# qcraftai/pillarnext

Measured on AMD Instinct MI355X. Metric: frames/s PillarNeXt-B nuScenes 300k-pt cloud (inference, end-to-end), higher is better.
Workload: dtype bf16

## Files before the change

include/pnx.h:

```cpp
#ifndef PNX_H
#define PNX_H

#include <stddef.h>
#include <stdint.h>

#ifdef __cplusplus
extern "C" {
#endif

typedef void* pnx_stream_t;

typedef enum pnx_status {
  PNX_OK = 0,
  PNX_ERR_INVALID = -1,
  PNX_ERR_UNSUPPORTED = -2,
  PNX_ERR_WORKSPACE = -3,
  PNX_ERR_HIP = -4
} pnx_status;

typedef enum pnx_dtype { PNX_F32 = 0, PNX_BF16 = 1, PNX_F16 = 2 } pnx_dtype;
typedef enum pnx_layout {
  PNX_NHWC = 0,
  PNX_NCHW = 1
} pnx_layout;
// ... 15 lines not shown
                    const float* w0, const float* gamma0, const float* beta0, const float* mean0, const float* var0,
                    const float* w1, const float* gamma1, const float* beta1, const float* mean1, const float* var1,
                    float eps, float* folded_out, pnx_stream_t stream);

size_t pnx_reader_workspace_bytes(int64_t n_points, int32_t batch, const pnx_geom* geom_host);

int pnx_reader_forward(const float* points, int64_t n_points, int32_t row_stride, int32_t batch, const pnx_geom* geom_host,
                       const float* pfn_folded, void* canvas, int32_t canvas_dtype, int32_t canvas_layout, uint8_t* occupancy,
                       float* feat_max, int32_t* coords, int64_t pillar_capacity, int64_t* unq_inv, int32_t* pillar_of_point,
                       int32_t* counts, void* workspace, size_t workspace_bytes, pnx_stream_t stream);

void pnx_reader_fill_split(int32_t* percent3_host);

int pnx_profile_begin(int32_t max_samples);
int pnx_profile_end(float* reader_us_avg_host, float* canvas_us_avg_host, int32_t* samples_host);
float pnx_profile_last_pfn_us(void);
float pnx_profile_last_voxelize_us(void);

size_t pnx_pfn_train_param_floats(int32_t num_point_features);
size_t pnx_pfn_train_partial_floats(int32_t num_point_features, int32_t which);
int pnx_pfn_forward_train(int32_t pass, const float* points, int64_t n_points, int32_t row_stride, int32_t batch, const pnx_geom* geom_host,
                          const float* params, float* partials, float* feat_max, int64_t pillar_capacity, int32_t* coords,
                          int32_t* pillar_of_point, int32_t* counts, void* workspace, size_t workspace_bytes, pnx_stream_t stream);
int pnx_pfn_backward(int32_t pass, int64_t n_points, int32_t row_stride, int32_t batch, const pnx_geom* geom_host, const float* params,
                     const float* grad_feat_max, const float* feat_max, float* partials, void* workspace, size_t workspace_bytes,
                     pnx_stream_t stream);

int pnx_voxelize(const float* points, int64_t n_points, int32_t row_stride, int32_t batch, const pnx_geom* geom_host,
                 float* features, int32_t* coords, int64_t pillar_capacity, int64_t* unq_inv, int32_t* pillar_of_point,
                 int32_t* counts, void* workspace, size_t workspace_bytes, pnx_stream_t stream);

typedef enum pnx_group_mode { PNX_GROUP_VOXEL = 0, PNX_GROUP_PILLAR_CLAMP = 1, PNX_GROUP_CYLINDER_CLAMP = 2 } pnx_group_mode;
typedef struct pnx_group_geom {
  float min[3], voxel[3];
  int32_t grid[3];
  int32_t mode;
  int32_t prefilter;
  float keep_min[3], keep_max[3];
} pnx_group_geom;
size_t pnx_group_workspace_bytes(int64_t n_points, int32_t row_stride, int32_t batch, const pnx_group_geom* geom_host);
int pnx_group_points(const float* points, int64_t n_points, int32_t row_stride, int32_t batch, const pnx_group_geom* geom_host, float* point_features,
                     int32_t feature_ld, int32_t* coords, int64_t group_capacity, int64_t* unq_inv, float* group_mean, int32_t* counts, void* workspace,
                     size_t workspace_bytes, pnx_stream_t stream);
int pnx_pfn_layer_eval(const float* xa, int32_t lda, int32_t ca, const float* gb, int32_t cb, const int64_t* inv, const float* wt, const float* shift,
                       int32_t cout, int64_t n, int64_t num_groups, float* y, int32_t ldy, float* gmax, pnx_stream_t stream);
int pnx_bilinear_gather(const void* image, int32_t dtype, int32_t batch, int32_t h, int32_t w, int32_t channels, const float* pos, int32_t pos_ld,
                        const float* pos_min2_host, const float* pos_voxel2_host, const int32_t* cell_coords, const int64_t* unq_inv, int32_t ds_rate,
                        int64_t n, float* out, int32_t out_ld, pnx_stream_t stream);
size_t pnx_bilinear_gather_backward_workspace_bytes(int64_t n, int32_t batch, int32_t h, int32_t w);
int pnx_bilinear_gather_backward(const float* grad_out, int32_t grad_ld, int32_t batch, int32_t h, int32_t w, int32_t channels, const float* pos,
                                 int32_t pos_ld, const float* pos_min2_host, const float* pos_voxel2_host, const int32_t* cell_coords,
                                 const int64_t* unq_inv, int32_t ds_rate, int64_t n, float* grad_image, void* workspace, size_t workspace_bytes,
                                 pnx_stream_t stream);

size_t pnx_scatter_max_workspace_bytes(int64_t n, int64_t num_pillars);
int pnx_scatter_max(const float* x, const int64_t* index, int64_t n, int32_t channels, int64_t num_pillars, float* out,
                    int64_t* argmax, void* workspace, size_t workspace_bytes, pnx_stream_t stream);
int pnx_scatter_max_backward(const float* grad_out, const int64_t* argmax, int64_t n, int32_t channels, int64_t num_pillars,
                             float* grad_x, pnx_stream_t stream);

int pnx_scatter_canvas(const float* feat_max, const int32_t* coords, const int32_t* num_pillars_dev, int64_t pillar_capacity,
                       int32_t batch, int32_t gy, int32_t gx, void* canvas, int32_t canvas_dtype, int32_t canvas_layout,
                       pnx_stream_t stream);

size_t pnx_merge_sweeps_desc_bytes(void);
size_t pnx_merge_sweeps_workspace_bytes(int64_t n_raw);
int pnx_merge_sweeps(const float* raw, int64_t n_raw, int32_t raw_stride, int32_t n_copy, const void* seg_descs_dev, int32_t n_segments, float* out,
                     int32_t* n_out_dev, void* workspace, size_t workspace_bytes, pnx_stream_t stream);

int pnx_bias_act_mask(const void* x, const void* residual, const float* bias, const uint8_t* mask, void* out, int64_t sites,
                      int32_t channels, int32_t dtype, int32_t relu, pnx_stream_t stream);
int pnx_sum_bias_act(const void* const* srcs, int32_t n_src, const float* bias, void* out, int64_t sites, int32_t channels, int32_t dtype,
                     int32_t relu, pnx_stream_t stream);
int pnx_deconv2x2_bf16(const void* x, const void* wfrag, const float* bias, void* y, int32_t batch, int32_t h, int32_t w, int32_t cin, int32_t cout,
                       int32_t relu, pnx_stream_t stream);
int pnx_deconv2x2_f16(const void* x, const void* wfrag, const float* bias, void* y, int32_t batch, int32_t h, int32_t w, int32_t cin, int32_t cout,
                       int32_t relu, pnx_stream_t stream);
int pnx_conv3x3_bf16(const void* x, const void* wfrag, const float* bias, const void* residual, const uint8_t* mask, void* y, int32_t batch,
                     int32_t h, int32_t w, int32_t cin, int32_t cout, int32_t stride, int32_t relu, uint8_t* row_dirty, const int32_t* tile_list,
                     const int32_t* tile_count, pnx_stream_t stream);
int pnx_conv3x3_f16(const void* x, const void* wfrag, const float* bias, const void* residual, const uint8_t* mask, void* y, int32_t batch,
                    int32_t h, int32_t w, int32_t cin, int32_t cout, int32_t stride, int32_t relu, uint8_t* row_dirty, const int32_t* tile_list,
                    const int32_t* tile_count, pnx_stream_t stream);
size_t pnx_conv3x3_wgrad_workspace_bytes(int32_t cin, int32_t cout);
int pnx_conv3x3_wgrad_bf16(const void* x, const void* dy, const uint8_t* mask, float* dw, int32_t batch, int32_t h, int32_t w, int32_t cin, int32_t cout,
                           int32_t stride, void* workspace, size_t workspace_bytes, pnx_stream_t stream);
int pnx_conv3x3_wgrad_x3(const void* x_hi, const void* x_lo, const void* dy_hi, const void* dy_lo, const uint8_t* mask, float* dw, int32_t batch, int32_t h,
                         int32_t w, int32_t cin, int32_t cout, int32_t stride, void* workspace, size_t workspace_bytes, pnx_stream_t stream);
int pnx_conv3x3_wgrad_x6(const void* x_hi, const void* x_mid, const void* x_lo, const void* dy_hi, const void* dy_mid, const void* dy_lo, const uint8_t* mask,
                         float* dw, int32_t batch, int32_t h, int32_t w, int32_t cin, int32_t cout, int32_t stride, void* workspace, size_t workspace_bytes,
                         pnx_stream_t stream);
int pnx_conv3x3_pack_weights(const void* w, int32_t dtype, int32_t cout, int32_t cin, int32_t transposed, void* wfrag, pnx_stream_t stream);
int pnx_conv3x3_tile_rows(int32_t cin, int32_t cout, int32_t stride);
int pnx_conv_tile_list(const uint8_t* mask, const uint8_t* const* row_dirty, int32_t n_dirty, int32_t batch, int32_t h, int32_t w, int32_t tile_rows,
                       int32_t* tile_list, int32_t* tile_count, pnx_stream_t stream);
int pnx_sephead_out_bf16(const void* x, const void* wfrag, const float* bias, void* y, int32_t batch, int32_t h, int32_t w, int32_t n_branch,
                         pnx_stream_t stream);
int pnx_sephead_out_f16(const void* x, const void* wfrag, const float* bias, void* y, int32_t batch, int32_t h, int32_t w, int32_t n_branch,
                         pnx_stream_t stream);
typedef struct {
  const void* up;
  const void* wfrag1;
  const float* bias1;
  const float* w2c;
  const float* bias2;
  int32_t h, w;
} PnxLazyTask;
int pnx_sephead_lazy_bf16(const PnxLazyTask* tasks, int32_t n_tasks, const int32_t* class_task, int32_t nc_total, int32_t batch, const int64_t* local,
                          const int32_t* seg_len, int32_t pre_max, float* out, pnx_stream_t stream);
int pnx_sephead_lazy_f16(const PnxLazyTask* tasks, int32_t n_tasks, const int32_t* class_task, int32_t nc_total, int32_t batch, const int64_t* local,
                          const int32_t* seg_len, int32_t pre_max, float* out, pnx_stream_t stream);
int pnx_split_f32(const float* x, void* hi, void* lo, int64_t n, const uint8_t* mask, int32_t channels, pnx_stream_t stream);
int pnx_conv3x3_x3(const void* x_hi, const void* x_lo, const void* wfrag_hi, const void* wfrag_lo, const float* bias, const uint8_t* mask, float* y,
                   int32_t batch, int32_t h, int32_t w, int32_t cin, int32_t cout, int32_t stride, pnx_stream_t stream);
int pnx_split3_f32(const float* x, void* hi, void* mid, void* lo, int64_t n, const uint8_t* mask, int32_t channels, pnx_stream_t stream);
int pnx_conv3x3_x6(const void* x_hi, const void* x_mid, const void* x_lo, const void* wfrag_hi, const void* wfrag_mid, const void* wfrag_lo, const float* bias,
                   const uint8_t* mask, float* y, int32_t batch, int32_t h, int32_t w, int32_t cin, int32_t cout, int32_t stride, pnx_stream_t stream);
int pnx_conv3x3_dgrad_s2_bf16(const void* g, const void* wfrag_t, const uint8_t* mask_in, void* dx, int32_t batch, int32_t h, int32_t w, int32_t cin,
                              int32_t cout, pnx_stream_t stream);
int pnx_conv3x3_dgrad_s2_x3(const void* g_hi, const void* g_lo, const void* wfrag_t_hi, const void* wfrag_t_lo, const uint8_t* mask_in, float* dx, int32_t batch,
                            int32_t h, int32_t w, int32_t cin, int32_t cout, pnx_stream_t stream);
int pnx_conv3x3_dgrad_s2_x6(const void* g_hi, const void* g_mid, const void* g_lo, const void* wfrag_t_hi, const void* wfrag_t_mid, const void* wfrag_t_lo,
                            const uint8_t* mask_in, float* dx, int32_t batch, int32_t h, int32_t w, int32_t cin, int32_t cout, pnx_stream_t stream);
int pnx_conv3x3_smallk(const void* x, const float* weight, const float* bias, void* y, int32_t batch, int32_t h, int32_t w, int32_t cin, int32_t k,
                       int32_t dtype, pnx_stream_t stream);
size_t pnx_conv3x3_smallk_wgrad_workspace_bytes(int32_t k);
int pnx_conv3x3_smallk_wgrad(const void* x, const void* dy, float* dw, float* dbias, int32_t batch, int32_t h, int32_t w, int32_t cin, int32_t k,
                             int32_t dtype, void* workspace, size_t workspace_bytes, pnx_stream_t stream);
int pnx_mask_pool3(const uint8_t* mask_in, int32_t batch, int32_t h, int32_t w, int32_t stride, uint8_t* mask_out, pnx_stream_t stream);

int pnx_boxes_overlap_bev(const float* boxes_a, int64_t n, const float* boxes_b, int64_t m, float* out, pnx_stream_t stream);
int pnx_boxes_iou_bev(const float* boxes_a, int64_t n, const float* boxes_b, int64_t m, float* out, pnx_stream_t stream);
int pnx_boxes_aligned_overlap_bev(const float* boxes_a, const float* boxes_b, int64_t n, float* out, pnx_stream_t stream);
int pnx_boxes_aligned_iou3d(const float* boxes_a, const float* boxes_b, int64_t n, float* out, pnx_stream_t stream);

int pnx_boxes_iou_bev_cpu(const float* boxes_a_host, int64_t n, const float* boxes_b_host, int64_t m, float* out_host);
int pnx_boxes_aligned_iou_bev_cpu(const float* boxes_a_host, const float* boxes_b_host, int64_t n, float* out_host);
size_t pnx_nms_workspace_bytes(int64_t total_boxes, int32_t num_segments, int32_t max_seg_len);
int32_t pnx_debug_nms_pair_cap(int32_t cap);
int pnx_nms_rotated_batched(const float* boxes, const int32_t* seg_offsets, const int32_t* seg_len, int32_t num_segments, int32_t max_seg_len,
                            const float* thresh, int32_t post_max, int32_t* keep, int32_t* keep_count, void* workspace,
                            size_t workspace_bytes, pnx_stream_t stream);
int pnx_nms_normal_batched(const float* boxes, const int32_t* seg_offsets, const int32_t* seg_len, int32_t num_segments, int32_t max_seg_len,
                           const float* thresh, int32_t post_max, int32_t* keep, int32_t* keep_count, void* workspace,
                           size_t workspace_bytes, pnx_stream_t stream);

size_t pnx_decode_task_desc_bytes(void);
size_t pnx_decode_topk_workspace_bytes(int64_t n_keys, int32_t num_segments);
int pnx_decode_topk(const uint64_t* keys, int64_t n_keys, int32_t num_segments, int32_t pre_max, uint64_t* sorted_keys, int64_t* order,
                    int64_t* seg_start, int32_t* seg_len, int32_t* seg_total, void* workspace, size_t workspace_bytes, pnx_stream_t stream);
int pnx_decode_keys(const void* packed, int32_t dtype, int32_t batch, int32_t n_classes_total, const void* task_desc_host, uint64_t* keys,
                    pnx_stream_t stream);
size_t pnx_sort_keys_workspace_bytes(int64_t n_keys);
int pnx_sort_keys(const uint64_t* keys, int64_t n_keys, int32_t num_segments, uint64_t* sorted_keys, int64_t* order, void* workspace,
                  size_t workspace_bytes, pnx_stream_t stream);
int pnx_decode_boxes(const void* const* task_ptrs_dev, const void* task_descs_dev, const int64_t* task_key_off_dev, int32_t n_tasks,
                     int32_t dtype, int32_t batch, const uint64_t* sorted_keys, const int64_t* order, const int64_t* seg_start,
                     const int32_t* seg_len, int32_t num_segments, int32_t pre_max, float* boxes9, float* boxes7, float* scores,
                     pnx_stream_t stream);
int pnx_decode_boxes_lazy(const void* task_descs_dev, const int64_t* task_key_off_dev, int32_t n_tasks, int32_t n_classes_total,
                          const uint64_t* sorted_keys, const int64_t* order, const int64_t* seg_start, int32_t* seg_len, const int32_t* seg_total,
                          int32_t num_segments, int32_t pre_max, const float* cand, float* boxes9, float* boxes7, float* scores, int32_t* flag_dev,
                          pnx_stream_t stream);
int pnx_gather_kept(const float* boxes9, const float* scores, const int32_t* keep, const int32_t* keep_count, int32_t num_segments,
                    int32_t pre_max, int32_t post_max, float* out, pnx_stream_t stream);

// ... 136 lines not shown
```

pillarnext_amd/_lib.py:

```python
import ctypes
import os

_HERE = os.path.dirname(os.path.abspath(__file__))
LIB_PATH = os.environ.get("PNX_LIB") or os.path.join(_HERE, "libpnx_hip.so")

PNX_F32, PNX_BF16, PNX_F16 = 0, 1, 2
PNX_NHWC, PNX_NCHW = 0, 1


class PnxError(RuntimeError):
    pass


class PnxGeom(ctypes.Structure):
    _fields_ = [("pc_min", ctypes.c_float * 3), ("voxel", ctypes.c_float * 3), ("gx", ctypes.c_int32), ("gy", ctypes.c_int32)]


PNX_GROUP_VOXEL, PNX_GROUP_PILLAR_CLAMP, PNX_GROUP_CYLINDER_CLAMP = 0, 1, 2


class PnxGroupGeom(ctypes.Structure):
    _fields_ = [("min", ctypes.c_float * 3), ("voxel", ctypes.c_float * 3), ("grid", ctypes.c_int32 * 3), ("mode", ctypes.c_int32),
                ("prefilter", ctypes.c_int32), ("keep_min", ctypes.c_float * 3), ("keep_max", ctypes.c_float * 3)]


PNX_ASSIGN_MAX_TASKS, PNX_ASSIGN_MAX_CLASSES = 8, 32
PNX_PASTE_MAX_BOXES, PNX_PASTE_MAX_BATCH = 512, 64
PNX_AUG_ROTATE, PNX_AUG_SCALE, PNX_AUG_TRANSLATE, PNX_AUG_FLIP_X, PNX_AUG_FLIP_Y = 1, 2, 4, 8, 16


class PnxAssignDesc(ctypes.Structure):
    _fields_ = [("lo", ctypes.c_double * 2), ("voxel", ctypes.c_double * 2), ("overlap", ctypes.c_double), ("min_radius", ctypes.c_int32),
                ("max_objs", ctypes.c_int32), ("n_tasks", ctypes.c_int32), ("n_classes", ctypes.c_int32)] + \
               [(k, ctypes.c_int32 * PNX_ASSIGN_MAX_TASKS) for k in ("osf", "h", "w", "ncls")] + \
               [(k, ctypes.c_int32 * PNX_ASSIGN_MAX_CLASSES) for k in ("class_task", "class_cls")]


_vp = ctypes.c_void_p
_i64 = ctypes.c_int64
_i32 = ctypes.c_int32
_f32 = ctypes.c_float
_sz = ctypes.c_size_t
_i3p = ctypes.POINTER(ctypes.c_int32)

PROTOTYPES = {
    "pnx_last_error": (ctypes.c_char_p, []),
    "pnx_version": (ctypes.c_char_p, []),
    "pnx_geom_init": (ctypes.c_int, [ctypes.POINTER(ctypes.c_double), ctypes.POINTER(ctypes.c_double), ctypes.POINTER(PnxGeom)]),
    "pnx_pfn_fold_bn": (ctypes.c_int, [_i32] + [_vp] * 10 + [_f32, _vp, _vp]),
    "pnx_reader_workspace_bytes": (_sz, [_i64, _i32, ctypes.POINTER(PnxGeom)]),
    "pnx_reader_forward": (ctypes.c_int, [_vp, _i64, _i32, _i32, ctypes.POINTER(PnxGeom), _vp, _vp, _i32, _i32, _vp, _vp, _vp, _i64, _vp, _vp,
                                          _vp, _vp, _sz, _vp]),
    "pnx_reader_fill_split": (None, [ctypes.POINTER(ctypes.c_int32)]),
    "pnx_profile_begin": (ctypes.c_int, [_i32]),
    "pnx_profile_end": (ctypes.c_int, [ctypes.POINTER(ctypes.c_float), ctypes.POINTER(ctypes.c_float), ctypes.POINTER(ctypes.c_int32)]),
    "pnx_profile_last_pfn_us": (ctypes.c_float, []),
    "pnx_profile_last_voxelize_us": (ctypes.c_float, []),
    "pnx_pfn_train_param_floats": (_sz, [_i32]),
    "pnx_pfn_train_partial_floats": (_sz, [_i32, _i32]),
    "pnx_pfn_forward_train": (ctypes.c_int, [_i32, _vp, _i64, _i32, _i32, ctypes.POINTER(PnxGeom), _vp, _vp, _vp, _i64, _vp, _vp, _vp, _vp, _sz, _vp]),
    "pnx_pfn_backward": (ctypes.c_int, [_i32, _i64, _i32, _i32, ctypes.POINTER(PnxGeom), _vp, _vp, _vp, _vp, _vp, _sz, _vp]),
    "pnx_voxelize": (ctypes.c_int, [_vp, _i64, _i32, _i32, ctypes.POINTER(PnxGeom), _vp, _vp, _i64, _vp, _vp, _vp, _vp, _sz, _vp]),
    "pnx_group_workspace_bytes": (_sz, [_i64, _i32, _i32, ctypes.POINTER(PnxGroupGeom)]),
    "pnx_group_points": (ctypes.c_int, [_vp, _i64, _i32, _i32, ctypes.POINTER(PnxGroupGeom), _vp, _i32, _vp, _i64, _vp, _vp, _vp, _vp, _sz, _vp]),
    "pnx_pfn_layer_eval": (ctypes.c_int, [_vp, _i32, _i32, _vp, _i32, _vp, _vp, _vp, _i32, _i64, _i64, _vp, _i32, _vp, _vp]),
    "pnx_bilinear_gather": (ctypes.c_int, [_vp, _i32, _i32, _i32, _i32, _i32, _vp, _i32, ctypes.POINTER(ctypes.c_float), ctypes.POINTER(ctypes.c_float), _vp,
                                           _vp, _i32, _i64, _vp, _i32, _vp]),
    "pnx_bilinear_gather_backward_workspace_bytes": (_sz, [_i64, _i32, _i32, _i32]),
    "pnx_bilinear_gather_backward": (ctypes.c_int, [_vp, _i32, _i32, _i32, _i32, _i32, _vp, _i32, ctypes.POINTER(ctypes.c_float),
                                                    ctypes.POINTER(ctypes.c_float), _vp, _vp, _i32, _i64, _vp, _vp, _sz, _vp]),
    "pnx_scatter_max_workspace_bytes": (_sz, [_i64, _i64]),
    "pnx_scatter_max": (ctypes.c_int, [_vp, _vp, _i64, _i32, _i64, _vp, _vp, _vp, _sz, _vp]),
    "pnx_scatter_max_backward": (ctypes.c_int, [_vp, _vp, _i64, _i32, _i64, _vp, _vp]),
    "pnx_scatter_canvas": (ctypes.c_int, [_vp, _vp, _vp, _i64, _i32, _i32, _i32, _vp, _i32, _i32, _vp]),
    "pnx_merge_sweeps_desc_bytes": (_sz, []),
    "pnx_merge_sweeps_workspace_bytes": (_sz, [_i64]),
    "pnx_merge_sweeps": (ctypes.c_int, [_vp, _i64, _i32, _i32, _vp, _i32, _vp, _vp, _vp, _sz, _vp]),
    "pnx_bias_act_mask": (ctypes.c_int, [_vp, _vp, _vp, _vp, _vp, _i64, _i32, _i32, _i32, _vp]),
    "pnx_sum_bias_act": (ctypes.c_int, [_vp, _i32, _vp, _vp, _i64, _i32, _i32, _i32, _vp]),
    "pnx_deconv2x2_bf16": (ctypes.c_int, [_vp, _vp, _vp, _vp, _i32, _i32, _i32, _i32, _i32, _i32, _vp]),
    "pnx_deconv2x2_f16": (ctypes.c_int, [_vp, _vp, _vp, _vp, _i32, _i32, _i32, _i32, _i32, _i32, _vp]),
    "pnx_sephead_out_bf16": (ctypes.c_int, [_vp, _vp, _vp, _vp, _i32, _i32, _i32, _i32, _vp]),
    "pnx_sephead_out_f16": (ctypes.c_int, [_vp, _vp, _vp, _vp, _i32, _i32, _i32, _i32, _vp]),
    "pnx_masked_bn_blocks": (_i32, []),
    "pnx_masked_bn_reduce": (ctypes.c_int, [_vp, _i32, _i32, _vp, _vp]),
    "pnx_masked_bn_finalize": (ctypes.c_int, [_vp, _i32, _vp, _vp, _vp, ctypes.c_double, ctypes.c_double, _vp, _vp, _vp, _vp, _vp, _vp, _vp, _vp, _vp]),
    "pnx_masked_bn_bwd_finalize": (ctypes.c_int, [_vp, _vp, _i32, _vp, _vp, _vp, _vp, _vp, _vp]),
    "pnx_masked_bn_stats": (ctypes.c_int, [_vp, _i32, _vp, _i64, _i32, _vp, _vp, _vp]),
    "pnx_masked_bn_apply": (ctypes.c_int, [_vp, _vp, _i32, _vp, _i64, _i32, _vp, _vp, _i32, _vp, _vp]),
    "pnx_masked_bn_bwd_stats": (ctypes.c_int, [_vp, _vp, _vp, _i32, _vp, _i64, _i32, _vp, _vp, _vp, _vp, _i32, _vp, _vp]),
    "pnx_masked_bn_bwd_apply": (ctypes.c_int, [_vp, _vp, _vp, _i32, _vp, _i64, _i32, _vp, _vp, _vp, _vp, _i32, _vp, _vp, _vp, _vp, _vp]),
    "pnx_sephead_lazy_bf16": (ctypes.c_int, [_vp, _i32, _vp, _i32, _i32, _vp, _vp, _i32, _vp, _vp]),
    "pnx_sephead_lazy_f16": (ctypes.c_int, [_vp, _i32, _vp, _i32, _i32, _vp, _vp, _i32, _vp, _vp]),
    "pnx_conv3x3_bf16": (ctypes.c_int, [_vp, _vp, _vp, _vp, _vp, _vp, _i32, _i32, _i32, _i32, _i32, _i32, _i32, _vp, _vp, _vp, _vp]),
    "pnx_conv3x3_f16": (ctypes.c_int, [_vp, _vp, _vp, _vp, _vp, _vp, _i32, _i32, _i32, _i32, _i32, _i32, _i32, _vp, _vp, _vp, _vp]),
    "pnx_conv3x3_tile_rows": (ctypes.c_int, [_i32, _i32, _i32]),
    "pnx_conv3x3_pack_weights": (ctypes.c_int, [_vp, _i32, _i32, _i32, _i32, _vp, _vp]),
    "pnx_conv3x3_wgrad_workspace_bytes": (_sz, [_i32, _i32]),
    "pnx_conv3x3_wgrad_bf16": (ctypes.c_int, [_vp, _vp, _vp, _vp, _i32, _i32, _i32, _i32, _i32, _i32, _vp, _sz, _vp]),
    "pnx_conv3x3_wgrad_x3": (ctypes.c_int, [_vp, _vp, _vp, _vp, _vp, _vp, _i32, _i32, _i32, _i32, _i32, _i32, _vp, _sz, _vp]),
    "pnx_conv3x3_wgrad_x6": (ctypes.c_int, [_vp, _vp, _vp, _vp, _vp, _vp, _vp, _vp, _i32, _i32, _i32, _i32, _i32, _i32, _vp, _sz, _vp]),
    "pnx_conv3x3_dgrad_s2_bf16": (ctypes.c_int, [_vp, _vp, _vp, _vp, _i32, _i32, _i32, _i32, _i32, _vp]),
    "pnx_conv3x3_dgrad_s2_x3": (ctypes.c_int, [_vp, _vp, _vp, _vp, _vp, _vp, _i32, _i32, _i32, _i32, _i32, _vp]),
    "pnx_conv3x3_dgrad_s2_x6": (ctypes.c_int, [_vp, _vp, _vp, _vp, _vp, _vp, _vp, _vp, _i32, _i32, _i32, _i32, _i32, _vp]),
    "pnx_conv3x3_smallk": (ctypes.c_int, [_vp, _vp, _vp, _vp, _i32, _i32, _i32, _i32, _i32, _i32, _vp]),
    "pnx_conv3x3_smallk_wgrad_workspace_bytes": (_sz, [_i32]),
    "pnx_conv3x3_smallk_wgrad": (ctypes.c_int, [_vp, _vp, _vp, _vp, _i32, _i32, _i32, _i32, _i32, _i32, _vp, _sz, _vp]),
    "pnx_conv_tile_list": (ctypes.c_int, [_vp, _vp, _i32, _i32, _i32, _i32, _i32, _vp, _vp, _vp]),
    "pnx_mask_pool3": (ctypes.c_int, [_vp, _i32, _i32, _i32, _i32, _vp, _vp]),
    "pnx_split_f32": (ctypes.c_int, [_vp, _vp, _vp, _i64, _vp, _i32, _vp]),
    "pnx_conv3x3_x3": (ctypes.c_int, [_vp, _vp, _vp, _vp, _vp, _vp, _vp, _i32, _i32, _i32, _i32, _i32, _i32, _vp]),
    "pnx_split3_f32": (ctypes.c_int, [_vp, _vp, _vp, _vp, _i64, _vp, _i32, _vp]),
    "pnx_conv3x3_x6": (ctypes.c_int, [_vp, _vp, _vp, _vp, _vp, _vp, _vp, _vp, _vp, _i32, _i32, _i32, _i32, _i32, _i32, _vp]),
    "pnx_decode_task_desc_bytes": (_sz, []),
    "pnx_decode_topk_workspace_bytes": (_sz, [_i64, _i32]),
    "pnx_decode_topk": (ctypes.c_int, [_vp, _i64, _i32, _i32, _vp, _vp, _vp, _vp, _vp, _vp, _sz, _vp]),
    "pnx_decode_keys": (ctypes.c_int, [_vp, _i32, _i32, _i32, _vp, _vp, _vp]),
    "pnx_sort_keys_workspace_bytes": (ctypes.c_size_t, [_i64]),
    "pnx_sort_keys": (ctypes.c_int, [_vp, _i64, _i32, _vp, _vp, _vp, ctypes.c_size_t, _vp]),
    "pnx_decode_boxes": (ctypes.c_int, [_vp, _vp, _vp, _i32, _i32, _i32, _vp, _vp, _vp, _vp, _i32, _i32, _vp, _vp, _vp, _vp]),
    "pnx_decode_boxes_lazy": (ctypes.c_int, [_vp, _vp, _i32, _i32, _vp, _vp, _vp, _vp, _vp, _i32, _i32, _vp, _vp, _vp, _vp, _vp, _vp]),
    "pnx_gather_kept": (ctypes.c_int, [_vp, _vp, _vp, _vp, _i32, _i32, _i32, _vp, _vp]),
    "pnx_enqueue": (ctypes.c_int, [_vp, _i32, _vp]),
    "pnx_decode_lazy_enqueue": (ctypes.c_int, [_vp, _vp]),
    "pnx_op_bytes": (_sz, []),
    "pnx_lazy_decode_bytes": (_sz, []),
    "pnx_center_loss_workspace_bytes": (_sz, [_i32, _i32]),
    "pnx_center_loss_forward": (ctypes.c_int, [_vp, _vp, _vp, _vp, _vp, _vp, _vp, _i32, _i32, _i32, _i32, _i32, _vp, _i32, _vp, _vp, _sz, _vp]),
    "pnx_center_loss_backward": (ctypes.c_int, [_vp, _vp, _vp, _vp, _vp, _vp, _vp, _vp, _i32, _i32, _i32, _i32, _i32, _vp, _i32, _vp, _vp, _vp, _vp, _sz, _vp]),
    "pnx_assign_workspace_bytes": (_sz, [_i32, _i32, _i32]),
    "pnx_assign_labels": (ctypes.c_int, [_vp, _vp, _vp, _i32, _i32, ctypes.POINTER(PnxAssignDesc), _vp, _vp, _vp, _vp, _vp, _vp, _vp, _vp, _sz, _vp]),
    "pnx_paste_chunk_rows": (_i32, []),
    "pnx_paste_select": (ctypes.c_int, [_vp, _vp, _vp, _i32, _i32, _i32, _vp, _vp, _vp, _vp, _i32, _i32, _vp, _i32, _vp, _vp, _vp, _vp, _vp, _vp, _vp]),
    "pnx_paste_augment_workspace_bytes": (_sz, [_i64, _i32]),
    "pnx_paste_augment_points": (ctypes.c_int, [_vp, _i64, _i32, _i32, _vp, _vp, _vp, _vp, _i32, _i32, _vp, _vp, _i32, _i64, _vp, _vp, _i64, _vp, _vp, _vp,
                                                _sz, _vp]),
    "pnx_augment_boxes": (ctypes.c_int, [_vp, _vp, _i32, _i32, _i32, _vp, _vp]),
    "pnx_boxes_overlap_bev": (ctypes.c_int, [_vp, _i64, _vp, _i64, _vp, _vp]),
    "pnx_boxes_iou_bev": (ctypes.c_int, [_vp, _i64, _vp, _i64, _vp, _vp]),
    "pnx_boxes_aligned_overlap_bev": (ctypes.c_int, [_vp, _vp, _i64, _vp, _vp]),
    "pnx_boxes_aligned_iou3d": (ctypes.c_int, [_vp, _vp, _i64, _vp, _vp]),
    "pnx_boxes_iou_bev_cpu": (ctypes.c_int, [_vp, _i64, _vp, _i64, _vp]),
    "pnx_boxes_aligned_iou_bev_cpu": (ctypes.c_int, [_vp, _vp, _i64, _vp]),
    "pnx_nms_workspace_bytes": (_sz, [_i64, _i32, _i32]),
    "pnx_debug_nms_pair_cap": (_i32, [_i32]),
    "pnx_nms_rotated_batched": (ctypes.c_int, [_vp, _vp, _vp, _i32, _i32, _vp, _i32, _vp, _vp, _vp, _sz, _vp]),
    "pnx_nms_normal_batched": (ctypes.c_int, [_vp, _vp, _vp, _i32, _i32, _vp, _i32, _vp, _vp, _vp, _sz, _vp]),
    "pnx_sp3_index_bytes": (_sz, [_i32, _i3p]),
    "pnx_sp3_index_build": (ctypes.c_int, [_vp, _i64, _i32, _i3p, _vp, _sz, _vp, _vp, _vp]),
    "pnx_sp3_out_grid": (ctypes.c_int, [_i32, _i3p, _i3p, _i3p, _i3p, _i3p]),
    "pnx_sp3_out_index": (ctypes.c_int, [_vp, _i64, _i32, _i3p, _i3p, _i3p, _i3p, _vp, _sz, _vp, _vp]),
    "pnx_sp3_index_coords": (ctypes.c_int, [_vp, _sz, _i32, _i3p, _vp, _i64, _vp]),
    "pnx_sp3_neighbor_map": (ctypes.c_int, [_vp, _i64, _vp, _sz, _i32, _i3p, _vp, _i3p, _i3p, _i3p, _vp, _vp]),
    "pnx_sp3_packed_weight_floats": (_sz, [_i32, _i32, _i32]),
    "pnx_sp3_conv": (ctypes.c_int, [_vp, _i64, _i32, _vp, _i64, _i32, _vp, _vp, _vp, _i32, _vp, _i32, _vp]),
    "pnx_sp3_conv_train": (ctypes.c_int, [_vp, _i64, _i32, _vp, _i64, _i32, _vp, _vp, _vp, _i32, _vp, _i32, _vp]),
    "pnx_sp3_dense": (ctypes.c_int, [_vp, _vp, _i64, _i32, _i32, _i3p, _vp, _vp]),
    "pnx_sp3_packed_weight_halfs": (_sz, [_i32, _i32, _i32]),
    "pnx_sp3_conv_h": (ctypes.c_int, [_vp, _i64, _i32, _i32, _vp, _i64, _i32, _vp, _vp, _vp, _i32, _vp, _i32, _i32, _i32, _vp]),
    "pnx_sp3_dense_h": (ctypes.c_int, [_vp, _i32, _vp, _i64, _i32, _i32, _i32, _i3p, _vp, _vp]),
    "pnx_sp3_transpose_map": (ctypes.c_int, [_vp, _i64, _i32, _i64, _vp, _vp]),
    "pnx_sp3_wgrad_workspace_bytes": (_sz, [_i64, _i32, _i32, _i32]),
    "pnx_sp3_wgrad": (ctypes.c_int, [_vp, _i64, _i32, _vp, _i32, _vp, _i64, _i32, _vp, _vp, _sz, _vp]),
    "pnx_sp3_dense_backward": (ctypes.c_int, [_vp, _vp, _i64, _i32, _i32, _i3p, _vp, _vp]),
}

_LIB = None


def lib():
    global _LIB
    if _LIB is None:
        if not os.path.exists(LIB_PATH):
            raise PnxError(f"{LIB_PATH} is missing: run `python -m pillarnext_amd.build` (hipcc, gfx950). "
                           "There is no CPU fallback for the product path.")
        L = ctypes.CDLL(LIB_PATH)
        for name, (res, args) in PROTOTYPES.items():
            fn = getattr(L, name)
# ... 29 lines not shown
```

pillarnext_amd/csrc/conv3x3.hip:

```cpp
#include "pnx_common.h"

namespace {

#include "conv_tile.h"

template <int CIN, int COUT, int STRIDE, bool W_LDS>
__global__ __launch_bounds__(256, 2) void k_conv3x3(const uint16_t* __restrict__ x, const uint4* __restrict__ wfrag,
                                                 const float* __restrict__ bias, const uint16_t* __restrict__ res,
                                                 const uint8_t* __restrict__ mask, uint16_t* __restrict__ y, int B, int H, int W, int Ho,
                                                 int Wo, int relu, uint8_t* __restrict__ row_dirty) {
  constexpr int CB = CIN / 16, MT = COUT / 32, KSTEPS = 9 * CB;
  constexpr int NT = (MT <= 2) ? 4 : 2;
  extern __shared__ uint4 s_w[];
  const int lane = threadIdx.x & 63, wv = threadIdx.x >> 6;
  const int px = lane & 31, kb = lane >> 5;
  if (W_LDS) {
    for (int i = threadIdx.x; i < KSTEPS * MT * 64; i += 256) s_w[i] = wfrag[i];
    __syncthreads();
  }
  const int tiles_x = (Wo + 31) >> 5, tiles_y = (Ho + NT - 1) / NT;
  const int64_t n_tiles = (int64_t)B * tiles_y * tiles_x;
  for (int64_t tile = (int64_t)blockIdx.x * 4 + wv; tile < n_tiles; tile += (int64_t)gridDim.x * 4) {
    const int tx = (int)(tile % tiles_x);
    const int ty = (int)((tile / tiles_x) % tiles_y);
// ... 199 lines not shown
  return PNX_OK;
}

}

extern "C" {

#if defined(PNX_CONV_TIMERS) && !defined(PNX_CONV_F16)
int pnx_debug_conv_timers(unsigned long long* out) {
  unsigned long long z[8] = {0, 0, 0, 0, 0, 0, 0, 0};
  PNX_CHECK_HIP(hipDeviceSynchronize());
  PNX_CHECK_HIP(hipMemcpyFromSymbol(out, HIP_SYMBOL(g_conv_T), sizeof(z)));
  PNX_CHECK_HIP(hipMemcpyToSymbol(HIP_SYMBOL(g_conv_T), z, sizeof(z)));
  return PNX_OK;
}
#endif

int PNX_CONV_FN(pnx_sephead_out)(const void* x, const void* wfrag, const float* bias, void* y, int32_t batch, int32_t h, int32_t w, int32_t n_branch,
                         pnx_stream_t stream) {
  PNX_REQUIRE(x && wfrag && bias && y && batch > 0 && h > 0 && w > 0, PNX_ERR_INVALID, "bad arguments");
  PNX_REQUIRE((((uintptr_t)x | (uintptr_t)y | (uintptr_t)wfrag | (uintptr_t)bias) & 15) == 0, PNX_ERR_INVALID, "16-byte alignment required");
  hipStream_t st = (hipStream_t)stream;
  switch (n_branch) {
    case 1: return launch_sephead<1>(x, wfrag, bias, y, batch, h, w, st);
    case 2: return launch_sephead<2>(x, wfrag, bias, y, batch, h, w, st);
    case 5: return launch_sephead<5>(x, wfrag, bias, y, batch, h, w, st);
    case 6: return launch_sephead<6>(x, wfrag, bias, y, batch, h, w, st);
    case 7: return launch_sephead<7>(x, wfrag, bias, y, batch, h, w, st);
    default: break;
  }
  pnx_set_error("pnx_sephead_out: no kernel for %d branches", n_branch);
  return PNX_ERR_UNSUPPORTED;
}

int PNX_CONV_FN(pnx_deconv2x2)(const void* x, const void* wfrag, const float* bias, void* y, int32_t batch, int32_t h, int32_t w, int32_t cin, int32_t cout,
                       int32_t relu, pnx_stream_t stream) {
  PNX_REQUIRE(x && wfrag && bias && y && batch > 0 && h > 0 && w > 0, PNX_ERR_INVALID, "bad arguments");
  PNX_REQUIRE((((uintptr_t)x | (uintptr_t)y | (uintptr_t)wfrag | (uintptr_t)bias) & 15) == 0, PNX_ERR_INVALID, "16-byte alignment required");
  if (cin != 64 || cout != 64) {
    pnx_set_error("pnx_deconv2x2: no kernel for %d -> %d channels", cin, cout);
    return PNX_ERR_UNSUPPORTED;
  }
  const int64_t n_seg = (int64_t)batch * h * ((w + 31) / 32);
  int64_t nb = (n_seg + 3) / 4;
  if (nb > 512) nb = 512;
  k_deconv2x2_64<<<(unsigned)nb, 256, 0, (hipStream_t)stream>>>((const uint16_t*)x, (const uint4*)wfrag, bias, (uint16_t*)y, batch, h, w, relu);
  PNX_LAUNCH_CHECK();
  return PNX_OK;
}

#ifndef PNX_CONV_F16
int pnx_conv3x3_tile_rows(int32_t cin, int32_t cout, int32_t stride) {
  if (stride != 1) return 0;
  if (cin == 64 && (cout == 64 || cout == 320 || cout == 384 || cout == 448)) return LDS_TH;
  if ((cin == 128 && cout == 128) || (cin == 256 && (cout == 256 || cout == 64))) return L128_TH;
  return 0;
}

static int conv_tile_list_impl(const uint8_t* mask, const uint8_t* const* row_dirty, int32_t n_dirty, int32_t batch, int32_t h, int32_t w, int32_t tile_rows,
                               int32_t* tile_list, int32_t* tile_count, pnx_stream_t stream, bool zero_count) {
  PNX_REQUIRE(mask && tile_list && tile_count && batch > 0 && h > 0 && w > 0 && tile_rows > 0, PNX_ERR_INVALID, "bad arguments");
  PNX_REQUIRE(n_dirty >= 0 && n_dirty <= 4 && (n_dirty == 0 || row_dirty != nullptr), PNX_ERR_INVALID, "0..4 row_dirty arrays");
  DirtySet ds;
  for (int k = 0; k < 4; k++) ds.p[k] = k < n_dirty ? row_dirty[k] : nullptr;
  hipStream_t st = (hipStream_t)stream;
  if (zero_count) PNX_CHECK_HIP(hipMemsetAsync(tile_count, 0, sizeof(int32_t), st));
  const int64_t n_tiles = (int64_t)batch * ((h + tile_rows - 1) / tile_rows) * ((w + 31) / 32);
  PNX_REQUIRE(tile_rows <= 16, PNX_ERR_UNSUPPORTED, "tile_rows %d (at most 16: one lane per row)", tile_rows);
  k_tile_list<<<(unsigned)((n_tiles + 15) / 16), 256, 0, st>>>(mask, ds, batch, h, w, tile_rows, tile_list, tile_count);
  PNX_LAUNCH_CHECK();
  return PNX_OK;
}
int pnx_conv_tile_list(const uint8_t* mask, const uint8_t* const* row_dirty, int32_t n_dirty, int32_t batch, int32_t h, int32_t w, int32_t tile_rows,
                       int32_t* tile_list, int32_t* tile_count, pnx_stream_t stream) {
  return conv_tile_list_impl(mask, row_dirty, n_dirty, batch, h, w, tile_rows, tile_list, tile_count, stream, true);
}
int pnx_conv_tile_list_prezeroed(const uint8_t* mask, const uint8_t* const* row_dirty, int32_t n_dirty, int32_t batch, int32_t h, int32_t w, int32_t tile_rows,
                                 int32_t* tile_list, int32_t* tile_count, pnx_stream_t stream) {
  return conv_tile_list_impl(mask, row_dirty, n_dirty, batch, h, w, tile_rows, tile_list, tile_count, stream, false);
}

#endif

int PNX_CONV_FN(pnx_conv3x3)(const void* x, const void* wfrag, const float* bias, const void* residual, const uint8_t* mask, void* y, int32_t batch,
                     int32_t h, int32_t w, int32_t cin, int32_t cout, int32_t stride, int32_t relu, uint8_t* row_dirty, const int32_t* tile_list,
                     const int32_t* tile_count, pnx_stream_t stream) {
  PNX_REQUIRE((tile_list == nullptr) == (tile_count == nullptr), PNX_ERR_INVALID, "tile_list and tile_count come together");
  PNX_REQUIRE(tile_list == nullptr || (mask != nullptr && pnx_conv3x3_tile_rows(cin, cout, stride) > 0), PNX_ERR_INVALID,
              "a tile list needs a mask and a kernel that takes one (pnx_conv3x3_tile_rows)");
  PNX_REQUIRE(x && wfrag && bias && y && batch > 0 && h > 0 && w > 0, PNX_ERR_INVALID, "bad arguments");
  PNX_REQUIRE(stride == 1 || stride == 2, PNX_ERR_UNSUPPORTED, "stride %d", stride);
  PNX_REQUIRE(row_dirty == nullptr || mask != nullptr, PNX_ERR_INVALID, "row_dirty needs an active-site mask");
  PNX_REQUIRE((((uintptr_t)x | (uintptr_t)y | (uintptr_t)wfrag | (uintptr_t)bias | (uintptr_t)residual) & 15) == 0, PNX_ERR_INVALID,
              "16-byte alignment required");
  const int ho = (h + 2 - 3) / stride + 1, wo = (w + 2 - 3) / stride + 1;
  hipStream_t st = (hipStream_t)stream;
  const ConvArgs a = {(const uint16_t*)x, (const uint4*)wfrag, bias, (const uint16_t*)residual, mask, (uint16_t*)y, batch, h, w, relu, row_dirty, tile_list,
                      tile_count, st};
  if (stride == 1 && getenv("PNX_CONV_DIRECT") == nullptr) {
    static const int pc_mode = getenv("PNX_CONV_PC") != nullptr ? atoi(getenv("PNX_CONV_PC")) : 1;
    static const int pack_mode = getenv("PNX_CONV_PACK") != nullptr ? atoi(getenv("PNX_CONV_PACK")) : 3;
    if (pc_mode != 0) {
      if (cin == 64 && cout == 64) return launch_pc<64, 64>(a, (pack_mode & 2) != 0);
      if (residual == nullptr && (pc_mode & 4)) {
        if (cin == 64 && cout == 320) return launch_pc<64, 320>(a);
        if (cin == 64 && cout == 384) return launch_pc<64, 384>(a);
        if (cin == 64 && cout == 448) return launch_pc<64, 448>(a);
      }
      if (pc_mode & 2) {
        if (cin == 128 && cout == 128) return launch_pc<128, 128>(a);
        if (cin == 256 && cout == 256) return launch_pc<256, 256>(a);
      }
    }
    if (cin == 64 && cout == 64) return launch_lds<64>(a);
    const bool pack = (pack_mode & 1) != 0;
    if (cin == 128 && cout == 128) return launch_ldsx<128, 128>(a, pack);
    if (cin == 256 && cout == 64) return launch_ldsx<256, 64>(a);
    if (cin == 256 && cout == 256) return launch_ldsx<256, 256>(a, pack);
    if (cin == 64 && cout == 384) return launch_lds<384>(a);
    if (cin == 64 && cout == 320) return launch_lds<320>(a);
    if (cin == 64 && cout == 448) return launch_lds<448>(a);
  }
  if (stride == 2 && residual == nullptr && getenv("PNX_CONV_DIRECT") == nullptr) {
    if (cin == 64 && cout == 128) return launch_s2<64, 128, 1>(x, wfrag, bias, mask, y, batch, h, w, ho, wo, relu, row_dirty, st);
    if (cin == 128 && cout == 256) return launch_s2<128, 256, 1>(x, wfrag, bias, mask, y, batch, h, w, ho, wo, relu, row_dirty, st);
    if (cin == 256 && cout == 256) return launch_s2<256, 256, 1>(x, wfrag, bias, mask, y, batch, h, w, ho, wo, relu, row_dirty, st);
  }
#define PNX_CONV_CASE(CI, CO)                             \
  if (cin == CI && cout == CO) {                          \
    if (stride == 1) return launch<CI, CO, 1>(a, ho, wo); \
    return launch<CI, CO, 2>(a, ho, wo);                  \
  }
  PNX_CONV_CASE(64, 64)
  PNX_CONV_CASE(64, 128)
  PNX_CONV_CASE(128, 128)
#undef PNX_CONV_CASE
  pnx_set_error("pnx_conv3x3: no kernel for %d -> %d channels", cin, cout);
  return PNX_ERR_UNSUPPORTED;
}

#ifndef PNX_CONV_F16
}
namespace {
#include "conv_dgrad_s2.h"

template <int NP>
int dgrad_s2_impl(const char* name, PnxPieces<NP> g, PnxPieces<NP> wfrag_t, const uint8_t* mask_in, void* dx, int32_t batch, int32_t h, int32_t w, int32_t cin,
                  int32_t cout, pnx_stream_t stream) {
  PNX_REQUIRE(g.complete() && wfrag_t.complete() && mask_in && dx && batch > 0 && h > 0 && w > 0, PNX_ERR_INVALID, "%s: bad arguments", name);
  PNX_REQUIRE(((g.bits() | wfrag_t.bits() | (uintptr_t)dx) & 15) == 0, PNX_ERR_INVALID, "16-byte alignment required");
  hipStream_t st = (hipStream_t)stream;
  if (cin == 64 && cout == 128) return launch_dgrad_s2<128, 64, NP>(g, wfrag_t, mask_in, dx, batch, h, w, st);
  if (cin == 128 && cout == 256) return launch_dgrad_s2<256, 128, NP>(g, wfrag_t, mask_in, dx, batch, h, w, st);
  if (cin == 256 && cout == 256) return launch_dgrad_s2<256, 256, NP>(g, wfrag_t, mask_in, dx, batch, h, w, st);
  pnx_set_error("%s: no kernel for %d -> %d channels", name, cin, cout);
  return PNX_ERR_UNSUPPORTED;
}

template <int NP>
int conv3x3_f32_impl(const char* name, PnxPieces<NP> x, PnxPieces<NP> wfrag, const float* bias, const uint8_t* mask, float* y, int32_t batch, int32_t h, int32_t w,
                     int32_t cin, int32_t cout, int32_t stride, pnx_stream_t stream) {
  PNX_REQUIRE(x.complete() && wfrag.complete() && y, PNX_ERR_INVALID, "null pointer");
  PNX_REQUIRE(batch > 0 && h > 0 && w > 0, PNX_ERR_INVALID, "bad shape");
  PNX_REQUIRE(stride == 1 || stride == 2, PNX_ERR_UNSUPPORTED, "stride %d", stride);
  PNX_REQUIRE(((x.bits() | wfrag.bits() | (uintptr_t)y | (uintptr_t)bias) & 15) == 0, PNX_ERR_INVALID, "16-byte alignment required");
  hipStream_t st = (hipStream_t)stream;
  if (stride == 1) {
    if (cin == 64 && cout == 64) return launch_pc_f32<64, 64, NP>(x, wfrag, bias, mask, y, batch, h, w, st);
    if (cin == 128 && cout == 128) return launch_pc_f32<128, 128, NP>(x, wfrag, bias, mask, y, batch, h, w, st);
    if (cin == 256 && cout == 256) return launch_pc_f32<256, 256, NP>(x, wfrag, bias, mask, y, batch, h, w, st);
  } else {
    const int ho = (h - 1) / 2 + 1, wo = (w - 1) / 2 + 1;
    if (cin == 64 && cout == 128) return launch_s2<64, 128, NP>(x, wfrag, bias, mask, y, batch, h, w, ho, wo, 0, nullptr, st);
    if (cin == 128 && cout == 256) return launch_s2<128, 256, NP>(x, wfrag, bias, mask, y, batch, h, w, ho, wo, 0, nullptr, st);
    if (cin == 256 && cout == 256) return launch_s2<256, 256, NP>(x, wfrag, bias, mask, y, batch, h, w, ho, wo, 0, nullptr, st);
  }
  pnx_set_error("%s: no kernel for %d -> %d channels, stride %d", name, cin, cout, stride);
  return PNX_ERR_UNSUPPORTED;
}

}
extern "C" {

int pnx_conv3x3_dgrad_s2_bf16(const void* g, const void* wfrag_t, const uint8_t* mask_in, void* dx, int32_t batch, int32_t h, int32_t w, int32_t cin, int32_t cout,
                              pnx_stream_t stream) {
  return dgrad_s2_impl<1>("pnx_conv3x3_dgrad_s2_bf16", {g}, {wfrag_t}, mask_in, dx, batch, h, w, cin, cout, stream);
}

int pnx_conv3x3_dgrad_s2_x3(const void* g_hi, const void* g_lo, const void* wfrag_t_hi, const void* wfrag_t_lo, const uint8_t* mask_in, float* dx, int32_t batch,
                            int32_t h, int32_t w, int32_t cin, int32_t cout, pnx_stream_t stream) {
  return dgrad_s2_impl<2>("pnx_conv3x3_dgrad_s2_x3", {g_hi, g_lo}, {wfrag_t_hi, wfrag_t_lo}, mask_in, dx, batch, h, w, cin, cout, stream);
}

int pnx_conv3x3_dgrad_s2_x6(const void* g_hi, const void* g_mid, const void* g_lo, const void* wfrag_t_hi, const void* wfrag_t_mid, const void* wfrag_t_lo,
                            const uint8_t* mask_in, float* dx, int32_t batch, int32_t h, int32_t w, int32_t cin, int32_t cout, pnx_stream_t stream) {
  return dgrad_s2_impl<3>("pnx_conv3x3_dgrad_s2_x6", {g_hi, g_mid, g_lo}, {wfrag_t_hi, wfrag_t_mid, wfrag_t_lo}, mask_in, dx, batch, h, w, cin, cout, stream);
}

int pnx_conv3x3_x3(const void* x_hi, const void* x_lo, const void* wfrag_hi, const void* wfrag_lo, const float* bias, const uint8_t* mask, float* y,
                   int32_t batch, int32_t h, int32_t w, int32_t cin, int32_t cout, int32_t stride, pnx_stream_t stream) {
  return conv3x3_f32_impl<2>("pnx_conv3x3_x3", {x_hi, x_lo}, {wfrag_hi, wfrag_lo}, bias, mask, y, batch, h, w, cin, cout, stride, stream);
}

int pnx_conv3x3_x6(const void* x_hi, const void* x_mid, const void* x_lo, const void* wfrag_hi, const void* wfrag_mid, const void* wfrag_lo, const float* bias,
                   const uint8_t* mask, float* y, int32_t batch, int32_t h, int32_t w, int32_t cin, int32_t cout, int32_t stride, pnx_stream_t stream) {
  return conv3x3_f32_impl<3>("pnx_conv3x3_x6", {x_hi, x_mid, x_lo}, {wfrag_hi, wfrag_mid, wfrag_lo}, bias, mask, y, batch, h, w, cin, cout, stride, stream);
}
#endif

}

namespace {

constexpr int kLzG = 32, kLzN = kLzG * 9, kLzNT = kLzN / 32;
constexpr int kLzPatch = kLzG * 25 * 8;
constexpr int kLzW2 = 10 * 9 * 32 * 3;
constexpr int kLzMaxTasks = 8, kLzMaxClasses = 32;
constexpr int kLzAhead = 2;

#include "sephead_lazy.h"

// ... 26 lines not shown
```

pillarnext_amd/csrc/conv_rows.h:

```cpp
#pragma once


template <int NR, int COUT, bool HAS_RES>
__device__ __forceinline__ void conv_rows(const uint4* __restrict__ s_in, const uint4* __restrict__ wfrag, const float* __restrict__ bias,
                                          const uint16_t* const (&rrow_res)[4], uint32_t res_off, const int (&rbase)[4], const uint32_t (&rmask)[4],
                                          uint16_t* const (&yrow)[4], int n_valid, int relu, int px, int kb, int lane) {
  constexpr int MTALL = COUT / 32;
#pragma unroll 1
  for (int mg = 0; mg < MTALL; mg += 2) {
    v16f acc[NR][2];
#pragma unroll
    for (int m = 0; m < 2; m++) {
      const v16f bq = bias_tile(bias, (mg + m) * 32, kb);
#pragma unroll
      for (int j = 0; j < NR; j++) acc[j][m] = bq;
    }
    uint4 rq[2][2];
    if (HAS_RES) load_residual_u(rq, rrow_res[0], res_off, rmask[0] >> px & 1u);
    conv_taps<NR, MTALL, 4, 1, 2, COUT == 64 ? 2 : TAPS_WD>(acc, s_in, wfrag, rbase, mg, px, kb, lane);
#pragma unroll
    for (int j = 0; j < NR; j++) {
      const bool act = (rmask[j] >> px) & 1u;
      uint4 rc[2][2];
      if (HAS_RES) {
// ... 70 lines not shown
#pragma unroll
    for (int j = 0; j < 4; j++) {
      was[j] = __builtin_amdgcn_readfirstlane(wasP[j]) != 0;
      const uint32_t bal = (uint32_t)__ballot(aP[j]);
      if (lane == 0) s_rowmask[wv * 4 + j] = bal;
    }
    __syncthreads();
    idxC = sched_next2(s_next, it, slot, idxB);
    tileC = tile_at(tlist, idxC, n_tiles);
    load_mask(tileB, aN, wasN);
#pragma unroll
    for (int j = 0; j < 4; j++) aP[j] = aN[j], wasP[j] = wasN[j];
    CT_TOCK(0)
    const uint32_t my_rm = s_rowmask[lane & 15];
    const uint32_t am = (uint32_t)__ballot(my_rm != 0) & 0xffffu;
#pragma unroll
    for (int j = 0; j < 4; j++) {
      const int rr = wv * 4 + j, oy = y0 + rr;
      const bool active = (am >> rr) & 1u;
      if (!active && was[j] && oy < H && ox < W) {
        uint4* dst = reinterpret_cast<uint4*>(y + (((int64_t)b * H + oy) * W + ox) * COUT);
#pragma unroll 1
        for (int ch = kb; ch < COUT / 8; ch += 2) dst[ch] = make_uint4(0, 0, 0, 0);
      }
      if (row_dirty != nullptr && oy < H && lane == 0 && was[j] != active) row_dirty[((int64_t)b * H + oy) * tiles_x + tx] = active ? 1 : 0;
    }
    if (am == 0) continue;
    int nr = 0;
    int rbase[4], rrow[4];
    {
      uint32_t rest = am;
      for (int k = 0; k < wv && rest; k++) rest &= rest - 1;
#pragma unroll
      for (int j = 0; j < 4; j++) {
        const bool has = rest != 0;
        rrow[j] = has ? __builtin_ctz(rest) : 0;
        nr += has ? 1 : 0;
        for (int k = 0; k < 4 && rest; k++) rest &= rest - 1;
      }
    }
    nr = __builtin_amdgcn_readfirstlane(nr);
    uint32_t rmask[4];
    uint16_t* yrow[4];
#pragma unroll
    for (int j = 0; j < 4; j++) {
      rrow[j] = __builtin_amdgcn_readfirstlane(rrow[j]);
      rbase[j] = rrow[j] * HW_ * 8;
      rmask[j] = j < nr ? __builtin_amdgcn_readfirstlane(s_rowmask[rrow[j]]) : 0u;
      yrow[j] = y + (((int64_t)b * H + (y0 + rrow[j])) * W + x0) * COUT;
    }
    const uint32_t need = am | (am << 1) | (am << 2);
    CT_TOCK(1)
    const uint16_t* rres[4];
#pragma unroll
    for (int j = 0; j < 4; j++) rres[j] = HAS_RES ? res + (((int64_t)b * H + (y0 + rrow[j])) * W + x0) * COUT : nullptr;
    const uint32_t res_off = (uint32_t)(px * COUT + 8 * kb) * 2u;
    stage_tile64<CIN>(s_in, x, b, H, W, 0, y0, x0, need);
    CT_TOCK(2)
    __syncthreads();
    CT_TOCK(3)
    const int n_valid = W - x0;
    switch (nr) {
      case 1: conv_rows<1, COUT, HAS_RES>(s_in, wfrag, bias, rres, res_off, rbase, rmask, yrow, n_valid, relu, px, kb, lane); break;
      case 2: conv_rows<2, COUT, HAS_RES>(s_in, wfrag, bias, rres, res_off, rbase, rmask, yrow, n_valid, relu, px, kb, lane); break;
      case 3: conv_rows<3, COUT, HAS_RES>(s_in, wfrag, bias, rres, res_off, rbase, rmask, yrow, n_valid, relu, px, kb, lane); break;
      case 4: conv_rows<4, COUT, HAS_RES>(s_in, wfrag, bias, rres, res_off, rbase, rmask, yrow, n_valid, relu, px, kb, lane); break;
      default: break;
    }
    CT_TOCK(4)
  }
  sched_done(slot);
  CT_FLUSH
}

constexpr int L128_TH = 8;
constexpr int L128_NSTAGE = (L128_TH + 2) * LDS_HW * 8;

int next_sched_slot() {
  static unsigned int n = 0;
  return (int)(n++ & 63u);
}

constexpr int LDSX_RES_WD = 2;
template <int NR, int CIN, int COUT, bool HAS_RES>
__device__ __forceinline__ void conv_rows_x(uint4* __restrict__ s_in, const uint16_t* __restrict__ x, const uint4* __restrict__ wfrag,
                                            const float* __restrict__ bias, const uint16_t* __restrict__ res, const int (&rrow)[4],
                                            const int (&rbase)[4], const uint32_t (&rmask)[4], uint16_t* const (&yrow)[4], int b, int H, int W,
                                            int y0, int x0, uint32_t need, int mg0, int relu, int px, int kb, int lane, int hsel) {
  constexpr int NS = CIN / 64, NRA = NR > 0 ? NR : 1;
  const int ox = x0 + px;
  {
    const int h = hsel;
    const int mg = mg0 + 4 * h;
    v16f acc[NRA][2];
    if (NR > 0) {
#pragma unroll
      for (int m = 0; m < 2; m++) {
        const v16f bq = bias_tile(bias, (mg + m) * 32, kb);
#pragma unroll
        for (int j = 0; j < NR; j++) acc[j][m] = bq;
      }
    }
    const uint16_t* rres[NRA];
    const uint32_t res_off = (uint32_t)(px * COUT + 8 * kb) * 2u;
    uint4 rq[2][2];
    if (NR > 0 && HAS_RES) {
#pragma unroll
      for (int j = 0; j < NR; j++) rres[j] = res + (((int64_t)b * H + (y0 + rrow[j])) * W + x0) * COUT + mg * 32;
    }
#pragma unroll 1
    for (int sl = 0; sl < NS; sl++) {
      if (sl) {
        __syncthreads();
        stage_tile64<CIN, L128_TH>(s_in, x, b, H, W, 64 * sl, y0, x0, need);
        __syncthreads();
      }
      if (NR > 0 && HAS_RES && sl == NS - 1) load_residual_u(rq, rres[0], res_off, rmask[0] >> px & 1u);
      if (NR > 0) conv_taps<NRA, COUT / 32, CIN / 16, 1, 2, HAS_RES ? LDSX_RES_WD : TAPS_WD>(acc, s_in, wfrag, rbase, mg, px, kb, lane, 4 * sl);
    }
    if (NR > 0) {
      const int n_valid = W - x0;
#pragma unroll
      for (int j = 0; j < NR; j++) {
        const bool act = (rmask[j] >> px) & 1u;
        uint4 rc[2][2];
        if (HAS_RES) {
#pragma unroll
          for (int m = 0; m < 2; m++)
#pragma unroll
            for (int t = 0; t < 2; t++) rc[m][t] = rq[m][t];
          if (j + 1 < NR) load_residual_u(rq, rres[j + 1], res_off, rmask[j + 1] >> px & 1u);
        }
        uint4 D[4];
#pragma unroll
        for (int m = 0; m < 2; m++) {
          uint4 pk[2];
          pack_tile(acc[j][m], act, relu, pk, HAS_RES ? rc[m] : nullptr);
          D[2 * m] = pk[0], D[2 * m + 1] = pk[1];
        }
        transpose_row64(D, lane);
        store_row64<COUT>(D, yrow[j] + mg * 32, n_valid, lane);
      }
    }
  }
}

__device__ __forceinline__ int pix_code(int row, int col) { return (row << 5) | col; }
template <int CSTRIDE>
__device__ __forceinline__ uint32_t pix_off(int code, int W) { return (uint32_t)(((code >> 5) * W + (code & 31)) * CSTRIDE) * 2u; }

template <int CSTRIDE>
__device__ __forceinline__ void store_pix64(const uint4 (&D)[4], uint16_t* __restrict__ tile, int code, int n_valid, int W, int lane) {
  int l = lane;
  asm volatile("" : "+v"(l));
#pragma unroll
  for (int d = 0; d < 4; d++) {
    const int P = 8 * d + (l >> 3);
    const int pc = __builtin_amdgcn_ds_bpermute(P << 2, code);
    if (P < n_valid) *reinterpret_cast<uint4*>(reinterpret_cast<char*>(tile) + pix_off<CSTRIDE>(pc, W) + (uint32_t)((l & 7) * 16)) = D[d];
  }
}

template <int NR, int CIN, int COUT, bool HAS_RES>
__device__ __forceinline__ void conv_pix_x(uint4* __restrict__ s_in, const uint16_t* __restrict__ x, const uint4* __restrict__ wfrag,
                                           const float* __restrict__ bias, const uint16_t* __restrict__ rtile, int codes, const int (&n_g)[4],
                                           uint16_t* __restrict__ ytile, int b, int H, int W, int y0, int x0, uint32_t need, int mg0, int relu, int px,
                                           int kb, int lane, int hsel) {
  constexpr int NS = CIN / 64, NRA = NR > 0 ? NR : 1;
  const int mg = mg0 + 4 * hsel;
  v16f acc[NRA][2];
  if (NR > 0) {
#pragma unroll
    for (int m = 0; m < 2; m++) {
      const v16f bq = bias_tile(bias, (mg + m) * 32, kb);
#pragma unroll
      for (int j = 0; j < NR; j++) acc[j][m] = bq;
    }
  }
  const uint16_t* const rres = HAS_RES ? rtile + mg * 32 : nullptr;
  auto code = [&](int j) { return (codes >> (8 * j)) & 255; };
  auto res_off = [&](int j) { return pix_off<COUT>(code(j), W) + (uint32_t)(16 * kb); };
  const int cw[4] = {codes, 0, 0, 0};
  uint4 rq[2][2];
#pragma unroll 1
  for (int sl = 0; sl < NS; sl++) {
    if (sl) {
      __syncthreads();
      stage_tile64<CIN, L128_TH>(s_in, x, b, H, W, 64 * sl, y0, x0, need);
      __syncthreads();
    }
    if (NR > 0 && HAS_RES && sl == NS - 1) load_residual_u(rq, rres, res_off(0), px < n_g[0]);
    if (NR > 0) conv_taps<NRA, COUT / 32, CIN / 16, 1, 2, HAS_RES ? LDSX_RES_WD : TAPS_WD, true>(acc, s_in, wfrag, cw, mg, px, kb, lane, 4 * sl);
  }
  if (NR > 0) {
#pragma unroll
    for (int j = 0; j < NR; j++) {
      const bool act = px < n_g[j];
      uint4 rc[2][2];
      if (HAS_RES) {
#pragma unroll
        for (int m = 0; m < 2; m++)
#pragma unroll
          for (int t = 0; t < 2; t++) rc[m][t] = rq[m][t];
        if (j + 1 < NR) load_residual_u(rq, rres, res_off(j + 1), px < n_g[j + 1]);
      }
      uint4 D[4];
#pragma unroll
      for (int m = 0; m < 2; m++) {
        uint4 pk[2];
        pack_tile(acc[j][m], act, relu, pk, HAS_RES ? rc[m] : nullptr);
        D[2 * m] = pk[0], D[2 * m + 1] = pk[1];
      }
      transpose_row64(D, lane);
      store_pix64<COUT>(D, ytile + mg * 32, code(j), n_g[j], W, lane);
    }
  }
}

template <int CIN, int COUT, bool HAS_RES, bool PACK = false>
__global__ __launch_bounds__(256, 2) void k_conv3x3_ldsx(const uint16_t* __restrict__ x, const uint4* __restrict__ wfrag,
                                                      const float* __restrict__ bias, const uint16_t* __restrict__ res,
                                                      const uint8_t* __restrict__ mask, uint16_t* __restrict__ y, int B, int H, int W,
                                                      int relu, uint8_t* __restrict__ row_dirty, int slot, const int32_t* __restrict__ tlist,
                                                      const int32_t* __restrict__ tcount) {
  static_assert(CIN % 64 == 0 && (COUT % 128 == 0 || COUT == 64), "64-channel input slabs, 128-channel output passes (or one of 64)");
  constexpr int TH = L128_TH, HW_ = LDS_HW;
  constexpr int NRG = COUT == 64 ? 4 : 2, NRMAX = TH / NRG;
  static_assert(!PACK || (CIN == COUT && NRG == 2), "the packed-pixel form serves 128 -> 128 and 256 -> 256");
  __shared__ uint4 s_in[L128_NSTAGE];
  __shared__ uint16_t s_list[PACK ? TH * 32 : 1];
  __shared__ uint32_t s_rowmask2[2 * TH];
  __shared__ unsigned int s_next[2];
  const int lane = threadIdx.x & 63, wv = threadIdx.x >> 6;
  const int px = lane & 31, kb = lane >> 5;
  const int rg = wv % NRG, mg0 = 2 * (wv / NRG);
  const int tiles_x = (W + 31) >> 5, tiles_y = (H + TH - 1) / TH;
  const int n_tiles = tlist != nullptr ? __builtin_amdgcn_readfirstlane(*tcount) : B * tiles_y * tiles_x;
  constexpr int NH = (COUT + 127) / 128;
  const int n_units = n_tiles * NH;
  auto unit_at = [&](int64_t idx) -> int {
    if (idx >= n_units) return -1;
    const int i = (int)idx;
    const int t = tlist != nullptr ? tlist[i / NH] : i / NH;
    return t * NH + i % NH;
  };
  auto load_mask = [&](int t, bool (&a)[2], int (&wz)[2]) {
#pragma unroll
    for (int j = 0; j < 2; j++) a[j] = false, wz[j] = 1;
    if (t < 0) return;
    const int tx = (int)(t % tiles_x);
    const int ty = (int)((t / tiles_x) % tiles_y);
    const int b = (int)(t / ((int64_t)tiles_x * tiles_y));
    const int ox = tx * 32 + px;
#pragma unroll
    for (int j = 0; j < 2; j++) {
      const int oy = ty * TH + wv * 2 + j;
      a[j] = ox < W && oy < H && (mask == nullptr || mask[((int64_t)b * H + oy) * W + ox] != 0);
      if (row_dirty != nullptr && oy < H) wz[j] = (int)row_dirty[((int64_t)b * H + oy) * tiles_x + tx];
    }
  };
  int64_t idxB = (int64_t)blockIdx.x + gridDim.x, idxC = 0;
  int tileA = unit_at(blockIdx.x), tileB = unit_at(idxB), tileC = -1;
  bool aP[2], aN[2];
  int wasP[2], wasN[2];
  load_mask(tileA >= 0 ? tileA / NH : -1, aP, wasP);
#pragma unroll
  for (int j = 0; j < 2; j++) aN[j] = false, wasN[j] = 1;
  int it = 0;
  for (; tileA >= 0; tileA = tileB, tileB = tileC, idxB = idxC, it++) {
    const int unit = __builtin_amdgcn_readfirstlane(tileA);
    const int tile = unit / NH;
    const int hsel = unit - tile * NH;
    sched_draw(s_next, it, slot);
    uint32_t* const s_rowmask = s_rowmask2 + (it & 1) * TH;
    const int tx = (int)(tile % tiles_x);
    const int ty = (int)((tile / tiles_x) % tiles_y);
    const int b = (int)(tile / ((int64_t)tiles_x * tiles_y));
    const int x0 = tx * 32, y0 = ty * TH;
    const int ox = x0 + px;
    bool was[2];
    uint32_t bal[2];
#pragma unroll
    for (int j = 0; j < 2; j++) {
      was[j] = __builtin_amdgcn_readfirstlane(wasP[j]) != 0;
      bal[j] = (uint32_t)__ballot(aP[j]);
      if (lane == 0) s_rowmask[wv * 2 + j] = bal[j];
    }
    __syncthreads();
    idxC = sched_next2(s_next, it, slot, idxB);
    tileC = unit_at(idxC);
    load_mask(tileB >= 0 ? tileB / NH : -1, aN, wasN);
#pragma unroll
    for (int j = 0; j < 2; j++) aP[j] = aN[j], wasP[j] = wasN[j];
    const uint32_t my_rm = s_rowmask[lane & 7];
    const uint32_t am = (uint32_t)__ballot(my_rm != 0) & 0xffu;
#pragma unroll
    for (int j = 0; j < 2; j++) {
      const int rr = wv * 2 + j, oy = y0 + rr;
      const bool active = (am >> rr) & 1u;
      if (hsel != 0) continue;
      if (!active && was[j] && oy < H && ox < W) {
        uint4* dst = reinterpret_cast<uint4*>(y + (((int64_t)b * H + oy) * W + ox) * COUT);
#pragma unroll 1
        for (int ch = kb; ch < COUT / 8; ch += 2) dst[ch] = make_uint4(0, 0, 0, 0);
      }
      if (row_dirty != nullptr && oy < H && lane == 0 && was[j] != active) row_dirty[((int64_t)b * H + oy) * tiles_x + tx] = active ? 1 : 0;
    }
    if (am == 0) continue;
    if constexpr (PACK) {
      const int wvu = __builtin_amdgcn_readfirstlane(wv);
      int n_px = 0, pos = 0;
#pragma unroll
      for (int k = 0; k < TH; k++) {
        const int n = __builtin_popcount(__builtin_amdgcn_readlane(my_rm, k));
        n_px += n;
        pos += k < 2 * wvu ? n : 0;
      }
#pragma unroll
      for (int j = 0; j < 2; j++) {
        if (kb == 0 && ((bal[j] >> px) & 1u)) s_list[pos + __builtin_popcount(bal[j] & ((1u << px) - 1u))] = (uint16_t)pix_code(wvu * 2 + j, px);
        pos += __builtin_popcount(bal[j]);
      }
      const int n_grp = (n_px + 31) >> 5, rgu = __builtin_amdgcn_readfirstlane(rg);
      const int nr = n_grp > rgu ? (n_grp - rgu + 1) >> 1 : 0;
      const uint32_t need = am | (am << 1) | (am << 2);
      stage_tile64<CIN, TH>(s_in, x, b, H, W, 0, y0, x0, need);
      __syncthreads();
      int codes = 0, n_g[4];
#pragma unroll
      for (int j = 0; j < 4; j++) {
        const int g = rgu + 2 * j;
        n_g[j] = min(max(n_px - 32 * g, 0), 32);
        if (j < nr && px < n_g[j]) codes |= (int)s_list[32 * g + px] << (8 * j);
      }
      const int64_t t0 = (((int64_t)b * H + y0) * W + x0) * COUT;
#define PNX_PIX_X(N_) conv_pix_x<N_, CIN, COUT, HAS_RES>(s_in, x, wfrag, bias, HAS_RES ? res + t0 : nullptr, codes, n_g, y + t0, b, H, W, y0, x0, need, mg0, relu, px, kb, lane, hsel)
      switch (nr) {
        case 0: PNX_PIX_X(0); break;
        case 1: PNX_PIX_X(1); break;
        case 2: PNX_PIX_X(2); break;
        case 3: PNX_PIX_X(3); break;
        default: PNX_PIX_X(4); break;
      }
#undef PNX_PIX_X
      int l = lane;
      asm volatile("" : "+v"(l));
      const uint32_t cols = W - x0 >= 32 ? 0xffffffffu : (1u << (W - x0)) - 1u;
#pragma unroll
      for (int j = 0; j < 2; j++) {
        const int rr = wvu * 2 + j;
        const uint32_t idle = ~bal[j] & cols;
        if (!((am >> rr) & 1u) || !was[j] || y0 + rr >= H || idle == 0) continue;
        char* const row = reinterpret_cast<char*>(y + t0) + (uint32_t)(rr * W * COUT * 2 + hsel * 256);
#pragma unroll 1
        for (int c0 = 0; c0 < 32; c0 += 4) {
          if (((idle >> c0) & 15u) == 0) continue;
          const int p = c0 + (l >> 4);
          if ((idle >> p) & 1u) *reinterpret_cast<uint4*>(row + (uint32_t)(p * COUT * 2 + (l & 15) * 16)) = make_uint4(0, 0, 0, 0);
        }
      }
      continue;
    }
    int nr = 0;
    int rbase[4], rrow[4];
    {
      uint32_t rest = am;
      for (int k = 0; k < rg && rest; k++) rest &= rest - 1;
#pragma unroll
      for (int j = 0; j < 4; j++) {
        const bool has = j < NRMAX && rest != 0;
        rrow[j] = has ? __builtin_ctz(rest) : 0;
        nr += has ? 1 : 0;
        for (int k = 0; k < NRG && rest; k++) rest &= rest - 1;
      }
    }
    nr = __builtin_amdgcn_readfirstlane(nr);
    uint32_t rmask[4];
    uint16_t* yrow[4];
#pragma unroll
    for (int j = 0; j < 4; j++) {
      rrow[j] = __builtin_amdgcn_readfirstlane(rrow[j]);
      rbase[j] = rrow[j] * HW_ * 8;
      rmask[j] = j < nr ? __builtin_amdgcn_readfirstlane(s_rowmask[rrow[j]]) : 0u;
      yrow[j] = y + (((int64_t)b * H + (y0 + rrow[j])) * W + x0) * COUT;
    }
    const uint32_t need = am | (am << 1) | (am << 2);
    stage_tile64<CIN, TH>(s_in, x, b, H, W, 0, y0, x0, need);
    __syncthreads();
#define PNX_ROWS_X(N_) conv_rows_x<(N_ <= NRMAX ? N_ : NRMAX), CIN, COUT, HAS_RES>(s_in, x, wfrag, bias, res, rrow, rbase, rmask, yrow, b, H, W, y0, x0, need, mg0, relu, px, kb, lane, hsel)
    switch (nr) {
      case 0: PNX_ROWS_X(0); break;
      case 1: PNX_ROWS_X(1); break;
      case 2: PNX_ROWS_X(2); break;
      case 3: PNX_ROWS_X(3); break;
      default: PNX_ROWS_X(4); break;
    }
#undef PNX_ROWS_X
  }
  sched_done(slot);
}

template <int CIN, int COUT>
int launch_ldsx(const ConvArgs& a, bool pack = false) {
  const int slot = a.mask != nullptr ? next_sched_slot() : -1;
  int64_t nb = (int64_t)a.B * ((a.H + L128_TH - 1) / L128_TH) * ((a.W + 31) / 32) * ((COUT + 127) / 128);
  if (nb > 512) nb = 512;
  if constexpr (CIN == COUT) {
    if (pack && a.mask != nullptr) {
      if (a.res != nullptr)
        k_conv3x3_ldsx<CIN, COUT, true, true><<<(unsigned)nb, 256, 0, a.st>>>(a.x, a.wfrag, a.bias, a.res, a.mask, a.y, a.B, a.H, a.W, a.relu, a.row_dirty, slot,
                                                                            a.tlist, a.tcount);
      else
        k_conv3x3_ldsx<CIN, COUT, false, true><<<(unsigned)nb, 256, 0, a.st>>>(a.x, a.wfrag, a.bias, nullptr, a.mask, a.y, a.B, a.H, a.W, a.relu, a.row_dirty, slot,
                                                                             a.tlist, a.tcount);
      PNX_LAUNCH_CHECK();
      return PNX_OK;
    }
  }
  if (a.res != nullptr)
    k_conv3x3_ldsx<CIN, COUT, true><<<(unsigned)nb, 256, 0, a.st>>>(a.x, a.wfrag, a.bias, a.res, a.mask, a.y, a.B, a.H, a.W, a.relu, a.row_dirty, slot, a.tlist,
                                                                   a.tcount);
  else
    k_conv3x3_ldsx<CIN, COUT, false><<<(unsigned)nb, 256, 0, a.st>>>(a.x, a.wfrag, a.bias, nullptr, a.mask, a.y, a.B, a.H, a.W, a.relu, a.row_dirty, slot, a.tlist,
                                                                    a.tcount);
  PNX_LAUNCH_CHECK();
  return PNX_OK;
}
```

pillarnext_amd/csrc/conv_s2.h:

```cpp
#pragma once

constexpr int S2_TH = 4;
constexpr int S2_ROWS = 2 * S2_TH + 1;
constexpr int S2_NSTAGE = S2_ROWS * S2_RS * 8;

template <int CSTRIDE>
__device__ __forceinline__ void stage_tile64_s2(uint4* __restrict__ s_in, const uint16_t* __restrict__ x, int b, int H, int W, int ch0, int iy0,
                                                int ix0, uint32_t need) {
  typedef __attribute__((address_space(1))) const void* gptr_t;
  typedef __attribute__((address_space(3))) void* lptr_t;
  int tid = threadIdx.x;
  asm volatile("" : "+v"(tid));
  const int slot = tid & 7, col = tid >> 3, wbase = (tid >> 6) * 8;
  const uint16_t* xb = x + (int64_t)b * H * W * CSTRIDE + ch0;
#pragma unroll
  for (int pl = 0; pl < 2; pl++) {
    const int ls = pl * 32 + col;
    const int ix = ix0 + 2 * col + (1 - pl);
    const bool col_ok = (unsigned)ix < (unsigned)W;
    const int chunk = slot ^ lds_swz(ls);
#pragma unroll
    for (int r = 0; r < S2_ROWS; r++) {
      if (!((need >> r) & 1u)) continue;
      const int iy = iy0 + r;
      if ((unsigned)iy < (unsigned)H && col_ok) {
        __builtin_amdgcn_global_load_lds((gptr_t)(xb + ((int64_t)iy * W + ix) * CSTRIDE + chunk * 8),
                                         (lptr_t)(s_in + (r * S2_RS + pl * 32 + wbase) * 8), 16, 0, 0);
      } else {
        s_in[(r * S2_RS + ls) * 8 + slot] = make_uint4(0, 0, 0, 0);
      }
    }
  }
  if (tid < S2_ROWS * 8) {
    const int re = tid >> 3, ce = tid & 7;
    if ((need >> re) & 1u) {
      const int iy = iy0 + re, ix = ix0 + 64;
      uint4 qe = make_uint4(0, 0, 0, 0);
      if ((unsigned)iy < (unsigned)H && (unsigned)ix < (unsigned)W) qe = *reinterpret_cast<const uint4*>(xb + ((int64_t)iy * W + ix) * CSTRIDE + ce * 8);
      s_in[(re * S2_RS + 64) * 8 + (ce ^ lds_swz(64))] = qe;
    }
  }
}

template <int NR, int CIN, int COUT, int MB, int NP = 1>
__device__ __forceinline__ void conv_rows_s2(uint4* __restrict__ s_in, const uint16_t* __restrict__ x, const uint16_t* __restrict__ x2,
                                             const uint16_t* __restrict__ x3, const uint4* __restrict__ wfrag, const uint4* __restrict__ wfrag2,
                                             const uint4* __restrict__ wfrag3, const float* __restrict__ bias, const int (&rbase)[4], const uint32_t (&rmask)[4],
                                             uint16_t* const (&yrow)[4], int b, int H, int W, int iy0, int ix0, int n_valid, uint32_t need, int mg,
                                             int relu, int px, int kb, int lane) {
  constexpr int NS = CIN / 64, NRA = NR > 0 ? NR : 1;
  constexpr bool X3 = NP == 2, F32 = NP > 1;
  v16f acc[NRA][MB];
  if (NR > 0) {
#pragma unroll
    for (int m = 0; m < MB; m++) {
      v16f bq;
      if (F32 && bias == nullptr) {
#pragma unroll
        for (int i = 0; i < 16; i++) bq[i] = 0.f;
      } else {
        bq = bias_tile(bias, (mg + m) * 32, kb);
      }
#pragma unroll
      for (int j = 0; j < NR; j++) acc[j][m] = bq;
    }
  }
#pragma unroll 1
  for (int sq = 0; sq < NS * NP; sq++) {
    const int sl = F32 ? sq % NS : sq;
    if (sq) {
      __syncthreads();
      const uint16_t* xs = X3 && sq >= NS ? x2 : x;
      if constexpr (NP == 3) xs = sq < NS ? x3 : sq < 2 * NS ? x2 : x;
      stage_tile64_s2<CIN>(s_in, xs, b, H, W, 64 * sl, iy0, ix0, need);
      __syncthreads();
    }
    if (NR > 0) {
      if constexpr (NP == 3) {
        const int q = sq / NS;
#pragma unroll 1
        for (int k = q; k >= 0; k--)
          conv_taps<NRA, COUT / 32, CIN / 16, 2, MB>(acc, s_in, k == 0 ? wfrag : k == 1 ? wfrag2 : wfrag3, rbase, mg, px, kb, lane, 4 * sl);
      } else {
        conv_taps<NRA, COUT / 32, CIN / 16, 2, MB>(acc, s_in, wfrag, rbase, mg, px, kb, lane, 4 * sl);
        if constexpr (X3) {
          if (sq < NS) conv_taps<NRA, COUT / 32, CIN / 16, 2, MB>(acc, s_in, wfrag2, rbase, mg, px, kb, lane, 4 * sl);
        }
      }
    }
  }
  if (NR > 0) {
#pragma unroll
    for (int j = 0; j < NR; j++) {
      const bool act = (rmask[j] >> px) & 1u;
      if constexpr (F32) {
#pragma unroll
        for (int m = 0; m < MB; m++) store_tile_f32<COUT>(acc[j][m], act, reinterpret_cast<float*>(yrow[j]) + (mg + m) * 32, n_valid, px, kb);
      } else if constexpr (MB == 2) {
        uint4 D[4];
#pragma unroll
        for (int m = 0; m < 2; m++) {
          uint4 pk[2];
          pack_tile(acc[j][m], act, relu, pk);
          D[2 * m] = pk[0], D[2 * m + 1] = pk[1];
        }
        transpose_row64(D, lane);
        store_row64<COUT>(D, yrow[j] + mg * 32, n_valid, lane);
      } else {
        uint4 pk[2];
        pack_tile(acc[j][0], act, relu, pk);
        transpose_row32(pk, lane);
        store_row32<COUT>(pk, yrow[j] + mg * 32, n_valid, lane);
      }
    }
  }
}

template <int CIN, int COUT, int NP = 1>
__global__ __launch_bounds__(256, 2) void k_conv3x3_s2(const uint16_t* __restrict__ x, const uint16_t* __restrict__ x2, const uint4* __restrict__ wfrag,
                                                    const uint4* __restrict__ wfrag2, const float* __restrict__ bias,
                                                    const uint8_t* __restrict__ mask, uint16_t* __restrict__ y, int B, int H, int W, int Ho, int Wo,
                                                    int relu, uint8_t* __restrict__ row_dirty, int slot, const uint16_t* __restrict__ x3 = nullptr,
                                                    const uint4* __restrict__ wfrag3 = nullptr) {
  static_assert(CIN % 64 == 0 && (COUT == 128 || COUT == 256), "64-channel input slabs; 4 groups of 32 or of 64 output channels");
  constexpr int TH = S2_TH, MB = COUT / 128, NCG = 4, NRG = 1, NRMAX = TH / NRG;
  constexpr int YS = NP > 1 ? 2 : 1;
  extern __shared__ uint4 s_in[];
  __shared__ uint32_t s_rowmask2[2 * TH];
  __shared__ unsigned int s_next[2];
  const int lane = threadIdx.x & 63, wv = threadIdx.x >> 6;
  const int px = lane & 31, kb = lane >> 5;
  const int rg = wv % NRG, mg = MB * (wv / NRG);
  static_assert(NCG * NRG == 4, "four waves");
  const int tiles_x = (Wo + 31) >> 5, tiles_y = (Ho + TH - 1) / TH;
  const int64_t n_tiles = (int64_t)B * tiles_y * tiles_x;
  int64_t next = 0;
  int it = 0;
  for (int64_t tile = blockIdx.x; tile < n_tiles; tile = next, it++) {
    sched_draw(s_next, it, slot);
    uint32_t* const s_rowmask = s_rowmask2 + (it & 1) * TH;
    const int tx = (int)(tile % tiles_x);
    const int ty = (int)((tile / tiles_x) % tiles_y);
    const int b = (int)(tile / ((int64_t)tiles_x * tiles_y));
    const int x0 = tx * 32, y0 = ty * TH;
    const int ox = x0 + px;
    bool was = true;
    {
      const int oy = y0 + wv;
      const bool a = ox < Wo && oy < Ho && (mask == nullptr || mask[((int64_t)b * Ho + oy) * Wo + ox] != 0);
      if (row_dirty != nullptr && oy < Ho) was = __builtin_amdgcn_readfirstlane((int)row_dirty[((int64_t)b * Ho + oy) * tiles_x + tx]) != 0;
      const uint32_t bal = (uint32_t)__ballot(a);
      if (lane == 0) s_rowmask[wv] = bal;
    }
    __syncthreads();
    next = sched_next(s_next, it, slot, tile);
    const uint32_t my_rm = s_rowmask[lane & 3];
    const uint32_t am = (uint32_t)__ballot(my_rm != 0) & 0xfu;
    {
      const int oy = y0 + wv;
      const bool active = (am >> wv) & 1u;
      if (!active && was && oy < Ho && ox < Wo) {
        uint4* dst = reinterpret_cast<uint4*>(y + (((int64_t)b * Ho + oy) * Wo + ox) * COUT * YS);
#pragma unroll 1
        for (int ch = kb; ch < COUT * YS / 8; ch += 2) dst[ch] = make_uint4(0, 0, 0, 0);
      }
      if (row_dirty != nullptr && oy < Ho && lane == 0 && was != active) row_dirty[((int64_t)b * Ho + oy) * tiles_x + tx] = active ? 1 : 0;
    }
    if (am == 0) continue;
    int nr = 0;
    int rbase[4], rrow[4];
    {
      uint32_t rest = am;
      for (int k = 0; k < rg && rest; k++) rest &= rest - 1;
#pragma unroll
      for (int j = 0; j < 4; j++) {
        const bool has = j < NRMAX && rest != 0;
        rrow[j] = has ? __builtin_ctz(rest) : 0;
        nr += has ? 1 : 0;
        for (int k = 0; k < NRG && rest; k++) rest &= rest - 1;
      }
    }
    nr = __builtin_amdgcn_readfirstlane(nr);
    uint32_t rmask[4];
    uint16_t* yrow[4];
#pragma unroll
    for (int j = 0; j < 4; j++) {
      rrow[j] = __builtin_amdgcn_readfirstlane(rrow[j]);
      rbase[j] = 2 * rrow[j] * S2_RS * 8;
      rmask[j] = j < nr ? __builtin_amdgcn_readfirstlane(s_rowmask[rrow[j]]) : 0u;
      yrow[j] = y + (((int64_t)b * Ho + (y0 + rrow[j])) * Wo + x0) * COUT * YS;
    }
    uint32_t need = 0;
#pragma unroll
    for (int r = 0; r < TH; r++)
      if ((am >> r) & 1u) need |= 7u << (2 * r);
    const int iy0 = 2 * y0 - 1, ix0 = 2 * x0 - 1;
    stage_tile64_s2<CIN>(s_in, NP == 3 ? x3 : x, b, H, W, 0, iy0, ix0, need);
    __syncthreads();
#define PNX_ROWS_S2(N_) conv_rows_s2<(N_ <= NRMAX ? N_ : NRMAX), CIN, COUT, MB, NP>(s_in, x, x2, x3, wfrag, wfrag2, wfrag3, bias, rbase, rmask, yrow, b, H, W, iy0, ix0, Wo - x0, need, mg, relu, px, kb, lane)
    switch (nr) {
      case 0: PNX_ROWS_S2(0); break;
      case 1: PNX_ROWS_S2(1); break;
      case 2: PNX_ROWS_S2(2); break;
      case 3: PNX_ROWS_S2(3); break;
      default: PNX_ROWS_S2(4); break;
    }
#undef PNX_ROWS_S2
  }
  sched_done(slot);
}

template <int CIN, int COUT, int NP>
int launch_s2(PnxPieces<NP> x, PnxPieces<NP> wfrag, const float* bias, const uint8_t* mask, void* y, int B, int H, int W, int Ho, int Wo, int relu,
              uint8_t* row_dirty, hipStream_t st) {
  const int slot = mask != nullptr ? next_sched_slot() : -1;
  int64_t nb = (int64_t)B * ((Ho + S2_TH - 1) / S2_TH) * ((Wo + 31) / 32);
  if (nb > 512) nb = 512;
  constexpr auto kern = k_conv3x3_s2<CIN, COUT, NP>;
  constexpr int lds = S2_NSTAGE * 16;
  if (const int rc = pnx_lds_optin<kern>(lds); rc != PNX_OK) return rc;
  kern<<<(unsigned)nb, 256, lds, st>>>((const uint16_t*)x.hi, (const uint16_t*)x.slot2(), (const uint4*)wfrag.hi, (const uint4*)wfrag.slot2(), bias, mask,
                                       (uint16_t*)y, B, H, W, Ho, Wo, relu, row_dirty, slot, (const uint16_t*)x.slot3(), (const uint4*)wfrag.slot3());
  PNX_LAUNCH_CHECK();
  return PNX_OK;
}
```

pillarnext_amd/csrc/conv_taps.h:

```cpp
#pragma once

#ifdef PNX_CONV_TIMERS
__device__ unsigned long long g_conv_T[8];
#define CT_DECL unsigned long long ct_T[8] = {0, 0, 0, 0, 0, 0, 0, 0}; unsigned long long tk = __builtin_amdgcn_s_memtime();
#define CT_TOCK(k)                                              \
  {                                                             \
    const unsigned long long _n = __builtin_amdgcn_s_memtime(); \
    ct_T[k] += _n - tk;                                         \
    tk = _n;                                                    \
  }
#define CT_FLUSH                                                                     \
  if ((threadIdx.x & 63) == 0) {                                                     \
    for (int k = 0; k < 8; k++) atomicAdd(&g_conv_T[k], ct_T[k]);                     \
  }
#else
#define CT_DECL
#define CT_TOCK(k)
#define CT_FLUSH
#endif

constexpr int LDS_TH = 16;
constexpr int LDS_HW = 34;
constexpr int LDS_NSTAGE = (LDS_TH + 2) * LDS_HW * 8;

__device__ __forceinline__ int lds_swz(int c) { return (c & 7) ^ ((c >> 3) & 1); }

__device__ unsigned int g_tile_ctr[64][2];
__device__ __forceinline__ void sched_draw(unsigned int* s_next, int it, int slot) {
  if (slot >= 0 && threadIdx.x == 0) s_next[it & 1] = atomicAdd(&g_tile_ctr[slot][0], 1u);
}
__device__ __forceinline__ int64_t sched_next(const unsigned int* s_next, int it, int slot, int64_t tile) {
  return slot >= 0 ? (int64_t)s_next[it & 1] + gridDim.x : tile + gridDim.x;
}
__device__ __forceinline__ int64_t sched_next2(const unsigned int* s_next, int it, int slot, int64_t idx_b) {
  return slot >= 0 ? (int64_t)s_next[it & 1] + 2 * (int64_t)gridDim.x : idx_b + gridDim.x;
}
__device__ __forceinline__ int64_t tile_at(const int32_t* __restrict__ tlist, int64_t idx, int64_t n) {
  if (idx >= n) return -1;
  return tlist != nullptr ? (int64_t)tlist[idx] : idx;
}
__device__ __forceinline__ void sched_done(int slot) {
  if (slot >= 0 && threadIdx.x == 0) {
    __threadfence();
    if (atomicAdd(&g_tile_ctr[slot][1], 1u) == gridDim.x - 1) {
      g_tile_ctr[slot][0] = 0;
      g_tile_ctr[slot][1] = 0;
      __threadfence();
    }
  }
}

template <int CSTRIDE, int TH = LDS_TH>
__device__ __forceinline__ void stage_tile64(uint4* __restrict__ s_in, const uint16_t* __restrict__ x, int b, int H, int W, int ch0, int y0, int x0,
                                             uint32_t need) {
  constexpr int NROW = TH + 2, NEXTRA = NROW * 16;
  static_assert(NEXTRA <= 512, "two slots of the extra columns per thread");
  typedef __attribute__((address_space(1))) const void* gptr_t;
  typedef __attribute__((address_space(3))) void* lptr_t;
  const uint16_t* xt = x + (((int64_t)b * H + (y0 - 1)) * W + (x0 - 1)) * CSTRIDE + ch0;
  int tid = threadIdx.x;
  asm volatile("" : "+v"(tid));
  const int slot = tid & 7, col = tid >> 3, wbase = (tid >> 6) * 8;
  uint32_t rows_in = (1u << NROW) - 1u;
  if (y0 == 0) rows_in &= ~1u;
  if (y0 - 1 + NROW > H) rows_in &= (1u << (H - (y0 - 1))) - 1u;
  const bool col_ok = (unsigned)(x0 - 1 + col) < (unsigned)W;
  const uint32_t voff = (uint32_t)(col * CSTRIDE + (slot ^ lds_swz(col)) * 8) * 2u;
#pragma unroll
  for (int r = 0; r < NROW; r++) {
    if (!((need >> r) & 1u)) continue;
    if (((rows_in >> r) & 1u) && col_ok) {
      __builtin_amdgcn_global_load_lds((gptr_t)(reinterpret_cast<const char*>(xt + (int64_t)r * W * CSTRIDE) + voff),
                                       (lptr_t)(s_in + (r * LDS_HW + wbase) * 8), 16, 0, 0);
    } else {
      s_in[(r * LDS_HW + col) * 8 + slot] = make_uint4(0, 0, 0, 0);
    }
  }
#pragma unroll
  for (int part = 0; part < (NEXTRA + 255) / 256; part++) {
    const int e = part * 256 + tid;
    const int re = e >> 4, ce = 32 + ((e >> 3) & 1);
    if (e < NEXTRA && ((need >> re) & 1u)) {
      uint4 qe = make_uint4(0, 0, 0, 0);
      if (((rows_in >> re) & 1u) && (unsigned)(x0 - 1 + ce) < (unsigned)W)
        qe = *reinterpret_cast<const uint4*>(xt + ((int64_t)re * W + ce) * CSTRIDE + (e & 7) * 8);
      s_in[(re * LDS_HW + ce) * 8 + ((e & 7) ^ lds_swz(ce))] = qe;
    }
  }
}

constexpr int S2_RS = 65;
template <int STRIDE>
__device__ __forceinline__ int tap_slot(int px, int dx) {
  return STRIDE == 1 ? px + dx : (dx == 1 ? px : 32 + px + (dx >> 1));
}

constexpr int TAPS_PD = 1;
constexpr int TAPS_WD = 4;
template <int NR, int MTALL, int CB = 4, int STRIDE = 1, int MB = 2, int WD = TAPS_WD, bool PIX = false, int PIXB = 8>
__device__ __forceinline__ void conv_taps(v16f (&acc)[NR][MB], const uint4* __restrict__ s_in, const uint4* __restrict__ wfrag, const int (&rbase)[4],
                                          int mg, int px, int kb, int lane, int kstep0 = 0) {
  constexpr int RS = STRIDE == 1 ? LDS_HW : S2_RS;
  constexpr int KS = 36, PD = TAPS_PD;
  const uint4* wu = wfrag + (int64_t)__builtin_amdgcn_readfirstlane(kstep0 * MTALL + mg) * 64;
  const __amdgpu_buffer_rsrc_t wrs = __builtin_amdgcn_make_buffer_rsrc(const_cast<uint4*>(wu), 0, 0x7fffffff, 0x00020000);
  const int wlo = lane * 16;
  auto wload = [&](int ks, uint4 (&dst)[MB]) {
    const int grp = ks / 3, cbl = grp & 3;
    const int tap = (ks % 3) * 3 + (grp >> 2);
#pragma unroll
    for (int m = 0; m < MB; m++) {
      typedef unsigned int u32x4 __attribute__((ext_vector_type(4)));
      const u32x4 r = __builtin_amdgcn_raw_buffer_load_b128(wrs, wlo, (((tap * CB + cbl) * MTALL + m) * 64) * 16, 0);
      dst[m] = make_uint4(r.x, r.y, r.z, r.w);
    }
  };
  int addr[NR];
  auto group_addr = [&](int grp) {
    const int dx = grp >> 2, cbl = grp & 3;
    if constexpr (PIX && PIXB == 16) {
      int p[2] = {rbase[0], rbase[1]};
      asm volatile("" : "+v"(p[0]));
      if (NR > 2) asm volatile("" : "+v"(p[1]));
#pragma unroll
      for (int j = 0; j < NR; j++) {
        const int q = (p[j >> 1] >> (16 * (j & 1))) & 0xffff;
        const int c = tap_slot<STRIDE>(q & 31, dx);
        addr[j] = (q >> 5) * (RS * 8) + c * 8 + ((2 * cbl + kb) ^ lds_swz(c));
        asm volatile("" : "+v"(addr[j]));
      }
      return;
    } else if constexpr (PIX) {
      int p = rbase[0];
      asm volatile("" : "+v"(p));
#pragma unroll
      for (int j = 0; j < NR; j++) {
        const int q = (p >> (8 * j)) & 255;
        const int c = tap_slot<STRIDE>(q & 31, dx);
        addr[j] = (q >> 5) * (RS * 8) + c * 8 + ((2 * cbl + kb) ^ lds_swz(c));
        asm volatile("" : "+v"(addr[j]));
      }
      return;
    }
    int p = px;
    asm volatile("" : "+v"(p));
    const int c = tap_slot<STRIDE>(p, dx);
    const int a = c * 8 + ((2 * cbl + kb) ^ lds_swz(c));
#pragma unroll
    for (int j = 0; j < NR; j++) addr[j] = a + rbase[j];
  };
  auto bload = [&](int ks, uint4 (&dst)[NR]) {
    const int dy = ks % 3;
    if (dy == 0) group_addr(ks / 3);
#pragma unroll
    for (int j = 0; j < NR; j++) dst[j] = s_in[addr[j] + dy * (RS * 8)];
  };
  uint4 w[WD][MB];
  uint4 q[PD + 1][NR];
#pragma unroll
  for (int k = 0; k < WD; k++) wload(k, w[k]);
#pragma unroll
  for (int k = 0; k < PD; k++) bload(k, q[k]);
#pragma unroll
  for (int ks = 0; ks < KS; ks++) {
    if (ks + PD < KS) bload(ks + PD, q[(ks + PD) % (PD + 1)]);
#pragma unroll
    for (int j = 0; j < NR; j++) {
      const el8 bfr = __builtin_bit_cast(el8, q[ks % (PD + 1)][j]);
// ... 8 lines not shown
```

pillarnext_amd/csrc/conv_tile.h:

```cpp
#pragma once

typedef float v16f __attribute__((ext_vector_type(16)));
typedef float f32x2 __attribute__((ext_vector_type(2)));

#ifdef PNX_CONV_F16
typedef _Float16 el8 __attribute__((ext_vector_type(8)));
typedef _Float16 el2 __attribute__((ext_vector_type(2)));
#define PNX_MFMA32(a, b, c) __builtin_amdgcn_mfma_f32_32x32x16_f16(a, b, c, 0, 0, 0)
#define PNX_MFMA16(a, b, c) __builtin_amdgcn_mfma_f32_16x16x32_f16(a, b, c, 0, 0, 0)
#define PNX_CONV_FN(name) name##_f16
__device__ __forceinline__ uint32_t el_lo_bits(uint32_t w) { return __float_as_uint((float)__builtin_bit_cast(el2, w)[0]); }
__device__ __forceinline__ uint32_t el_hi_bits(uint32_t w) { return __float_as_uint((float)__builtin_bit_cast(el2, w)[1]); }
#else
typedef __bf16 el8 __attribute__((ext_vector_type(8)));
typedef __bf16 el2 __attribute__((ext_vector_type(2)));
#define PNX_MFMA32(a, b, c) __builtin_amdgcn_mfma_f32_32x32x16_bf16(a, b, c, 0, 0, 0)
#define PNX_MFMA16(a, b, c) __builtin_amdgcn_mfma_f32_16x16x32_bf16(a, b, c, 0, 0, 0)
#define PNX_CONV_FN(name) name##_bf16
__device__ __forceinline__ uint32_t el_lo_bits(uint32_t w) { return w << 16; }
__device__ __forceinline__ uint32_t el_hi_bits(uint32_t w) { return w & 0xffff0000u; }
#endif
__device__ __forceinline__ uint32_t pack_el(float lo, float hi) {
  const f32x2 v = {lo, hi};
  return __builtin_bit_cast(uint32_t, __builtin_convertvector(v, el2));
// ... 79 lines not shown
    R[k].w = (uint32_t)__builtin_amdgcn_ds_bpermute(src << 2, (int)R[k].w);
  }
  cswap(T != 0, R[0], R[1]);
}

template <int CSTRIDE>
__device__ __forceinline__ void store_row32(const uint4 (&D)[2], uint16_t* __restrict__ row, int n_valid, int lane) {
  const uint32_t voff = (uint32_t)((lane >> 2) * CSTRIDE + (lane & 3) * 8) * 2u;
#pragma unroll
  for (int d = 0; d < 2; d++) {
    const int P = 16 * d + (lane >> 2);
    if (P < n_valid) *reinterpret_cast<uint4*>(reinterpret_cast<char*>(row) + voff + (uint32_t)(d * 16 * CSTRIDE * 2)) = D[d];
  }
}

template <int COUT>
__device__ __forceinline__ void store_tile_f32(const v16f& a, bool act, float* __restrict__ row, int n_valid, int px, int kb) {
  if (px >= n_valid) return;
  float* p = row + (int64_t)px * COUT + 4 * kb;
#pragma unroll
  for (int g = 0; g < 4; g++) {
    float4 v = make_float4(a[4 * g], a[4 * g + 1], a[4 * g + 2], a[4 * g + 3]);
    if (!act) v = make_float4(0.f, 0.f, 0.f, 0.f);
    *reinterpret_cast<float4*>(p + 8 * g) = v;
  }
}

__device__ __forceinline__ v16f bias_tile(const float* __restrict__ bias, int cbase, int kb) {
  v16f r;
#pragma unroll
  for (int g = 0; g < 4; g++) {
    const float4 q = *reinterpret_cast<const float4*>(bias + cbase + 8 * g + 4 * kb);
    r[4 * g + 0] = q.x, r[4 * g + 1] = q.y, r[4 * g + 2] = q.z, r[4 * g + 3] = q.w;
  }
  return r;
}

__device__ __forceinline__ void load_residual(uint4 (&rq)[2][2], const uint16_t* __restrict__ res_px, bool act, int kb) {
#pragma unroll
  for (int m = 0; m < 2; m++)
#pragma unroll
    for (int t = 0; t < 2; t++) {
      rq[m][t] = make_uint4(0, 0, 0, 0);
      if (act) rq[m][t] = *reinterpret_cast<const uint4*>(res_px + m * 32 + 16 * t + 8 * kb);
    }
}
__device__ __forceinline__ void load_residual_u(uint4 (&rq)[2][2], const uint16_t* __restrict__ row, uint32_t lane_off, bool act) {
#pragma unroll
  for (int m = 0; m < 2; m++)
#pragma unroll
    for (int t = 0; t < 2; t++) {
      rq[m][t] = make_uint4(0, 0, 0, 0);
      if (act) rq[m][t] = *reinterpret_cast<const uint4*>(reinterpret_cast<const char*>(row) + lane_off + (uint32_t)((m * 32 + 16 * t) * 2));
    }
}
__device__ __forceinline__ void add_residual(v16f (&acc2)[2], const uint4 (&rq)[2][2]) {
#pragma unroll
  for (int m = 0; m < 2; m++)
#pragma unroll
    for (int t = 0; t < 2; t++) {
      const uint4 r = rq[m][t];
      const uint32_t lo[4] = {el_lo_bits(r.x), el_hi_bits(r.x), el_lo_bits(r.y), el_hi_bits(r.y)};
      const uint32_t hi[4] = {el_lo_bits(r.z), el_hi_bits(r.z), el_lo_bits(r.w), el_hi_bits(r.w)};
#pragma unroll
      for (int i = 0; i < 4; i++) {
        const u32x2 q = __builtin_amdgcn_permlane32_swap(lo[i], hi[i], false, false);
        acc2[m][8 * t + i] += __uint_as_float(q.x);
        acc2[m][8 * t + 4 + i] += __uint_as_float(q.y);
      }
    }
}

struct ConvArgs {
  const uint16_t* x;
  const uint4* wfrag;
  const float* bias;
  const uint16_t* res;
  const uint8_t* mask;
  uint16_t* y;
  int B, H, W, relu;
  uint8_t* row_dirty;
  const int32_t *tlist, *tcount;
  hipStream_t st;
};
```

pillarnext_amd/csrc/enqueue.hip:

```cpp
#include "pnx_common.h"

extern "C" int pnx_conv_tile_list_prezeroed(const uint8_t* mask, const uint8_t* const* row_dirty, int32_t n_dirty, int32_t batch, int32_t h, int32_t w,
                                            int32_t tile_rows, int32_t* tile_list, int32_t* tile_count, pnx_stream_t stream);

namespace {

__global__ __launch_bounds__(256) void k_lazy_cells(const int64_t* __restrict__ order, const int32_t* __restrict__ seg_len, const int64_t* __restrict__ list_key_off,
                                                    int32_t pre_max, int64_t n, int64_t* __restrict__ local) {
  const int64_t i = (int64_t)blockIdx.x * blockDim.x + threadIdx.x;
  if (i >= n) return;
  const int64_t s = i / pre_max;
  const int32_t j = (int32_t)(i - s * pre_max);
  local[i] = j < seg_len[s] ? order[i] - list_key_off[s] : 0;
}

struct ZeroRanges {
  uint32_t* p[8];
  int64_t end[8];
  int n;
};
__global__ __launch_bounds__(256) void k_zero_ranges(ZeroRanges z) {
  const int64_t total = z.end[z.n - 1];
  for (int64_t i = (int64_t)blockIdx.x * 256 + threadIdx.x; i < total; i += (int64_t)gridDim.x * 256) {
    int r = 0;
    while (i >= z.end[r]) r++;
    z.p[r][i - (r ? z.end[r - 1] : 0)] = 0u;
  }
}
int launch_zero_ranges(ZeroRanges& z, hipStream_t st) {
  if (z.n == 0) return PNX_OK;
  const int64_t total = z.end[z.n - 1];
  int nb = (int)((total + 256 * 8 - 1) / (256 * 8));
  nb = nb < 1 ? 1 : (nb > 2048 ? 2048 : nb);
  k_zero_ranges<<<nb, 256, 0, st>>>(z);
  PNX_LAUNCH_CHECK();
  return PNX_OK;
}
void add_range(ZeroRanges& z, void* p, int64_t words) {
  z.p[z.n] = (uint32_t*)p;
  z.end[z.n] = (z.n ? z.end[z.n - 1] : 0) + words;
  z.n++;
}

int run_op(const pnx_op& o, hipStream_t st) {
  const int32_t* i = o.i;
  const void* const* p = o.p;
  switch (o.kind) {
    case PNX_OP_MASK_POOL3:
      return pnx_mask_pool3((const uint8_t*)p[0], i[0], i[1], i[2], i[3], (uint8_t*)p[1], st);
    case PNX_OP_TILE_LIST:
      PNX_REQUIRE(i[0] >= 0 && i[0] <= 8, PNX_ERR_INVALID, "tile list over %d row_dirty arrays (at most 8)", i[0]);
      return pnx_conv_tile_list_prezeroed((const uint8_t*)p[0], (const uint8_t* const*)&p[3], i[0], i[1], i[2], i[3], i[4], (int32_t*)p[1], (int32_t*)p[2], st);
    case PNX_OP_CONV3X3:
      return (i[7] == PNX_F16 ? pnx_conv3x3_f16 : pnx_conv3x3_bf16)(p[0], p[1], (const float*)p[2], p[3], (const uint8_t*)p[4], (void*)p[5], i[0], i[1], i[2],
                                                                    i[3], i[4], i[5], i[6], (uint8_t*)p[6], (const int32_t*)p[7], (const int32_t*)p[8], st);
    case PNX_OP_DECONV2X2:
      return (i[6] == PNX_F16 ? pnx_deconv2x2_f16 : pnx_deconv2x2_bf16)(p[0], p[1], (const float*)p[2], (void*)p[3], i[0], i[1], i[2], i[3], i[4], i[5], st);
    case PNX_OP_SEPHEAD_OUT:
      return (i[4] == PNX_F16 ? pnx_sephead_out_f16 : pnx_sephead_out_bf16)(p[0], p[1], (const float*)p[2], (void*)p[3], i[0], i[1], i[2], i[3], st);
    default:
      pnx_set_error("unknown op kind %d", o.kind);
      return PNX_ERR_INVALID;
  }
}

}

extern "C" int pnx_enqueue(const pnx_op* ops, int32_t n_ops, pnx_stream_t stream) {
  PNX_REQUIRE(ops != nullptr && n_ops >= 0, PNX_ERR_INVALID, "pnx_enqueue: bad arguments");
  hipStream_t st = (hipStream_t)stream;
  {
    ZeroRanges z;
    z.n = 0;
    for (int32_t k = 0; k < n_ops; k++) {
      if (ops[k].kind != PNX_OP_TILE_LIST) continue;
      if (z.n == 8) {
        const int rc = launch_zero_ranges(z, st);
        if (rc != PNX_OK) return rc;
        z.n = 0;
      }
      add_range(z, const_cast<void*>(ops[k].p[2]), 1);
    }
    const int rc = launch_zero_ranges(z, st);
    if (rc != PNX_OK) return rc;
  }
  for (int32_t k = 0; k < n_ops; k++) {
    const int rc = run_op(ops[k], st);
    if (rc != PNX_OK) {
      char msg[400];
      snprintf(msg, sizeof msg, "%s", pnx_last_error());
      pnx_set_error("pnx_enqueue: entry %d (kind %d): %s", k, ops[k].kind, msg);
      return rc;
    }
  }
  return PNX_OK;
}

extern "C" int pnx_decode_lazy_enqueue(const pnx_lazy_decode* d, pnx_stream_t stream) {
  PNX_REQUIRE(d != nullptr, PNX_ERR_INVALID, "pnx_decode_lazy_enqueue: null descriptor");
  PNX_REQUIRE(d->n_tasks > 0 && d->n_tasks <= 8 && d->n_classes_total > 0 && d->batch > 0 && d->pre_max > 0 && d->post_max > 0, PNX_ERR_INVALID,
              "pnx_decode_lazy_enqueue: bad sizes");
  PNX_REQUIRE(d->dense_host && d->task_descs_host && d->task_descs_dev && d->task_key_off_host && d->task_key_off_dev && d->list_key_off_dev &&
                  d->lazy_tasks_host && d->class_task_host && d->seg_off_dev && d->nms_thresh_dev,
              PNX_ERR_INVALID, "pnx_decode_lazy_enqueue: null table");
  PNX_REQUIRE(d->keys && d->sorted_keys && d->order && d->seg_start && d->seg_len && d->seg_total && d->local && d->cand && d->boxes9 && d->boxes7 &&
                  d->scores && d->flag && d->keep && d->keep_count && d->topk_ws && d->nms_ws && d->out,
              PNX_ERR_INVALID, "pnx_decode_lazy_enqueue: null buffer");
  hipStream_t st = (hipStream_t)stream;
  const int32_t S = d->batch * d->n_classes_total;
  const int64_t n_rows = (int64_t)S * d->pre_max;
  const int64_t n_keys = d->task_key_off_host[d->n_tasks];
  const size_t desc_bytes = pnx_decode_task_desc_bytes();
  int rc;
  for (int32_t t = 0; t < d->n_tasks; t++) {
    rc = pnx_decode_keys(d->dense_host[t], d->dtype, d->batch, d->n_classes_total, (const char*)d->task_descs_host + (size_t)t * desc_bytes,
                         d->keys + d->task_key_off_host[t], st);
    if (rc != PNX_OK) return rc;
  }
  {
    ZeroRanges z;
    z.n = 0;
    add_range(z, d->order, n_rows * 2);
    add_range(z, d->boxes7, n_rows * 7);
    add_range(z, d->flag, 1);
    add_range(z, d->keep_count, S);
    rc = launch_zero_ranges(z, st);
    if (rc != PNX_OK) return rc;
  }
  rc = pnx_decode_topk(d->keys, n_keys, S, d->pre_max, d->sorted_keys, d->order, d->seg_start, d->seg_len, d->seg_total, d->topk_ws, d->topk_ws_bytes, st);
  if (rc != PNX_OK) return rc;
  k_lazy_cells<<<(unsigned)((n_rows + 255) / 256), 256, 0, st>>>(d->order, d->seg_len, d->list_key_off_dev, d->pre_max, n_rows, d->local);
  PNX_LAUNCH_CHECK();
  rc = (d->dtype == PNX_F16 ? pnx_sephead_lazy_f16 : pnx_sephead_lazy_bf16)(d->lazy_tasks_host, d->n_tasks, d->class_task_host, d->n_classes_total, d->batch, d->local, d->seg_len, d->pre_max, d->cand, st);
  if (rc != PNX_OK) return rc;
  rc = pnx_decode_boxes_lazy(d->task_descs_dev, d->task_key_off_dev, d->n_tasks, d->n_classes_total, d->sorted_keys, d->order, d->seg_start, d->seg_len,
                             d->seg_total, S, d->pre_max, d->cand, d->boxes9, d->boxes7, d->scores, d->flag, st);
  if (rc != PNX_OK) return rc;
  rc = pnx_nms_rotated_batched(d->boxes7, d->seg_off_dev, d->seg_len, S, d->pre_max, d->nms_thresh_dev, d->post_max, d->keep, d->keep_count, d->nms_ws,
// ... 13 lines not shown
```

pillarnext_amd/models.py:

```python
import copy
import inspect
import os
import weakref

import numpy as np

import torch
import torch.nn.functional as F
from torch import nn

from . import ops
from .plan import Dyn, LaunchPlan


def _spconv_weight_to_conv2d(w, conv):
    want = tuple(conv.weight.shape)
    co, ci, kh, kw = want
    layout = getattr(conv, "assume_layout", None)
    if layout == "dense":
        if tuple(w.shape) != want:
            raise RuntimeError(f"dense-layout checkpoint holds {tuple(w.shape)} for Conv2d {want}")
        return w
    if layout == "spconv":
        if tuple(w.shape) != (co, kh, kw, ci):
# ... 883 lines not shown
    def validation_step(self, example):
        preds = self._forward(example)
        outputs = self.head.predict(example, preds, self.post_processing)
        detections = {}
        for output in outputs:
            token = output["token"]
            for k, v in output.items():
                if k != "token":
                    output[k] = v.to(torch.device("cpu"))
            detections[token] = output
        return detections


NUSC_TASKS = [["car"], ["truck", "construction_vehicle"], ["bus", "trailer"], ["barrier"], ["motorcycle", "bicycle"], ["pedestrian", "traffic_cone"]]


def build_pillarnext_b(pc_range, voxel_size, tasks=None, num_point_features=5, ds_layer_strides=(1, 2, 2, 2), with_iou_head=False,
                       rectifier=None, post_processing=None):
    from .reader import PillarFeatureNet

    tasks = tasks or NUSC_TASKS
    common = {"reg": (2, 2), "height": (1, 2), "dim": (3, 2), "rot": (2, 2), "vel": (2, 2)}
    if with_iou_head:
        common["iou"] = (1, 2)
    reader = PillarFeatureNet(num_point_features, [64, 64], list(voxel_size), list(pc_range))
    backbone = SparseResNet([2, 2, 2, 2], list(ds_layer_strides), [64, 128, 256, 256], 64)
    neck = ASPPNeck(256)
    rect = rectifier or [[0.5] * len(t) for t in tasks]
    head = CenterHead(256, tasks, 0.25, [1.0] * 6 + [0.2, 0.2, 1.0, 1.0], common, [2] * len(tasks), with_reg_iou=True,
                      voxel_size=list(voxel_size), pc_range=list(pc_range), out_size_factor=[4] * len(tasks), rectifier=rect)
    if post_processing is None:
        post_processing = dict(post_center_limit_range=[-61.2, -61.2, -10.0, 61.2, 61.2, 10.0], score_threshold=0.1,
                               nms=dict(nms_pre_max_size=1000, nms_post_max_size=83, nms_iou_threshold=[[0.2] * len(t) for t in tasks]),
                               out_size_factor=[4] * len(tasks), voxel_size=list(voxel_size), pc_range=list(pc_range))
    return SingleStageDetector(reader, backbone, neck, head, post_processing)


def _fold_bn(weight, bn, conv_bias=None, transposed=False):
    w = weight.detach().float()
    a = bn.weight.detach().float() * torch.rsqrt(bn.running_var.detach().float() + bn.eps)
    shape = (1, -1, 1, 1) if transposed else (-1, 1, 1, 1)
    b0 = conv_bias.detach().float() if conv_bias is not None else torch.zeros_like(a)
    return w * a.view(shape), (b0 - bn.running_mean.detach().float()) * a + bn.bias.detach().float()


def fold_aspp(nk):
    wp, bp = _fold_bn(nk.post_conv.conv.conv.weight, nk.post_conv.norm)
    C = nk.weight.shape[0]
    P = wp.detach().float().reshape(wp.shape[0], 6, C)
    w1 = nk.conv1x1.weight.detach().float().reshape(C, C)
    ws = nk.weight.detach().float()
    wds = [torch.einsum("om,mikl->oikl", P[:, 2 + k], ws) for k in range(4)]
    wds[0][:, :, 1, 1] += P[:, 0] + P[:, 1] @ w1
    return wds, bp.float()


class _FusedConv(nn.Module):

    def __init__(self, weight, bias, stride=1, padding=0, dilation=1, relu=True, transposed=False, dtype=torch.bfloat16):
        super().__init__()
        self.register_buffer("weight", weight.to(dtype).contiguous(memory_format=torch.channels_last) if weight.dim() == 4 else weight.to(dtype))
        self.register_buffer("bias", bias.float().contiguous())
        self.stride, self.padding, self.dilation, self.relu, self.transposed = stride, padding, dilation, relu, transposed

    def forward(self, x, mask=None, residual=None, post_residual=None):
        if self.transposed:
            y = F.conv_transpose2d(x, self.weight, None, self.stride, self.padding)
        else:
            y = F.conv2d(x, self.weight, None, self.stride, self.padding, self.dilation)
        if not y.is_contiguous(memory_format=torch.channels_last):
            y = y.contiguous(memory_format=torch.channels_last)
        if post_residual is not None:
            return ops.bias_act_mask_(y, self.bias, mask, post_residual, 2 if self.relu else 0)
        return ops.bias_act_mask_(y, self.bias, mask, residual, self.relu)


class _HipConv3x3(nn.Module):

    def __init__(self, weight, bias, stride=1, dtype=torch.bfloat16):
        super().__init__()
        self.cout, self.cin, self.stride = weight.shape[0], weight.shape[1], int(stride)
        self.register_buffer("wfrag", ops.conv3x3_pack_weights(weight, dtype=dtype))
        self.register_buffer("bias", bias.float().contiguous())
    def forward(self, x, mask=None, residual=None, out=None, tiles=None, plan=None):
        call = ops.conv3x3_masked if plan is None else plan.conv3x3
        return call(x, self.wfrag, self.bias, self.cout, self.stride, mask, residual, True, out=out, tiles=tiles if self.stride == 1 else None)


class _HipDeconv2x2(nn.Module):

    def __init__(self, weight, bias, relu=True, dtype=torch.bfloat16):
        super().__init__()
        self.cout, self.relu = weight.shape[1], relu
        self.register_buffer("wfrag", ops.deconv2x2_pack_weights(weight, dtype=dtype))
        self.register_buffer("bias", bias.float().contiguous())

    def forward(self, x, mask=None, residual=None, out=None, plan=None):
        if plan is None:
            return ops.deconv2x2(x, self.wfrag, self.bias, self.cout, self.relu)
        return plan.deconv2x2(x, self.wfrag, self.bias, self.cout, out, self.relu)


class _HipSepHeadOut(nn.Module):

    def __init__(self, weight, bias, dtype=torch.bfloat16):
        super().__init__()
        self.cout = weight.shape[0]
        self.register_buffer("wfrag", ops.sephead_pack_weights(weight, dtype=dtype))
        self.register_buffer("bias", bias.float().contiguous())

    def forward(self, x, mask=None, residual=None, out=None, plan=None):
        if plan is None:
            return ops.sephead_out(x, self.wfrag, self.bias)
        return plan.sephead_out(x, self.wfrag, self.bias, out)


def _backbone_conv(weight, bias, stride, padding, dtype, hip_conv):
    co, ci, kh, kw = weight.shape
    shapes = ops.CONV3X3_SHAPES_S1 if stride == 1 else ops.CONV3X3_SHAPES_S2
    if hip_conv and dtype in ops._HALF and (kh, kw) == (3, 3) and padding == 1 and (ci, co) in shapes and stride in (1, 2):
        return _HipConv3x3(weight, bias, stride, dtype=dtype)
    return _FusedConv(weight, bias, stride, padding, dtype=dtype)


class LazyTask:

    def __init__(self, dense, up):
        self.dense, self.up = dense, up


class _DeferredDecode:

    def __init__(self, model, packed, tokens):
        self.model, self.packed, self.tokens = model, packed, tokens
        self.head_done = torch.cuda.Event()
        self.head_done.record()
        self.launched, self.pend = False, None

    def launch(self, behind_reader=False):
        if self.launched:
            return
        self.launched = True
        m = self.model
        main = torch.cuda.current_stream()
        side = m.__dict__.get("_decode_stream")
        if side is None or side.device != main.device:
            side = m.__dict__["_decode_stream"] = torch.cuda.Stream(device=main.device)
        side.wait_event(self.head_done)
        if behind_reader:
            ev = torch.cuda.Event()
            ev.record(main)
            side.wait_event(ev)
        with torch.cuda.stream(side):
            self.pend = m.launch_decode(self.packed, self.tokens)
        for p in self.packed:
            p.dense.record_stream(side), p.up.record_stream(side)
        self.packed = None
        ref = m.__dict__.get("_deferred")
        if ref is not None and ref() is self:
            m.__dict__["_deferred"] = None

    def result(self):
        self.launch()
        return self.pend.result()

    def __getattr__(self, name):
        if name in ("pend", "launched", "packed", "model", "tokens", "head_done"):
            raise AttributeError(name)
        self.launch()
# ... 116 lines not shown
                o = 0
                for j in range(5):
                    w2 = w2s[j]
                    for pos in range(9):
                        w2m[pos * 5 * hc + j * hc: pos * 5 * hc + (j + 1) * hc, o:o + outs[j]] = w2[:, :, pos // 3, pos % 3].t()
                    b2z[o:o + outs[j]] = b2s[j]
                    o += outs[j]
                self.register_buffer(f"lazy_w1_{ti}", w1m.to(dtype).contiguous())
                self.register_buffer(f"lazy_b1_{ti}", torch.cat(b1s[:5]).float().contiguous())
                self.register_buffer(f"lazy_w2_{ti}", w2m.to(dtype).float().contiguous())
                self.register_buffer(f"lazy_b2_{ti}", b2z)
                self.register_buffer(f"lazy_wf1_{ti}", ops.conv3x3_pack_weights(W1z, dtype=dtype))
                self.register_buffer(f"lazy_w2c_{ti}", ops.sephead_lazy_pack_w2(getattr(self, f"lazy_w2_{ti}")))
            else:
                self.lazy_conv1.append(nn.Identity())
                self.lazy_conv2.append(nn.Identity())
        self.lazy_head = self.lazy_head and all(self._lazy_ok)

    @torch.no_grad()
    def forward_preds(self, points, batch_size, marks=None, packed_out=None, taps=None, lazy=None, after_reader=None):
        def mark(name):
            if marks is not None:
                e = torch.cuda.Event(enable_timing=True)
                e.record()
                marks.append((name, e))

        mark("start")
        planned = marks is None and taps is None and self._plan_ok()
        if planned:
            bb = self._backbone_plan(batch_size, points.device)
            canvas, occ = bb["canvas"], bb["occ"]
        else:
            ny, nx = (int(v) for v in self.reader.grid_size)
            canvas, occ = None, torch.empty((batch_size, ny, nx), dtype=torch.uint8, device=points.device)
        x = self.reader.forward_dense(points, batch_size, dtype=self.dtype, out=canvas, occupancy=occ)
        if after_reader is not None:
            after_reader()
        mark("reader")
        if planned:
            bb["plan"].run()
            x, mask = bb["out"], bb["mask"]
        else:
            x, mask = self._backbone(x, occ, mark=mark, taps=taps)
        x = self.mapping(x, mask)
        x = self.pre2(self.pre1(x), post_residual=x)
        parts = [F.conv2d(x, getattr(self, f"aspp_w{k}"), None, 1, d, d) for k, d in enumerate((1, 6, 12, 18))]
        parts = [p if p.is_contiguous(memory_format=torch.channels_last) else p.contiguous(memory_format=torch.channels_last) for p in parts]
        x = ops.sum_bias_act(parts, self.aspp_bias, relu=True)
        mark("mapping+neck")
        if taps is not None:
            taps["neck"] = x
        lazy = packed_out is not None and self.lazy_head and (lazy is None or lazy)
        if planned and lazy and self._head_plan_ok():
            packed_out.extend(self._run_head_plan(x))
            return []
        preds = []
        for (t, up), (names, outs_n) in zip(self._head(x, lazy), self.task_split):
            if lazy:
                packed_out.append(LazyTask(t, up))
            elif packed_out is not None:
                packed_out.append(t)
            else:
                d, o = {}, 0
                for nme, k in zip(names, outs_n):
                    d[nme] = t[:, o:o + k]
                    o += k
                preds.append(d)
        mark("head")
        return preds

    def _backbone(self, x, mask, plan=None, mark=lambda name: None, taps=None):
        for si, (mods, (stride, subm)) in enumerate(zip(self.stages, self.stage_meta)):
            if not subm:
                mask = ops.mask_pool3(mask, stride) if plan is None else plan.mask_pool3(mask, ops.mask_pool3_out(mask, stride), stride)
            ws, k = self._stage_workspace(si, mods, mask), 0
            tiles = self._stage_tiles(si, mods, mask, ws, plan)

            def run(m, inp, res=None):
                nonlocal k
                if ws is None or not isinstance(m, _HipConv3x3):
                    assert plan is None
                    return m(inp, mask, residual=res)
                k += 1
                return m(inp, mask, residual=res, out=ws[(k - 1) % 3], tiles=tiles, plan=plan)

            x = run(mods[0], x)
            for j in range(1, len(mods), 2):
                y = run(mods[j], x)
                x = run(mods[j + 1], y, x)
            mark(f"backbone.stage{si}")
            if taps is not None:
                taps[f"stage{si}"] = x
        return x, mask

    def _head(self, x, lazy, plan=None):
        c1s, c2s = (self.lazy_conv1, self.lazy_conv2) if lazy else (self.task_conv1, self.task_conv2)

        def run(m, inp, out):
            return m(inp) if plan is None else m(inp, out=out, plan=plan)

        o_sh, outs = None, [(None, None, None)] * len(c1s)
        if plan is not None:
            def new(c, s):
                return torch.empty((x.shape[0], c, s * x.shape[2], s * x.shape[3]), dtype=self.dtype, device=x.device, memory_format=torch.channels_last)

            o_sh, mids = (new(self.shared.cout, 1), None), {c1.cout: new(c1.cout, 2) for c1 in c1s}
            outs = [(Dyn(f"up{ti}", new(64, 2)), (mids[c1.cout], None), Dyn(f"dense{ti}", new(16, 2))) for ti, c1 in enumerate(c1s)]
            x = Dyn("x", x)
        sh = run(self.shared, x, o_sh)
        for db, c1, c2, (o_up, o_mid, o_map) in zip(self.task_deblock, c1s, c2s, outs):
            up = run(db, sh, o_up)
            yield run(c2, run(c1, up, o_mid), o_map), up

    def _plan_ok(self):
        return (self.use_plan and self.sparse_ws and self.tile_lists and self.dtype in ops._HALF and not self.reader.training
                and self.reader._fused_supported() and all(isinstance(m, _HipConv3x3) for mods in self.stages for m in mods))

    def _head_plan_ok(self):
        return isinstance(self.shared, _HipConv3x3) and all(isinstance(d, _HipDeconv2x2) for d in self.task_deblock)

    def _backbone_plan(self, B, dev):
        key = ("plan_bb", B, dev)
        st = self._ws.get(key)
        wkey = tuple(t.data_ptr() for mods in self.stages for m in mods for t in (m.wfrag, m.bias))
        if st is not None and st["weights_at"] == wkey:
            return st
        ny, nx = (int(v) for v in self.reader.grid_size)
        canvas = torch.empty((B, 64, ny, nx), dtype=self.dtype, device=dev, memory_format=torch.channels_last)
        occ = torch.empty((B, ny, nx), dtype=torch.uint8, device=dev)
        plan = LaunchPlan()
        x, mask = self._backbone(canvas, occ, plan)
        st = self._ws[key] = {"canvas": canvas, "occ": occ, "plan": plan.freeze(), "out": x, "mask": mask, "weights_at": wkey}
        return st

    def _head_plan(self, x):
        key = ("plan_head", *x.shape[:1], *x.shape[2:], x.device, self.shared.wfrag.data_ptr())
        if key not in self._ws:
            plan = LaunchPlan()
            list(self._head(x, True, plan))
            self._ws[key] = plan.freeze()
        return self._ws[key]

    def _run_head_plan(self, x):
        st = self._head_plan(x)
        B, _, H, W = x.shape
        st.bind("x", x)
        tasks = []
        for ti in range(len(self.task_deblock)):
            up, dense = (torch.empty((B, c, 2 * H, 2 * W), dtype=self.dtype, device=x.device, memory_format=torch.channels_last) for c in (64, 16))
            st.bind(f"up{ti}", up)
            st.bind(f"dense{ti}", dense)
            tasks.append(LazyTask(dense, up))
        st.run()
        return tasks

    def _stage_workspace(self, si, mods, mask):
        if not self.sparse_ws or not any(isinstance(m, _HipConv3x3) for m in mods):
            return None
        B, H, W = mask.shape
        key = (si, B, H, W, mask.device)
        if key not in self._ws:
            cout = next(m.cout for m in mods if isinstance(m, _HipConv3x3))
            self._ws[key] = [ops.conv3x3_workspace(B, cout, H, W, mask.device, self.dtype) for _ in range(3)]
        return self._ws[key]

    def _stage_tiles(self, si, mods, mask, ws, plan=None):
        if ws is None or not self.tile_lists:
# ... 110 lines not shown
```

pillarnext_amd/ops.py:

```python
import ctypes

import torch

from . import _lib
from ._lib import PNX_BF16, PNX_F16, PNX_F32, PNX_NCHW, PNX_NHWC, PnxError, check, lib, ptr, stream_ptr

_DT = {torch.float32: PNX_F32, torch.bfloat16: PNX_BF16, torch.float16: PNX_F16}


def _need_cuda(t, name):
    if not t.is_cuda:
        raise PnxError(f"{name} must be a CUDA (ROCm) tensor; the PillarNeXt hot path has no CPU implementation")
    if not t.is_contiguous():
        raise PnxError(f"{name} must be contiguous")


class Workspace:

    def __init__(self):
        self.buf = None

    def get(self, nbytes, device):
        if self.buf is None or self.buf.numel() < nbytes or self.buf.device != device:
            self.buf = torch.empty(int(nbytes * 1.25) + 256, dtype=torch.uint8, device=device)
# ... 532 lines not shown
    name = "pnx_conv3x3_wgrad_" + _PIECES_TAG[len(xs)]
    check(getattr(lib(), name)(*map(ptr, xs), *map(ptr, gs), ptr(mask), ptr(dw), B, H, W, ci, co, stride, ptr(ws), ws.numel(), stream_ptr()), name)
    return dw


def conv3x3_dgrad_s2(g, wfrag_t, cin, in_hw, mask_in):
    gs, ws = _pieces(g), _pieces(wfrag_t)
    if len(gs) not in _PIECES_TAG:
        raise PnxError("conv3x3_dgrad_s2: g must be one bf16 tensor or a tuple of 2 or 3 pieces")
    _bf16_maps(gs, "conv3x3_dgrad_s2")
    _bf16_packs(ws, len(gs), "conv3x3_dgrad_s2")
    H, W = in_hw
    B, co, Ho, Wo = gs[0].shape
    if (Ho, Wo) != ((H - 1) // 2 + 1, (W - 1) // 2 + 1) or tuple(mask_in.shape) != (B, H, W) or mask_in.dtype != torch.uint8 or not mask_in.is_contiguous():
        raise PnxError("conv3x3_dgrad_s2: g (B,cout,Ho,Wo) with Ho = (H - 1) // 2 + 1 and a contiguous uint8 (B,H,W) mask of the input sites")
    dx = torch.empty((B, cin, H, W), dtype=torch.bfloat16 if len(gs) == 1 else torch.float32, device=gs[0].device, memory_format=torch.channels_last)
    name = "pnx_conv3x3_dgrad_s2_" + _PIECES_TAG[len(gs)]
    check(getattr(lib(), name)(*map(ptr, gs), *map(ptr, ws), ptr(mask_in), ptr(dx), B, H, W, cin, co, stream_ptr()), name)
    return dx


def _smallk_check(x, what):
    if not (x.is_cuda and x.dim() == 4 and x.dtype in (torch.float32, torch.bfloat16) and x.is_contiguous(memory_format=torch.channels_last)):
        raise PnxError(f"{what} must be a channels_last fp32 / bf16 CUDA tensor")


def conv3x3_smallk(x, weight, bias=None):
    _smallk_check(x, "conv3x3_smallk: x")
    k = weight.shape[0]
    if not (weight.is_cuda and weight.dtype == torch.float32 and tuple(weight.shape[1:]) == (64, 3, 3) and weight.is_contiguous() and 1 <= k <= 4
            and x.shape[1] == 64 and (bias is None or (bias.is_cuda and bias.dtype == torch.float32 and bias.numel() == k and bias.is_contiguous()))):
        raise PnxError("conv3x3_smallk: weight must be a contiguous fp32 (k,64,3,3) with k <= 4, bias fp32 (k)")
    B, _, H, W = x.shape
    y = torch.empty((B, k, H, W), dtype=x.dtype, device=x.device, memory_format=torch.channels_last)
    if k == 1:
        y = torch.empty((B, H, W, 1), dtype=x.dtype, device=x.device).permute(0, 3, 1, 2)
    check(lib().pnx_conv3x3_smallk(ptr(x), ptr(weight), ptr(bias), ptr(y), B, H, W, 64, k, 0 if x.dtype == torch.float32 else 1, stream_ptr()), "pnx_conv3x3_smallk")
    return y


def conv3x3_smallk_wgrad(x, dy, want_bias=True):
    _smallk_check(x, "conv3x3_smallk_wgrad: x")
    B, c, H, W = x.shape
    k = dy.shape[1]
    if not (c == 64 and 1 <= k <= 4 and dy.is_cuda and dy.dtype == x.dtype and tuple(dy.shape) == (B, k, H, W)):
        raise PnxError("conv3x3_smallk_wgrad: x (B,64,H,W), dy (B,k,H,W) of the same dtype, k <= 4")
    dyc = dy.permute(0, 2, 3, 1).contiguous()
    nbytes = int(lib().pnx_conv3x3_smallk_wgrad_workspace_bytes(k))
    ws = _wgrad_workspace(nbytes, x.device)
    dw = torch.empty((k, 64, 3, 3), dtype=torch.float32, device=x.device)
    db = torch.empty((k,), dtype=torch.float32, device=x.device) if want_bias else None
    check(lib().pnx_conv3x3_smallk_wgrad(ptr(x), ptr(dyc), ptr(dw), ptr(db), B, H, W, 64, k, 0 if x.dtype == torch.float32 else 1, ptr(ws), ws.numel(), stream_ptr()),
          "pnx_conv3x3_smallk_wgrad")
    return dw, db


def conv3x3_workspace(batch, cout, ho, wo, device, dtype=torch.bfloat16):
    y = torch.zeros((batch, cout, ho, wo), dtype=dtype, device=device).contiguous(memory_format=torch.channels_last)
    return y, torch.zeros((batch, ho, (wo + 31) // 32), dtype=torch.uint8, device=device)


def conv_tile_rows(cin, cout, stride=1):
    return int(lib().pnx_conv3x3_tile_rows(cin, cout, stride))


def conv_tile_buffers(mask, tile_rows, out=None):
    B, H, W = _like(mask).shape
    n_tiles = B * ((H + tile_rows - 1) // tile_rows) * ((W + 31) // 32)
    if out is None:
        return torch.empty((n_tiles,), dtype=torch.int32, device=mask.device), torch.zeros((1,), dtype=torch.int32, device=mask.device)
    if out[0].numel() < n_tiles or out[0].dtype != torch.int32 or out[1].dtype != torch.int32:
        raise PnxError("conv_tile_list: needs an int32 list of >= n_tiles entries + an int32 count")
    return out


def conv_tile_list(mask, dirties, tile_rows, out=None):
    B, H, W = mask.shape
    out = conv_tile_buffers(mask, tile_rows, out)
    arr = (ctypes.c_void_p * max(len(dirties), 1))(*[d.data_ptr() for d in dirties])
    check(lib().pnx_conv_tile_list(ptr(mask), arr, len(dirties), B, H, W, tile_rows, ptr(out[0]), ptr(out[1]), stream_ptr()), "pnx_conv_tile_list")
    return out


def _conv3x3_dims(x, wfrag, cout, stride, mask, residual, out, cuda=False):
    xs = _half_nhwc(x, "conv3x3", cuda=cuda)
    if wfrag.dtype != xs.dtype or (residual is not None and _like(residual).dtype != xs.dtype):
        raise PnxError("conv3x3: weights / residual of another dtype than the input")
    B, ci, H, W = xs.shape
    Ho, Wo = _out_hw(H, W, stride)
    if out is not None:
        y, dirty = out
        if (tuple(_half_nhwc(y, "conv3x3 output", xs.dtype).shape) != (B, cout, Ho, Wo)
                or (dirty is not None and (mask is None or tuple(dirty.shape) != (B, Ho, (Wo + 31) // 32)))):
            raise PnxError("conv3x3: output / workspace of the wrong shape (a workspace needs a mask)")
    return B, H, W, ci, _DT[xs.dtype], Ho, Wo


def conv3x3_masked(x, wfrag, bias, cout, stride=1, mask=None, residual=None, relu=True, out=None, tiles=None):
    B, H, W, ci, _, Ho, Wo = _conv3x3_dims(x, wfrag, cout, stride, mask, residual, out, cuda=True)
    y, dirty = out if out is not None else (torch.empty((B, cout, Ho, Wo), dtype=x.dtype, device=x.device, memory_format=torch.channels_last), None)
    tl, tc = tiles if tiles is not None else (None, None)
    check(_conv_fn("conv3x3", x.dtype)(ptr(x), ptr(wfrag), ptr(bias), ptr(residual), ptr(mask), ptr(y), B, H, W, ci, cout, stride, 1 if relu else 0,
                                       ptr(dirty), ptr(tl), ptr(tc), stream_ptr()), "pnx_conv3x3")
    return y


def _i3(v):
    return (ctypes.c_int32 * 3)(*[int(a) for a in v])


class Sp3Index:

    def __init__(self, batch, grid, device):
        self.batch, self.grid = int(batch), tuple(int(g) for g in grid)
        self.nbytes = lib().pnx_sp3_index_bytes(self.batch, _i3(self.grid))
        if self.nbytes == 0:
            raise PnxError(f"sparse3d: bad grid {self.batch} x {self.grid}")
        self.buf = torch.empty((self.nbytes,), dtype=torch.uint8, device=device)


def _need_coords(coords):
    _need_cuda(coords, "coords")
    if coords.dtype != torch.int32 or coords.dim() != 2 or coords.shape[1] != 4:
        raise PnxError("coords must be (N, 4) int32 [b, z, y, x]")


def sp3_out_grid(batch, grid, kernel, stride, pad):
    out = _i3((0, 0, 0))
    check(lib().pnx_sp3_out_grid(int(batch), _i3(grid), _i3(kernel), _i3(stride), _i3(pad), out), "pnx_sp3_out_grid")
    return tuple(out)


def sp3_index_build(coords, batch, grid, want_rows=False):
    _need_coords(coords)
    ix = Sp3Index(batch, grid, coords.device)
    n = coords.shape[0]
    rows = torch.full((max(n, 1),), -1, dtype=torch.int32, device=coords.device) if want_rows else None
    count = torch.zeros((1,), dtype=torch.int32, device=coords.device)
    check(lib().pnx_sp3_index_build(ptr(coords), n, ix.batch, _i3(ix.grid), ptr(ix.buf), ix.nbytes, ptr(rows), ptr(count), stream_ptr()),
          "pnx_sp3_index_build")
    return ix, (rows[:n] if want_rows else None), count


def sp3_out_index(coords_in, batch, grid_in, kernel, stride, pad):
    _need_coords(coords_in)
    ix = Sp3Index(batch, sp3_out_grid(batch, grid_in, kernel, stride, pad), coords_in.device)
    count = torch.zeros((1,), dtype=torch.int32, device=coords_in.device)
    check(lib().pnx_sp3_out_index(ptr(coords_in), coords_in.shape[0], ix.batch, _i3(grid_in), _i3(kernel), _i3(stride), _i3(pad), ptr(ix.buf), ix.nbytes,
                                  ptr(count), stream_ptr()), "pnx_sp3_out_index")
    return ix, count


def sp3_index_coords(ix, n):
    coords = torch.empty((max(int(n), 1), 4), dtype=torch.int32, device=ix.buf.device)
    check(lib().pnx_sp3_index_coords(ptr(ix.buf), ix.nbytes, ix.batch, _i3(ix.grid), ptr(coords), int(n), stream_ptr()), "pnx_sp3_index_coords")
    return coords[: int(n)]


def sp3_neighbor_map(coords_out, ix_in, row_of_rank, kernel, stride, pad):
    _need_coords(coords_out)
    T = int(kernel[0]) * int(kernel[1]) * int(kernel[2])
    m = torch.empty((coords_out.shape[0], T), dtype=torch.int32, device=coords_out.device)
    check(lib().pnx_sp3_neighbor_map(ptr(coords_out), coords_out.shape[0], ptr(ix_in.buf), ix_in.nbytes, ix_in.batch, _i3(ix_in.grid), ptr(row_of_rank),
                                     _i3(kernel), _i3(stride), _i3(pad), ptr(m), stream_ptr()), "pnx_sp3_neighbor_map")
    return m


def sp3_pack_weight(w):
    co, ci = w.shape[0], w.shape[-1]
    T = w.shape[1] * w.shape[2] * w.shape[3]
    n = lib().pnx_sp3_packed_weight_floats(T, ci, co)
    ci4, co16 = (ci + 3) // 4 * 4, (co + 15) // 16 * 16
    if n != T * ci4 * co16:
        raise PnxError(f"sp3_pack_weight: no packing for {tuple(w.shape)}")
    wp = torch.zeros((T, ci4, co16), dtype=torch.float32, device=w.device)
    wp[:, :ci, :co] = w.float().reshape(co, T, ci).permute(1, 2, 0)
    return wp


def sp3_conv(x, nbmap, w_packed, shift, cout, residual=None, relu=True, per_tap=False):
    for t, name in ((x, "x"), (nbmap, "nbmap"), (w_packed, "w_packed"), (shift, "shift")):
        _need_cuda(t, name)
    if x.dtype != torch.float32 or w_packed.dtype != torch.float32 or shift.dtype != torch.float32 or nbmap.dtype != torch.int32:
        raise PnxError("sp3_conv: fp32 features, weights and shift, int32 map")
    n_out, T = nbmap.shape
    ci = x.shape[1]
# ... 286 lines not shown
```

pillarnext_amd/plan.py:

```python
import ctypes

from . import ops
from ._lib import PnxError, check, lib, stream_ptr

OP_MASK_POOL3, OP_TILE_LIST, OP_CONV3X3, OP_DECONV2X2, OP_SEPHEAD_OUT = 1, 2, 3, 4, 5


class PnxOp(ctypes.Structure):
    _fields_ = [("kind", ctypes.c_int32), ("i", ctypes.c_int32 * 9), ("p", ctypes.c_void_p * 11)]


assert ctypes.sizeof(PnxOp) == 128, "pnx_op layout drifted (include/pnx.h)"


class Dyn:

    def __init__(self, name, like):
        self.name, self.like = name, like


class LaunchPlan:
    def __init__(self):
        self._ops, self._keep, self._dyn, self._arr = [], [], {}, None

    def __len__(self):
        return len(self._ops)

    def _add(self, kind, ints, ptrs):
        if self._arr is not None:
            raise PnxError("the plan is frozen")
        op = PnxOp()
        op.kind = kind
        for k, v in enumerate(ints):
            op.i[k] = int(v)
        for k, a in enumerate(ptrs):
            if isinstance(a, Dyn):
                meta = (a.like.shape, a.like.dtype, a.like.stride(), a.like.device)
                self._dyn.setdefault(a.name, (meta, []))[1].append((len(self._ops), k))
                op.p[k] = a.like.data_ptr()
            elif a is not None:
                op.p[k] = a.data_ptr()
                self._keep.append(a)
        self._ops.append(op)

    def mask_pool3(self, mask_in, mask_out, stride):
        self._add(OP_MASK_POOL3, [*ops._like(mask_in).shape, stride], [mask_in, ops.mask_pool3_out(mask_in, stride, mask_out)])
        return mask_out

    def tile_list(self, mask, dirties, tile_rows, out):
        if len(dirties) > 8:
            raise PnxError("tile_list: an entry has room for 8 row_dirty arrays")
        tl, tc = ops.conv_tile_buffers(mask, tile_rows, out)
        self._add(OP_TILE_LIST, [len(dirties), *ops._like(mask).shape, tile_rows], [mask, tl, tc] + list(dirties))
        return out

    def conv3x3(self, x, wfrag, bias, cout, stride=1, mask=None, residual=None, relu=True, out=None, tiles=None):
        B, H, W, ci, dt, _, _ = ops._conv3x3_dims(x, wfrag, cout, stride, mask, residual, out)
        tl, tc = tiles if tiles is not None else (None, None)
        self._add(OP_CONV3X3, [B, H, W, ci, cout, stride, 1 if relu else 0, dt], [x, wfrag, bias, residual, mask, *out, tl, tc])
        return out[0]

    def deconv2x2(self, x, wfrag, bias, cout, y, relu=True):
        B, H, W, ci, dt = ops._conv_dims("deconv2x2", x, wfrag, y, cout, 2)
        self._add(OP_DECONV2X2, [B, H, W, ci, cout, 1 if relu else 0, dt], [x, wfrag, bias, y])
        return y

    def sephead_out(self, x, wfrag, bias, y):
        B, H, W, ci, dt = ops._conv_dims("sephead_out", x, wfrag, y, 16, 1)
        self._add(OP_SEPHEAD_OUT, [B, H, W, ci // 64, dt], [x, wfrag, bias, y])
        return y

    def freeze(self):
        self._arr = (PnxOp * max(len(self._ops), 1))(*self._ops)
        self._bound = {}
        return self

    def bind(self, name, t):
        if self._arr is None:
            self.freeze()
        meta, where = self._dyn[name]
        if (t.shape, t.dtype, t.stride(), t.device) != meta:
            raise PnxError(f"plan: tensor bound to '{name}' differs from the one the plan was built for")
        a = t.data_ptr()
        for k, j in where:
            self._arr[k].p[j] = a
        self._bound[name] = t

    def run(self):
        if self._arr is None:
            self.freeze()
        missing = set(self._dyn) - set(self._bound)
        if missing:
            raise PnxError(f"plan: dynamic tensors never bound: {sorted(missing)}")
        if not all(a.is_cuda for a in self._keep) or not all(t.is_cuda for t in self._bound.values()):
            raise PnxError("plan: every tensor of a launch table must live on the GPU")
        check(lib().pnx_enqueue(self._arr, len(self._ops), stream_ptr()), "pnx_enqueue")
```

Baseline: 761.6.

## Skip global loads of inactive input sites in sparse 3x3 conv via input mask

Adds an input-site mask (x_mask) path to the LDS-staged 3x3 conv kernels. Each tile's mask window is prefetched into LDS, and the tile is staged from global memory only at active input sites; inactive ones read from a zero line. This targets memory bandwidth wasted loading empty pillars. The cost is extra mask fetch, LDS use and sync per tile. The path is enabled by default for stride-1 stages after the first when a plan is used.

```diff
diff --git a/include/pnx.h b/include/pnx.h
--- a/include/pnx.h
+++ b/include/pnx.h
@@ -121,6 +121,12 @@
 int pnx_conv3x3_f16(const void* x, const void* wfrag, const float* bias, const void* residual, const uint8_t* mask, void* y, int32_t batch,
                     int32_t h, int32_t w, int32_t cin, int32_t cout, int32_t stride, int32_t relu, uint8_t* row_dirty, const int32_t* tile_list,
                     const int32_t* tile_count, pnx_stream_t stream);
+int pnx_conv3x3_xm_bf16(const void* x, const void* wfrag, const float* bias, const void* residual, const uint8_t* mask, const uint8_t* x_mask, void* y,
+                        int32_t batch, int32_t h, int32_t w, int32_t cin, int32_t cout, int32_t stride, int32_t relu, uint8_t* row_dirty,
+                        const int32_t* tile_list, const int32_t* tile_count, pnx_stream_t stream);
+int pnx_conv3x3_xm_f16(const void* x, const void* wfrag, const float* bias, const void* residual, const uint8_t* mask, const uint8_t* x_mask, void* y,
+                       int32_t batch, int32_t h, int32_t w, int32_t cin, int32_t cout, int32_t stride, int32_t relu, uint8_t* row_dirty,
+                       const int32_t* tile_list, const int32_t* tile_count, pnx_stream_t stream);
 size_t pnx_conv3x3_wgrad_workspace_bytes(int32_t cin, int32_t cout);
 int pnx_conv3x3_wgrad_bf16(const void* x, const void* dy, const uint8_t* mask, float* dw, int32_t batch, int32_t h, int32_t w, int32_t cin, int32_t cout,
                            int32_t stride, void* workspace, size_t workspace_bytes, pnx_stream_t stream);
diff --git a/pillarnext_amd/_lib.py b/pillarnext_amd/_lib.py
--- a/pillarnext_amd/_lib.py
+++ b/pillarnext_amd/_lib.py
@@ -94,6 +94,8 @@
     "pnx_sephead_lazy_f16": (ctypes.c_int, [_vp, _i32, _vp, _i32, _i32, _vp, _vp, _i32, _vp, _vp]),
     "pnx_conv3x3_bf16": (ctypes.c_int, [_vp, _vp, _vp, _vp, _vp, _vp, _i32, _i32, _i32, _i32, _i32, _i32, _i32, _vp, _vp, _vp, _vp]),
     "pnx_conv3x3_f16": (ctypes.c_int, [_vp, _vp, _vp, _vp, _vp, _vp, _i32, _i32, _i32, _i32, _i32, _i32, _i32, _vp, _vp, _vp, _vp]),
+    "pnx_conv3x3_xm_bf16": (ctypes.c_int, [_vp, _vp, _vp, _vp, _vp, _vp, _vp, _i32, _i32, _i32, _i32, _i32, _i32, _i32, _vp, _vp, _vp, _vp]),
+    "pnx_conv3x3_xm_f16": (ctypes.c_int, [_vp, _vp, _vp, _vp, _vp, _vp, _vp, _i32, _i32, _i32, _i32, _i32, _i32, _i32, _vp, _vp, _vp, _vp]),
     "pnx_conv3x3_tile_rows": (ctypes.c_int, [_i32, _i32, _i32]),
     "pnx_conv3x3_pack_weights": (ctypes.c_int, [_vp, _i32, _i32, _i32, _i32, _vp, _vp]),
     "pnx_conv3x3_wgrad_workspace_bytes": (_sz, [_i32, _i32]),
diff --git a/pillarnext_amd/csrc/conv3x3.hip b/pillarnext_amd/csrc/conv3x3.hip
--- a/pillarnext_amd/csrc/conv3x3.hip
+++ b/pillarnext_amd/csrc/conv3x3.hip
@@ -305,9 +305,9 @@
 
 #endif
 
-int PNX_CONV_FN(pnx_conv3x3)(const void* x, const void* wfrag, const float* bias, const void* residual, const uint8_t* mask, void* y, int32_t batch,
-                     int32_t h, int32_t w, int32_t cin, int32_t cout, int32_t stride, int32_t relu, uint8_t* row_dirty, const int32_t* tile_list,
-                     const int32_t* tile_count, pnx_stream_t stream) {
+int PNX_CONV_FN(pnx_conv3x3_xm)(const void* x, const void* wfrag, const float* bias, const void* residual, const uint8_t* mask, const uint8_t* x_mask, void* y,
+                        int32_t batch, int32_t h, int32_t w, int32_t cin, int32_t cout, int32_t stride, int32_t relu, uint8_t* row_dirty,
+                        const int32_t* tile_list, const int32_t* tile_count, pnx_stream_t stream) {
   PNX_REQUIRE((tile_list == nullptr) == (tile_count == nullptr), PNX_ERR_INVALID, "tile_list and tile_count come together");
   PNX_REQUIRE(tile_list == nullptr || (mask != nullptr && pnx_conv3x3_tile_rows(cin, cout, stride) > 0), PNX_ERR_INVALID,
               "a tile list needs a mask and a kernel that takes one (pnx_conv3x3_tile_rows)");
@@ -318,8 +318,9 @@
               "16-byte alignment required");
   const int ho = (h + 2 - 3) / stride + 1, wo = (w + 2 - 3) / stride + 1;
   hipStream_t st = (hipStream_t)stream;
+  static const int xmask_mode = getenv("PNX_CONV_XMASK") != nullptr ? atoi(getenv("PNX_CONV_XMASK")) : 1;
   const ConvArgs a = {(const uint16_t*)x, (const uint4*)wfrag, bias, (const uint16_t*)residual, mask, (uint16_t*)y, batch, h, w, relu, row_dirty, tile_list,
-                      tile_count, st};
+                      tile_count, st, x_mask};
   if (stride == 1 && getenv("PNX_CONV_DIRECT") == nullptr) {
     static const int pc_mode = getenv("PNX_CONV_PC") != nullptr ? atoi(getenv("PNX_CONV_PC")) : 1;
     static const int pack_mode = getenv("PNX_CONV_PACK") != nullptr ? atoi(getenv("PNX_CONV_PACK")) : 3;
@@ -336,18 +337,19 @@
       }
     }
     if (cin == 64 && cout == 64) return launch_lds<64>(a);
-    const bool pack = (pack_mode & 1) != 0;
-    if (cin == 128 && cout == 128) return launch_ldsx<128, 128>(a, pack);
+    const bool pack = (pack_mode & 1) != 0, xm = (xmask_mode & 1) != 0;
+    if (cin == 128 && cout == 128) return launch_ldsx<128, 128>(a, pack, xm);
     if (cin == 256 && cout == 64) return launch_ldsx<256, 64>(a);
-    if (cin == 256 && cout == 256) return launch_ldsx<256, 256>(a, pack);
+    if (cin == 256 && cout == 256) return launch_ldsx<256, 256>(a, pack, xm);
     if (cin == 64 && cout == 384) return launch_lds<384>(a);
     if (cin == 64 && cout == 320) return launch_lds<320>(a);
     if (cin == 64 && cout == 448) return launch_lds<448>(a);
   }
   if (stride == 2 && residual == nullptr && getenv("PNX_CONV_DIRECT") == nullptr) {
-    if (cin == 64 && cout == 128) return launch_s2<64, 128, 1>(x, wfrag, bias, mask, y, batch, h, w, ho, wo, relu, row_dirty, st);
-    if (cin == 128 && cout == 256) return launch_s2<128, 256, 1>(x, wfrag, bias, mask, y, batch, h, w, ho, wo, relu, row_dirty, st);
-    if (cin == 256 && cout == 256) return launch_s2<256, 256, 1>(x, wfrag, bias, mask, y, batch, h, w, ho, wo, relu, row_dirty, st);
+    const uint8_t* const xm = (xmask_mode & 2) != 0 ? x_mask : nullptr;
+    if (cin == 64 && cout == 128) return launch_s2<64, 128, 1>(x, wfrag, bias, mask, y, batch, h, w, ho, wo, relu, row_dirty, st, xm);
+    if (cin == 128 && cout == 256) return launch_s2<128, 256, 1>(x, wfrag, bias, mask, y, batch, h, w, ho, wo, relu, row_dirty, st, xm);
+    if (cin == 256 && cout == 256) return launch_s2<256, 256, 1>(x, wfrag, bias, mask, y, batch, h, w, ho, wo, relu, row_dirty, st, xm);
   }
 #define PNX_CONV_CASE(CI, CO)                             \
   if (cin == CI && cout == CO) {                          \
@@ -360,6 +362,12 @@
 #undef PNX_CONV_CASE
   pnx_set_error("pnx_conv3x3: no kernel for %d -> %d channels", cin, cout);
   return PNX_ERR_UNSUPPORTED;
+}
+
+int PNX_CONV_FN(pnx_conv3x3)(const void* x, const void* wfrag, const float* bias, const void* residual, const uint8_t* mask, void* y, int32_t batch,
+                     int32_t h, int32_t w, int32_t cin, int32_t cout, int32_t stride, int32_t relu, uint8_t* row_dirty, const int32_t* tile_list,
+                     const int32_t* tile_count, pnx_stream_t stream) {
+  return PNX_CONV_FN(pnx_conv3x3_xm)(x, wfrag, bias, residual, mask, nullptr, y, batch, h, w, cin, cout, stride, relu, row_dirty, tile_list, tile_count, stream);
 }
 
 #ifndef PNX_CONV_F16
diff --git a/pillarnext_amd/csrc/conv_rows.h b/pillarnext_amd/csrc/conv_rows.h
--- a/pillarnext_amd/csrc/conv_rows.h
+++ b/pillarnext_amd/csrc/conv_rows.h
@@ -176,11 +176,12 @@
 }
 
 constexpr int LDSX_RES_WD = 2;
-template <int NR, int CIN, int COUT, bool HAS_RES>
+template <int NR, int CIN, int COUT, bool HAS_RES, bool XM = false>
 __device__ __forceinline__ void conv_rows_x(uint4* __restrict__ s_in, const uint16_t* __restrict__ x, const uint4* __restrict__ wfrag,
                                             const float* __restrict__ bias, const uint16_t* __restrict__ res, const int (&rrow)[4],
                                             const int (&rbase)[4], const uint32_t (&rmask)[4], uint16_t* const (&yrow)[4], int b, int H, int W,
-                                            int y0, int x0, uint32_t need, int mg0, int relu, int px, int kb, int lane, int hsel) {
+                                            int y0, int x0, uint32_t need, int mg0, int relu, int px, int kb, int lane, int hsel,
+                                            const uint4* __restrict__ xm CT_PARAMS) {
   constexpr int NS = CIN / 64, NRA = NR > 0 ? NR : 1;
   const int ox = x0 + px;
   {
@@ -206,11 +207,15 @@
     for (int sl = 0; sl < NS; sl++) {
       if (sl) {
         __syncthreads();
-        stage_tile64<CIN, L128_TH>(s_in, x, b, H, W, 64 * sl, y0, x0, need);
+        CT_TOCK(5)
+        stage_tile64<CIN, L128_TH, XM>(s_in, x, b, H, W, 64 * sl, y0, x0, need, xm);
+        CT_TOCK(1)
         __syncthreads();
+        CT_TOCK(2)
       }
       if (NR > 0 && HAS_RES && sl == NS - 1) load_residual_u(rq, rres[0], res_off, rmask[0] >> px & 1u);
       if (NR > 0) conv_taps<NRA, COUT / 32, CIN / 16, 1, 2, HAS_RES ? LDSX_RES_WD : TAPS_WD>(acc, s_in, wfrag, rbase, mg, px, kb, lane, 4 * sl);
+      CT_TOCK(3)
     }
     if (NR > 0) {
       const int n_valid = W - x0;
@@ -236,6 +241,7 @@
         store_row64<COUT>(D, yrow[j] + mg * 32, n_valid, lane);
       }
     }
+    CT_TOCK(4)
   }
 }
 
@@ -255,11 +261,11 @@
   }
 }
 
-template <int NR, int CIN, int COUT, bool HAS_RES>
+template <int NR, int CIN, int COUT, bool HAS_RES, bool XM = false>
 __device__ __forceinline__ void conv_pix_x(uint4* __restrict__ s_in, const uint16_t* __restrict__ x, const uint4* __restrict__ wfrag,
                                            const float* __restrict__ bias, const uint16_t* __restrict__ rtile, int codes, const int (&n_g)[4],
                                            uint16_t* __restrict__ ytile, int b, int H, int W, int y0, int x0, uint32_t need, int mg0, int relu, int px,
-                                           int kb, int lane, int hsel) {
+                                           int kb, int lane, int hsel, const uint4* __restrict__ xm CT_PARAMS) {
   constexpr int NS = CIN / 64, NRA = NR > 0 ? NR : 1;
   const int mg = mg0 + 4 * hsel;
   v16f acc[NRA][2];
@@ -280,11 +286,15 @@
   for (int sl = 0; sl < NS; sl++) {
     if (sl) {
       __syncthreads();
-      stage_tile64<CIN, L128_TH>(s_in, x, b, H, W, 64 * sl, y0, x0, need);
+      CT_TOCK(5)
+      stage_tile64<CIN, L128_TH, XM>(s_in, x, b, H, W, 64 * sl, y0, x0, need, xm);
+      CT_TOCK(1)
       __syncthreads();
+      CT_TOCK(2)
     }
     if (NR > 0 && HAS_RES && sl == NS - 1) load_residual_u(rq, rres, res_off(0), px < n_g[0]);
     if (NR > 0) conv_taps<NRA, COUT / 32, CIN / 16, 1, 2, HAS_RES ? LDSX_RES_WD : TAPS_WD, true>(acc, s_in, wfrag, cw, mg, px, kb, lane, 4 * sl);
+    CT_TOCK(3)
   }
   if (NR > 0) {
 #pragma unroll
@@ -309,21 +319,25 @@
       store_pix64<COUT>(D, ytile + mg * 32, code(j), n_g[j], W, lane);
     }
   }
-}
-
-template <int CIN, int COUT, bool HAS_RES, bool PACK = false>
+  CT_TOCK(4)
+}
+
+template <int CIN, int COUT, bool HAS_RES, bool PACK = false, bool XM = false>
 __global__ __launch_bounds__(256, 2) void k_conv3x3_ldsx(const uint16_t* __restrict__ x, const uint4* __restrict__ wfrag,
                                                       const float* __restrict__ bias, const uint16_t* __restrict__ res,
                                                       const uint8_t* __restrict__ mask, uint16_t* __restrict__ y, int B, int H, int W,
                                                       int relu, uint8_t* __restrict__ row_dirty, int slot, const int32_t* __restrict__ tlist,
-                                                      const int32_t* __restrict__ tcount) {
+                                                      const int32_t* __restrict__ tcount, const uint8_t* __restrict__ xmask = nullptr) {
   static_assert(CIN % 64 == 0 && (COUT % 128 == 0 || COUT == 64), "64-channel input slabs, 128-channel output passes (or one of 64)");
   constexpr int TH = L128_TH, HW_ = LDS_HW;
   constexpr int NRG = COUT == 64 ? 4 : 2, NRMAX = TH / NRG;
   static_assert(!PACK || (CIN == COUT && NRG == 2), "the packed-pixel form serves 128 -> 128 and 256 -> 256");
+  static_assert(TH + 2 <= 4 * XM_ROWS_PER_WAVE, "xmask_load covers the halo rows");
   __shared__ uint4 s_in[L128_NSTAGE];
   __shared__ uint16_t s_list[PACK ? TH * 32 : 1];
   __shared__ uint32_t s_rowmask2[2 * TH];
+  __shared__ uint4 s_xm2[XM ? 2 * HW_ : 1];
+  __shared__ uint32_t s_xraw[XM ? 4 * XM_ROWS_PER_WAVE * HW_ : 1];
   __shared__ unsigned int s_next[2];
   const int lane = threadIdx.x & 63, wv = threadIdx.x >> 6;
   const int px = lane & 31, kb = lane >> 5;
@@ -353,13 +367,23 @@
       if (row_dirty != nullptr && oy < H) wz[j] = (int)row_dirty[((int64_t)b * H + oy) * tiles_x + tx];
     }
   };
+  auto load_xmask = [&](int t) {
+    if (!XM || t < 0) return;
+    const int tx = (int)(t % tiles_x);
+    const int ty = (int)((t / tiles_x) % tiles_y);
+    const int b = (int)(t / ((int64_t)tiles_x * tiles_y));
+    const int wvu = __builtin_amdgcn_readfirstlane(wv);
+    xmask_fetch(s_xraw + wvu * XM_ROWS_PER_WAVE * HW_, xmask, b, H, W, ty * TH - 1, tx * 32 - 1, TH + 2, wvu, threadIdx.x & 63);
+  };
   int64_t idxB = (int64_t)blockIdx.x + gridDim.x, idxC = 0;
   int tileA = unit_at(blockIdx.x), tileB = unit_at(idxB), tileC = -1;
   bool aP[2], aN[2];
   int wasP[2], wasN[2];
   load_mask(tileA >= 0 ? tileA / NH : -1, aP, wasP);
+  load_xmask(tileA >= 0 ? tileA / NH : -1);
 #pragma unroll
   for (int j = 0; j < 2; j++) aN[j] = false, wasN[j] = 1;
+  CT_DECL
   int it = 0;
   for (; tileA >= 0; tileA = tileB, tileB = tileC, idxB = idxC, it++) {
     const int unit = __builtin_amdgcn_readfirstlane(tileA);
@@ -380,12 +404,20 @@
       bal[j] = (uint32_t)__ballot(aP[j]);
       if (lane == 0) s_rowmask[wv * 2 + j] = bal[j];
     }
+    const uint4* const s_xm = s_xm2 + (XM ? (it & 1) * HW_ : 0);
+    if constexpr (XM) {
+      __builtin_amdgcn_s_waitcnt(0x0f70);
+      const int wvu = __builtin_amdgcn_readfirstlane(wv);
+      if (lane < HW_) reinterpret_cast<uint32_t*>(s_xm2)[((it & 1) * HW_ + lane) * 4 + wvu] = xmask_word_raw(s_xraw + wvu * XM_ROWS_PER_WAVE * HW_, wvu, lane);
+    }
     __syncthreads();
     idxC = sched_next2(s_next, it, slot, idxB);
     tileC = unit_at(idxC);
     load_mask(tileB >= 0 ? tileB / NH : -1, aN, wasN);
+    load_xmask(tileB >= 0 ? tileB / NH : -1);
 #pragma unroll
     for (int j = 0; j < 2; j++) aP[j] = aN[j], wasP[j] = wasN[j];
+    CT_TOCK(0)
     const uint32_t my_rm = s_rowmask[lane & 7];
     const uint32_t am = (uint32_t)__ballot(my_rm != 0) & 0xffu;
 #pragma unroll
@@ -418,8 +450,11 @@
       const int n_grp = (n_px + 31) >> 5, rgu = __builtin_amdgcn_readfirstlane(rg);
       const int nr = n_grp > rgu ? (n_grp - rgu + 1) >> 1 : 0;
       const uint32_t need = am | (am << 1) | (am << 2);
-      stage_tile64<CIN, TH>(s_in, x, b, H, W, 0, y0, x0, need);
+      CT_TOCK(0)
+      stage_tile64<CIN, TH, XM>(s_in, x, b, H, W, 0, y0, x0, need, s_xm);
+      CT_TOCK(1)
       __syncthreads();
+      CT_TOCK(2)
       int codes = 0, n_g[4];
 #pragma unroll
       for (int j = 0; j < 4; j++) {
@@ -428,7 +463,7 @@
         if (j < nr && px < n_g[j]) codes |= (int)s_list[32 * g + px] << (8 * j);
       }
       const int64_t t0 = (((int64_t)b * H + y0) * W + x0) * COUT;
-#define PNX_PIX_X(N_) conv_pix_x<N_, CIN, COUT, HAS_RES>(s_in, x, wfrag, bias, HAS_RES ? res + t0 : nullptr, codes, n_g, y + t0, b, H, W, y0, x0, need, mg0, relu, px, kb, lane, hsel)
+#define PNX_PIX_X(N_) conv_pix_x<N_, CIN, COUT, HAS_RES, XM>(s_in, x, wfrag, bias, HAS_RES ? res + t0 : nullptr, codes, n_g, y + t0, b, H, W, y0, x0, need, mg0, relu, px, kb, lane, hsel, s_xm CT_ARGS)
       switch (nr) {
         case 0: PNX_PIX_X(0); break;
         case 1: PNX_PIX_X(1); break;
@@ -453,6 +488,7 @@
           if ((idle >> p) & 1u) *reinterpret_cast<uint4*>(row + (uint32_t)(p * COUT * 2 + (l & 15) * 16)) = make_uint4(0, 0, 0, 0);
         }
       }
+      CT_TOCK(4)
       continue;
     }
     int nr = 0;
@@ -479,9 +515,12 @@
       yrow[j] = y + (((int64_t)b * H + (y0 + rrow[j])) * W + x0) * COUT;
     }
     const uint32_t need = am | (am << 1) | (am << 2);
-    stage_tile64<CIN, TH>(s_in, x, b, H, W, 0, y0, x0, need);
+    CT_TOCK(0)
+    stage_tile64<CIN, TH, XM>(s_in, x, b, H, W, 0, y0, x0, need, s_xm);
+    CT_TOCK(1)
     __syncthreads();
-#define PNX_ROWS_X(N_) conv_rows_x<(N_ <= NRMAX ? N_ : NRMAX), CIN, COUT, HAS_RES>(s_in, x, wfrag, bias, res, rrow, rbase, rmask, yrow, b, H, W, y0, x0, need, mg0, relu, px, kb, lane, hsel)
+    CT_TOCK(2)
+#define PNX_ROWS_X(N_) conv_rows_x<(N_ <= NRMAX ? N_ : NRMAX), CIN, COUT, HAS_RES, XM>(s_in, x, wfrag, bias, res, rrow, rbase, rmask, yrow, b, H, W, y0, x0, need, mg0, relu, px, kb, lane, hsel, s_xm CT_ARGS)
     switch (nr) {
       case 0: PNX_ROWS_X(0); break;
       case 1: PNX_ROWS_X(1); break;
@@ -492,14 +531,27 @@
 #undef PNX_ROWS_X
   }
   sched_done(slot);
+  CT_FLUSH
 }
 
 template <int CIN, int COUT>
-int launch_ldsx(const ConvArgs& a, bool pack = false) {
+int launch_ldsx(const ConvArgs& a, bool pack = false, bool xm = false) {
   const int slot = a.mask != nullptr ? next_sched_slot() : -1;
   int64_t nb = (int64_t)a.B * ((a.H + L128_TH - 1) / L128_TH) * ((a.W + 31) / 32) * ((COUT + 127) / 128);
   if (nb > 512) nb = 512;
   if constexpr (CIN == COUT) {
+    if (xm && a.mask != nullptr && a.xmask != nullptr) {
+#define PNX_LDSX_XM(RES_, PACK_) \
+  k_conv3x3_ldsx<CIN, COUT, RES_, PACK_, true><<<(unsigned)nb, 256, 0, a.st>>>(a.x, a.wfrag, a.bias, a.res, a.mask, a.y, a.B, a.H, a.W, a.relu, a.row_dirty, slot, a.tlist, a.tcount, a.xmask)
+      if (pack) {
+        if (a.res != nullptr) PNX_LDSX_XM(true, true); else PNX_LDSX_XM(false, true);
+      } else {
+        if (a.res != nullptr) PNX_LDSX_XM(true, false); else PNX_LDSX_XM(false, false);
+      }
+#undef PNX_LDSX_XM
+      PNX_LAUNCH_CHECK();
+      return PNX_OK;
+    }
     if (pack && a.mask != nullptr) {
       if (a.res != nullptr)
         k_conv3x3_ldsx<CIN, COUT, true, true><<<(unsigned)nb, 256, 0, a.st>>>(a.x, a.wfrag, a.bias, a.res, a.mask, a.y, a.B, a.H, a.W, a.relu, a.row_dirty, slot,
diff --git a/pillarnext_amd/csrc/conv_s2.h b/pillarnext_amd/csrc/conv_s2.h
--- a/pillarnext_amd/csrc/conv_s2.h
+++ b/pillarnext_amd/csrc/conv_s2.h
@@ -4,9 +4,9 @@
 constexpr int S2_ROWS = 2 * S2_TH + 1;
 constexpr int S2_NSTAGE = S2_ROWS * S2_RS * 8;
 
-template <int CSTRIDE>
+template <int CSTRIDE, bool XM = false>
 __device__ __forceinline__ void stage_tile64_s2(uint4* __restrict__ s_in, const uint16_t* __restrict__ x, int b, int H, int W, int ch0, int iy0,
-                                                int ix0, uint32_t need) {
+                                                int ix0, uint32_t need, const uint4* __restrict__ xm = nullptr) {
   typedef __attribute__((address_space(1))) const void* gptr_t;
   typedef __attribute__((address_space(3))) void* lptr_t;
   int tid = threadIdx.x;
@@ -19,11 +19,17 @@
     const int ix = ix0 + 2 * col + (1 - pl);
     const bool col_ok = (unsigned)ix < (unsigned)W;
     const int chunk = slot ^ lds_swz(ls);
+    uint32_t cm = 0;
+    if constexpr (XM) cm = xmask_col(xm, 2 * col + (1 - pl));
 #pragma unroll
     for (int r = 0; r < S2_ROWS; r++) {
       if (!((need >> r) & 1u)) continue;
       const int iy = iy0 + r;
-      if ((unsigned)iy < (unsigned)H && col_ok) {
+      if constexpr (XM) {
+        const uint16_t* const src = xb + ((int64_t)iy * W + ix) * CSTRIDE + chunk * 8;
+        __builtin_amdgcn_global_load_lds((gptr_t)(((cm >> r) & 1u) ? reinterpret_cast<const char*>(src) : reinterpret_cast<const char*>(g_zero_line) + slot * 16),
+                                         (lptr_t)(s_in + (r * S2_RS + pl * 32 + wbase) * 8), 16, 0, 0);
+      } else if ((unsigned)iy < (unsigned)H && col_ok) {
         __builtin_amdgcn_global_load_lds((gptr_t)(xb + ((int64_t)iy * W + ix) * CSTRIDE + chunk * 8),
                                          (lptr_t)(s_in + (r * S2_RS + pl * 32 + wbase) * 8), 16, 0, 0);
       } else {
@@ -36,18 +42,20 @@
     if ((need >> re) & 1u) {
       const int iy = iy0 + re, ix = ix0 + 64;
       uint4 qe = make_uint4(0, 0, 0, 0);
-      if ((unsigned)iy < (unsigned)H && (unsigned)ix < (unsigned)W) qe = *reinterpret_cast<const uint4*>(xb + ((int64_t)iy * W + ix) * CSTRIDE + ce * 8);
+      bool ld = (unsigned)iy < (unsigned)H && (unsigned)ix < (unsigned)W;
+      if constexpr (XM) ld = ((xmask_col(xm, 64) >> re) & 1u) != 0;
+      if (ld) qe = *reinterpret_cast<const uint4*>(xb + ((int64_t)iy * W + ix) * CSTRIDE + ce * 8);
       s_in[(re * S2_RS + 64) * 8 + (ce ^ lds_swz(64))] = qe;
     }
   }
 }
 
-template <int NR, int CIN, int COUT, int MB, int NP = 1>
+template <int NR, int CIN, int COUT, int MB, int NP = 1, bool XM = false>
 __device__ __forceinline__ void conv_rows_s2(uint4* __restrict__ s_in, const uint16_t* __restrict__ x, const uint16_t* __restrict__ x2,
                                              const uint16_t* __restrict__ x3, const uint4* __restrict__ wfrag, const uint4* __restrict__ wfrag2,
                                              const uint4* __restrict__ wfrag3, const float* __restrict__ bias, const int (&rbase)[4], const uint32_t (&rmask)[4],
                                              uint16_t* const (&yrow)[4], int b, int H, int W, int iy0, int ix0, int n_valid, uint32_t need, int mg,
-                                             int relu, int px, int kb, int lane) {
+                                             int relu, int px, int kb, int lane, const uint4* __restrict__ xm CT_PARAMS) {
   constexpr int NS = CIN / 64, NRA = NR > 0 ? NR : 1;
   constexpr bool X3 = NP == 2, F32 = NP > 1;
   v16f acc[NRA][MB];
@@ -70,10 +78,13 @@
     const int sl = F32 ? sq % NS : sq;
     if (sq) {
       __syncthreads();
+      CT_TOCK(5)
       const uint16_t* xs = X3 && sq >= NS ? x2 : x;
       if constexpr (NP == 3) xs = sq < NS ? x3 : sq < 2 * NS ? x2 : x;
-      stage_tile64_s2<CIN>(s_in, xs, b, H, W, 64 * sl, iy0, ix0, need);
+      stage_tile64_s2<CIN, XM>(s_in, xs, b, H, W, 64 * sl, iy0, ix0, need, xm);
+      CT_TOCK(1)
       __syncthreads();
+      CT_TOCK(2)
     }
     if (NR > 0) {
       if constexpr (NP == 3) {
@@ -88,6 +99,7 @@
         }
       }
     }
+    CT_TOCK(3)
   }
   if (NR > 0) {
 #pragma unroll
@@ -114,19 +126,23 @@
       }
     }
   }
-}
-
-template <int CIN, int COUT, int NP = 1>
+  CT_TOCK(4)
+}
+
+template <int CIN, int COUT, int NP = 1, bool XM = false>
 __global__ __launch_bounds__(256, 2) void k_conv3x3_s2(const uint16_t* __restrict__ x, const uint16_t* __restrict__ x2, const uint4* __restrict__ wfrag,
                                                     const uint4* __restrict__ wfrag2, const float* __restrict__ bias,
                                                     const uint8_t* __restrict__ mask, uint16_t* __restrict__ y, int B, int H, int W, int Ho, int Wo,
                                                     int relu, uint8_t* __restrict__ row_dirty, int slot, const uint16_t* __restrict__ x3 = nullptr,
-                                                    const uint4* __restrict__ wfrag3 = nullptr) {
+                                                    const uint4* __restrict__ wfrag3 = nullptr, const uint8_t* __restrict__ xmask = nullptr) {
   static_assert(CIN % 64 == 0 && (COUT == 128 || COUT == 256), "64-channel input slabs; 4 groups of 32 or of 64 output channels");
+  static_assert(!XM || NP == 1, "x_mask serves the bf16 / fp16 inference entry only");
+  static_assert(S2_ROWS <= 4 * XM_ROWS_PER_WAVE, "xmask_load covers the halo rows");
   constexpr int TH = S2_TH, MB = COUT / 128, NCG = 4, NRG = 1, NRMAX = TH / NRG;
   constexpr int YS = NP > 1 ? 2 : 1;
   extern __shared__ uint4 s_in[];
   __shared__ uint32_t s_rowmask2[2 * TH];
+  __shared__ uint4 s_xm2[XM ? 2 * S2_RS : 1];
   __shared__ unsigned int s_next[2];
   const int lane = threadIdx.x & 63, wv = threadIdx.x >> 6;
   const int px = lane & 31, kb = lane >> 5;
@@ -135,6 +151,7 @@
   const int tiles_x = (Wo + 31) >> 5, tiles_y = (Ho + TH - 1) / TH;
   const int64_t n_tiles = (int64_t)B * tiles_y * tiles_x;
   int64_t next = 0;
+  CT_DECL
   int it = 0;
   for (int64_t tile = blockIdx.x; tile < n_tiles; tile = next, it++) {
     sched_draw(s_next, it, slot);
@@ -144,6 +161,13 @@
     const int b = (int)(tile / ((int64_t)tiles_x * tiles_y));
     const int x0 = tx * 32, y0 = ty * TH;
     const int ox = x0 + px;
+    const uint4* const s_xm = s_xm2 + (XM ? (it & 1) * S2_RS : 0);
+    uint8_t xh[XM_ROWS_PER_WAVE], xh64 = 0;
+    if constexpr (XM) {
+      xmask_load(xmask, b, H, W, 2 * y0 - 1, 2 * x0 - 1, S2_ROWS, 64, wv, lane, xh);
+      const int iy = 2 * y0 - 1 + lane, ix = 2 * x0 - 1 + 64;
+      if (wv == 1 && lane < S2_ROWS && (unsigned)iy < (unsigned)H && (unsigned)ix < (unsigned)W) xh64 = xmask[((int64_t)b * H + iy) * W + ix];
+    }
     bool was = true;
     {
       const int oy = y0 + wv;
@@ -152,7 +176,15 @@
       const uint32_t bal = (uint32_t)__ballot(a);
       if (lane == 0) s_rowmask[wv] = bal;
     }
+    if constexpr (XM) {
+      reinterpret_cast<uint32_t*>(s_xm2)[((it & 1) * S2_RS + lane) * 4 + wv] = xmask_word(xh, wv);
+      if (wv == 1) {
+        const uint32_t b64 = (uint32_t)__ballot(xh64 != 0);
+        if (lane == 0) s_xm2[(it & 1) * S2_RS + 64] = make_uint4(b64, 0, 0, 0);
+      }
+    }
     __syncthreads();
+    CT_TOCK(0)
     next = sched_next(s_next, it, slot, tile);
     const uint32_t my_rm = s_rowmask[lane & 3];
     const uint32_t am = (uint32_t)__ballot(my_rm != 0) & 0xfu;
@@ -195,9 +227,12 @@
     for (int r = 0; r < TH; r++)
       if ((am >> r) & 1u) need |= 7u << (2 * r);
     const int iy0 = 2 * y0 - 1, ix0 = 2 * x0 - 1;
-    stage_tile64_s2<CIN>(s_in, NP == 3 ? x3 : x, b, H, W, 0, iy0, ix0, need);
+    CT_TOCK(0)
+    stage_tile64_s2<CIN, XM>(s_in, NP == 3 ? x3 : x, b, H, W, 0, iy0, ix0, need, s_xm);
+    CT_TOCK(1)
     __syncthreads();
-#define PNX_ROWS_S2(N_) conv_rows_s2<(N_ <= NRMAX ? N_ : NRMAX), CIN, COUT, MB, NP>(s_in, x, x2, x3, wfrag, wfrag2, wfrag3, bias, rbase, rmask, yrow, b, H, W, iy0, ix0, Wo - x0, need, mg, relu, px, kb, lane)
+    CT_TOCK(2)
+#define PNX_ROWS_S2(N_) conv_rows_s2<(N_ <= NRMAX ? N_ : NRMAX), CIN, COUT, MB, NP, XM>(s_in, x, x2, x3, wfrag, wfrag2, wfrag3, bias, rbase, rmask, yrow, b, H, W, iy0, ix0, Wo - x0, need, mg, relu, px, kb, lane, s_xm CT_ARGS)
     switch (nr) {
       case 0: PNX_ROWS_S2(0); break;
       case 1: PNX_ROWS_S2(1); break;
@@ -208,19 +243,30 @@
 #undef PNX_ROWS_S2
   }
   sched_done(slot);
+  CT_FLUSH
 }
 
 template <int CIN, int COUT, int NP>
 int launch_s2(PnxPieces<NP> x, PnxPieces<NP> wfrag, const float* bias, const uint8_t* mask, void* y, int B, int H, int W, int Ho, int Wo, int relu,
-              uint8_t* row_dirty, hipStream_t st) {
+              uint8_t* row_dirty, hipStream_t st, const uint8_t* xmask = nullptr) {
   const int slot = mask != nullptr ? next_sched_slot() : -1;
   int64_t nb = (int64_t)B * ((Ho + S2_TH - 1) / S2_TH) * ((Wo + 31) / 32);
   if (nb > 512) nb = 512;
+  constexpr int lds = S2_NSTAGE * 16;
+  if constexpr (NP == 1) {
+    if (xmask != nullptr && mask != nullptr) {
+      constexpr auto kern_xm = k_conv3x3_s2<CIN, COUT, 1, true>;
+      if (const int rc = pnx_lds_optin<kern_xm>(lds); rc != PNX_OK) return rc;
+      kern_xm<<<(unsigned)nb, 256, lds, st>>>((const uint16_t*)x.hi, nullptr, (const uint4*)wfrag.hi, nullptr, bias, mask, (uint16_t*)y, B, H, W, Ho, Wo, relu,
+                                              row_dirty, slot, nullptr, nullptr, xmask);
+      PNX_LAUNCH_CHECK();
+      return PNX_OK;
+    }
+  }
   constexpr auto kern = k_conv3x3_s2<CIN, COUT, NP>;
-  constexpr int lds = S2_NSTAGE * 16;
   if (const int rc = pnx_lds_optin<kern>(lds); rc != PNX_OK) return rc;
   kern<<<(unsigned)nb, 256, lds, st>>>((const uint16_t*)x.hi, (const uint16_t*)x.slot2(), (const uint4*)wfrag.hi, (const uint4*)wfrag.slot2(), bias, mask,
-                                       (uint16_t*)y, B, H, W, Ho, Wo, relu, row_dirty, slot, (const uint16_t*)x.slot3(), (const uint4*)wfrag.slot3());
+                                       (uint16_t*)y, B, H, W, Ho, Wo, relu, row_dirty, slot, (const uint16_t*)x.slot3(), (const uint4*)wfrag.slot3(), nullptr);
   PNX_LAUNCH_CHECK();
   return PNX_OK;
 }
diff --git a/pillarnext_amd/csrc/conv_taps.h b/pillarnext_amd/csrc/conv_taps.h
--- a/pillarnext_amd/csrc/conv_taps.h
+++ b/pillarnext_amd/csrc/conv_taps.h
@@ -13,10 +13,14 @@
   if ((threadIdx.x & 63) == 0) {                                                     \
     for (int k = 0; k < 8; k++) atomicAdd(&g_conv_T[k], ct_T[k]);                     \
   }
+#define CT_PARAMS , unsigned long long (&ct_T)[8], unsigned long long& tk
+#define CT_ARGS , ct_T, tk
 #else
 #define CT_DECL
 #define CT_TOCK(k)
 #define CT_FLUSH
+#define CT_PARAMS
+#define CT_ARGS
 #endif
 
 constexpr int LDS_TH = 16;
@@ -50,9 +54,52 @@
   }
 }
 
-template <int CSTRIDE, int TH = LDS_TH>
+__device__ __attribute__((aligned(128))) uint4 g_zero_line[8];
+constexpr int XM_ROWS_PER_WAVE = 3;
+__device__ __forceinline__ void xmask_fetch(uint32_t* __restrict__ raw, const uint8_t* __restrict__ xmask, int b, int H, int W, int iy0, int ix0, int n_rows,
+                                            int wv, int lane) {
+  typedef __attribute__((address_space(1))) const void* gptr_t;
+  typedef __attribute__((address_space(3))) void* lptr_t;
+  const int ix = ix0 + lane;
+  if (lane >= LDS_HW) return;
+#pragma unroll
+  for (int k = 0; k < XM_ROWS_PER_WAVE; k++) {
+    const int r = wv + 4 * k, iy = iy0 + r;
+    if (r < n_rows && (unsigned)iy < (unsigned)H && (unsigned)ix < (unsigned)W)
+      __builtin_amdgcn_global_load_lds((gptr_t)(xmask + (((int64_t)b * H + iy) * W + ix)), (lptr_t)(raw + k * LDS_HW), 1, 0, 0);
+    else
+      raw[k * LDS_HW + lane] = 0u;
+  }
+}
+__device__ __forceinline__ uint32_t xmask_word_raw(const uint32_t* __restrict__ raw, int wv, int lane) {
+  uint32_t w = 0;
+#pragma unroll
+  for (int k = 0; k < XM_ROWS_PER_WAVE; k++) w |= ((raw[k * LDS_HW + lane] & 0xffu) != 0 ? 1u : 0u) << (wv + 4 * k);
+  return w;
+}
+__device__ __forceinline__ void xmask_load(const uint8_t* __restrict__ xmask, int b, int H, int W, int iy0, int ix0, int n_rows, int n_cols, int wv, int lane,
+                                           uint8_t (&h)[XM_ROWS_PER_WAVE]) {
+  const int ix = ix0 + lane;
+#pragma unroll
+  for (int k = 0; k < XM_ROWS_PER_WAVE; k++) {
+    const int r = wv + 4 * k, iy = iy0 + r;
+    h[k] = 0;
+    if (r < n_rows && lane < n_cols && (unsigned)iy < (unsigned)H && (unsigned)ix < (unsigned)W) h[k] = xmask[((int64_t)b * H + iy) * W + ix];
+  }
+}
+__device__ __forceinline__ uint32_t xmask_word(const uint8_t (&h)[XM_ROWS_PER_WAVE], int wv) {
+  uint32_t w = 0;
+#pragma unroll
+  for (int k = 0; k < XM_ROWS_PER_WAVE; k++) w |= (h[k] != 0 ? 1u : 0u) << (wv + 4 * k);
+  return w;
+}
+__device__ __forceinline__ uint32_t xmask_col(const uint4* __restrict__ xm, int c) {
+  const uint4 q = xm[c];
+  return q.x | q.y | q.z | q.w;
+}
+template <int CSTRIDE, int TH = LDS_TH, bool XM = false>
 __device__ __forceinline__ void stage_tile64(uint4* __restrict__ s_in, const uint16_t* __restrict__ x, int b, int H, int W, int ch0, int y0, int x0,
-                                             uint32_t need) {
+                                             uint32_t need, const uint4* __restrict__ xm = nullptr) {
   constexpr int NROW = TH + 2, NEXTRA = NROW * 16;
   static_assert(NEXTRA <= 512, "two slots of the extra columns per thread");
   typedef __attribute__((address_space(1))) const void* gptr_t;
@@ -66,10 +113,16 @@
   if (y0 - 1 + NROW > H) rows_in &= (1u << (H - (y0 - 1))) - 1u;
   const bool col_ok = (unsigned)(x0 - 1 + col) < (unsigned)W;
   const uint32_t voff = (uint32_t)(col * CSTRIDE + (slot ^ lds_swz(col)) * 8) * 2u;
+  uint32_t cm = 0;
+  if constexpr (XM) cm = xmask_col(xm, col);
 #pragma unroll
   for (int r = 0; r < NROW; r++) {
     if (!((need >> r) & 1u)) continue;
-    if (((rows_in >> r) & 1u) && col_ok) {
+    if constexpr (XM) {
+      const char* const src = reinterpret_cast<const char*>(xt + (int64_t)r * W * CSTRIDE) + voff;
+      __builtin_amdgcn_global_load_lds((gptr_t)(((cm >> r) & 1u) ? src : reinterpret_cast<const char*>(g_zero_line) + slot * 16),
+                                       (lptr_t)(s_in + (r * LDS_HW + wbase) * 8), 16, 0, 0);
+    } else if (((rows_in >> r) & 1u) && col_ok) {
       __builtin_amdgcn_global_load_lds((gptr_t)(reinterpret_cast<const char*>(xt + (int64_t)r * W * CSTRIDE) + voff),
                                        (lptr_t)(s_in + (r * LDS_HW + wbase) * 8), 16, 0, 0);
     } else {
@@ -82,8 +135,9 @@
     const int re = e >> 4, ce = 32 + ((e >> 3) & 1);
     if (e < NEXTRA && ((need >> re) & 1u)) {
       uint4 qe = make_uint4(0, 0, 0, 0);
-      if (((rows_in >> re) & 1u) && (unsigned)(x0 - 1 + ce) < (unsigned)W)
-        qe = *reinterpret_cast<const uint4*>(xt + ((int64_t)re * W + ce) * CSTRIDE + (e & 7) * 8);
+      bool ld = ((rows_in >> re) & 1u) && (unsigned)(x0 - 1 + ce) < (unsigned)W;
+      if constexpr (XM) ld = ((xmask_col(xm, ce) >> re) & 1u) != 0;
+      if (ld) qe = *reinterpret_cast<const uint4*>(xt + ((int64_t)re * W + ce) * CSTRIDE + (e & 7) * 8);
       s_in[(re * LDS_HW + ce) * 8 + ((e & 7) ^ lds_swz(ce))] = qe;
     }
   }
diff --git a/pillarnext_amd/csrc/conv_tile.h b/pillarnext_amd/csrc/conv_tile.h
--- a/pillarnext_amd/csrc/conv_tile.h
+++ b/pillarnext_amd/csrc/conv_tile.h
@@ -185,4 +185,5 @@
   uint8_t* row_dirty;
   const int32_t *tlist, *tcount;
   hipStream_t st;
+  const uint8_t* xmask;
 };
diff --git a/pillarnext_amd/csrc/enqueue.hip b/pillarnext_amd/csrc/enqueue.hip
--- a/pillarnext_amd/csrc/enqueue.hip
+++ b/pillarnext_amd/csrc/enqueue.hip
@@ -52,8 +52,10 @@
       PNX_REQUIRE(i[0] >= 0 && i[0] <= 8, PNX_ERR_INVALID, "tile list over %d row_dirty arrays (at most 8)", i[0]);
       return pnx_conv_tile_list_prezeroed((const uint8_t*)p[0], (const uint8_t* const*)&p[3], i[0], i[1], i[2], i[3], i[4], (int32_t*)p[1], (int32_t*)p[2], st);
     case PNX_OP_CONV3X3:
-      return (i[7] == PNX_F16 ? pnx_conv3x3_f16 : pnx_conv3x3_bf16)(p[0], p[1], (const float*)p[2], p[3], (const uint8_t*)p[4], (void*)p[5], i[0], i[1], i[2],
-                                                                    i[3], i[4], i[5], i[6], (uint8_t*)p[6], (const int32_t*)p[7], (const int32_t*)p[8], st);
+      return (i[7] == PNX_F16 ? pnx_conv3x3_xm_f16 : pnx_conv3x3_xm_bf16)(p[0], p[1], (const float*)p[2], p[3], (const uint8_t*)p[4],
+                                                                          (const uint8_t*)((i[8] & 1) ? p[4] : p[9]),
+                                                                          (void*)p[5], i[0], i[1], i[2], i[3], i[4], i[5], i[6], (uint8_t*)p[6],
+                                                                          (const int32_t*)p[7], (const int32_t*)p[8], st);
     case PNX_OP_DECONV2X2:
       return (i[6] == PNX_F16 ? pnx_deconv2x2_f16 : pnx_deconv2x2_bf16)(p[0], p[1], (const float*)p[2], (void*)p[3], i[0], i[1], i[2], i[3], i[4], i[5], st);
     case PNX_OP_SEPHEAD_OUT:
diff --git a/pillarnext_amd/models.py b/pillarnext_amd/models.py
--- a/pillarnext_amd/models.py
+++ b/pillarnext_amd/models.py
@@ -989,9 +989,10 @@
         self.cout, self.cin, self.stride = weight.shape[0], weight.shape[1], int(stride)
         self.register_buffer("wfrag", ops.conv3x3_pack_weights(weight, dtype=dtype))
         self.register_buffer("bias", bias.float().contiguous())
-    def forward(self, x, mask=None, residual=None, out=None, tiles=None, plan=None):
+    def forward(self, x, mask=None, residual=None, out=None, tiles=None, plan=None, x_mask=None):
         call = ops.conv3x3_masked if plan is None else plan.conv3x3
-        return call(x, self.wfrag, self.bias, self.cout, self.stride, mask, residual, True, out=out, tiles=tiles if self.stride == 1 else None)
+        kw = {} if x_mask is None else {"x_mask": x_mask}
+        return call(x, self.wfrag, self.bias, self.cout, self.stride, mask, residual, True, out=out, tiles=tiles if self.stride == 1 else None, **kw)
 
 
 class _HipDeconv2x2(nn.Module):
@@ -1274,7 +1275,8 @@
                     assert plan is None
                     return m(inp, mask, residual=res)
                 k += 1
-                return m(inp, mask, residual=res, out=ws[(k - 1) % 3], tiles=tiles, plan=plan)
+                xm = mask if plan is not None and si > 0 and m.stride == 1 else None
+                return m(inp, mask, residual=res, out=ws[(k - 1) % 3], tiles=tiles, plan=plan, x_mask=xm)
 
             x = run(mods[0], x)
             for j in range(1, len(mods), 2):
diff --git a/pillarnext_amd/ops.py b/pillarnext_amd/ops.py
--- a/pillarnext_amd/ops.py
+++ b/pillarnext_amd/ops.py
@@ -638,11 +638,15 @@
     return out
 
 
-def _conv3x3_dims(x, wfrag, cout, stride, mask, residual, out, cuda=False):
+def _conv3x3_dims(x, wfrag, cout, stride, mask, residual, out, cuda=False, x_mask=None):
     xs = _half_nhwc(x, "conv3x3", cuda=cuda)
     if wfrag.dtype != xs.dtype or (residual is not None and _like(residual).dtype != xs.dtype):
         raise PnxError("conv3x3: weights / residual of another dtype than the input")
     B, ci, H, W = xs.shape
+    if x_mask is not None:
+        xm = _like(x_mask)
+        if xm.dtype != torch.uint8 or tuple(xm.shape) != (B, H, W) or xm.device != xs.device or not xm.is_contiguous():
+            raise PnxError("conv3x3: x_mask must be a contiguous uint8 (B, H, W) tensor of the INPUT's sites, on the input's device")
     Ho, Wo = _out_hw(H, W, stride)
     if out is not None:
         y, dirty = out
@@ -652,12 +656,12 @@
     return B, H, W, ci, _DT[xs.dtype], Ho, Wo
 
 
-def conv3x3_masked(x, wfrag, bias, cout, stride=1, mask=None, residual=None, relu=True, out=None, tiles=None):
-    B, H, W, ci, _, Ho, Wo = _conv3x3_dims(x, wfrag, cout, stride, mask, residual, out, cuda=True)
+def conv3x3_masked(x, wfrag, bias, cout, stride=1, mask=None, residual=None, relu=True, out=None, tiles=None, x_mask=None):
+    B, H, W, ci, _, Ho, Wo = _conv3x3_dims(x, wfrag, cout, stride, mask, residual, out, cuda=True, x_mask=x_mask)
     y, dirty = out if out is not None else (torch.empty((B, cout, Ho, Wo), dtype=x.dtype, device=x.device, memory_format=torch.channels_last), None)
     tl, tc = tiles if tiles is not None else (None, None)
-    check(_conv_fn("conv3x3", x.dtype)(ptr(x), ptr(wfrag), ptr(bias), ptr(residual), ptr(mask), ptr(y), B, H, W, ci, cout, stride, 1 if relu else 0,
-                                       ptr(dirty), ptr(tl), ptr(tc), stream_ptr()), "pnx_conv3x3")
+    check(_conv_fn("conv3x3_xm", x.dtype)(ptr(x), ptr(wfrag), ptr(bias), ptr(residual), ptr(mask), ptr(x_mask), ptr(y), B, H, W, ci, cout, stride,
+                                          1 if relu else 0, ptr(dirty), ptr(tl), ptr(tc), stream_ptr()), "pnx_conv3x3")
     return y
 
 
diff --git a/pillarnext_amd/plan.py b/pillarnext_amd/plan.py
--- a/pillarnext_amd/plan.py
+++ b/pillarnext_amd/plan.py
@@ -54,10 +54,12 @@
         self._add(OP_TILE_LIST, [len(dirties), *ops._like(mask).shape, tile_rows], [mask, tl, tc] + list(dirties))
         return out
 
-    def conv3x3(self, x, wfrag, bias, cout, stride=1, mask=None, residual=None, relu=True, out=None, tiles=None):
-        B, H, W, ci, dt, _, _ = ops._conv3x3_dims(x, wfrag, cout, stride, mask, residual, out)
+    def conv3x3(self, x, wfrag, bias, cout, stride=1, mask=None, residual=None, relu=True, out=None, tiles=None, x_mask=None):
+        B, H, W, ci, dt, _, _ = ops._conv3x3_dims(x, wfrag, cout, stride, mask, residual, out, x_mask=x_mask)
         tl, tc = tiles if tiles is not None else (None, None)
-        self._add(OP_CONV3X3, [B, H, W, ci, cout, stride, 1 if relu else 0, dt], [x, wfrag, bias, residual, mask, *out, tl, tc])
+        same = x_mask is not None and x_mask is mask
+        self._add(OP_CONV3X3, [B, H, W, ci, cout, stride, 1 if relu else 0, dt, 1 if same else 0],
+                  [x, wfrag, bias, residual, mask, *out, tl, tc, None if same else x_mask])
         return out[0]
 
     def deconv2x2(self, x, wfrag, bias, cout, y, relu=True):
```

New measurement: 768.9, median of 6. No clear change (+1.0%).
